# aerius-labs/paillier-halo2

Hardware: AMD Instinct MI355X
Metric: Paillier-encrypt proofs/s (2048-bit n, k=17); MSM achieved HBM GB/s vs peak (higher is better)
Workload: dtype u32 limbs (29-bit reduced radix, 254-bit modular integers), u64 limbs (4096-bit integers)

## Files before the change

### include/pz.h

```cpp
#ifndef PZ_H
#define PZ_H

#include <stddef.h>
#include <stdint.h>

#ifdef __cplusplus
extern "C" {
#endif

typedef struct pz_ctx pz_ctx;
typedef struct pz_bases pz_bases;

enum pz_status {
    PZ_OK = 0,
    PZ_ERR_INVALID = -1,
    PZ_ERR_HIP = -2,
    PZ_ERR_NO_DEVICE = -3,
    PZ_ERR_OOM = -4,
    PZ_ERR_ZERO_MODULUS = -5,
    PZ_ERR_RANGE = -6,
    PZ_ERR_UNSUPPORTED = -7,
    PZ_ERR_CAPACITY = -8,
    PZ_ERR_MESSAGE_RANGE = -9,
    PZ_ERR_ASYNC = -10
// ... 135 lines not shown
                     const uint8_t* d_selectors, const uint64_t* constants, size_t n_constants, const uint32_t* d_map_col,
                     const uint32_t* d_map_row, size_t tile, uint64_t* fixed_affine, uint64_t* sigma_affine);
int pz_vk_keygen(pz_ctx* ctx, const pz_bases* bases_lagrange, uint32_t k, uint32_t lookup_bits, size_t n_adv, size_t n_lk,
                 const uint8_t* selectors, const uint64_t* constants, size_t n_constants, const uint32_t* map_col, const uint32_t* map_row,
                 size_t tile, uint64_t* fixed_affine, uint64_t* sigma_affine);
int pz_g1_compress_dev(pz_ctx* ctx, const uint64_t* d_points, size_t n, uint8_t* d_bytes);
int pz_g1_decompress_dev(pz_ctx* ctx, const uint8_t* d_bytes, size_t n, uint64_t* d_points, int32_t* d_status);
int pz_g1_compress(pz_ctx* ctx, const uint64_t* points, size_t n, uint8_t* bytes);
int pz_g1_decompress(pz_ctx* ctx, const uint8_t* bytes, size_t n, uint64_t* points, int32_t* status, uint64_t* n_bad);
int pz_proof_wire_bytes(const pz_vk* vk, size_t* bytes);
int pz_proof_encode(pz_vk* vk, const uint64_t* proofs_words, size_t n_proofs, uint8_t* out_bytes);
int pz_proof_decode(pz_vk* vk, const uint8_t* bytes, size_t n_proofs, uint64_t* out_words, int32_t* status);
int pz_verify_batch_bytes(pz_vk* vk, const uint8_t* bytes, size_t n_proofs, const uint8_t* seeds, const size_t* seed_offsets,
                          int32_t* verdicts, uint64_t* h_evals, uint64_t* ab_affine, int* all_ok);
typedef struct pz_params pz_params;
#define PZ_SERDE_PROCESSED 0
#define PZ_SERDE_RAW 1
#define PZ_SERDE_RAW_UNCHECKED 2
#define PZ_PARAMS_BAD_G1 1u
#define PZ_PARAMS_BAD_G2 2u
#define PZ_PARAMS_BAD_G0 4u
#define PZ_PARAMS_BAD_POWERS 8u
#define PZ_PARAMS_BAD_LAGRANGE 16u
int pz_g2_compress(pz_ctx* ctx, const uint64_t* points, size_t n, uint8_t* bytes);
int pz_g2_decompress(pz_ctx* ctx, const uint8_t* bytes, size_t n, uint64_t* points, int32_t* status, uint64_t* n_bad);
int pz_g2_check_dev(pz_ctx* ctx, const uint64_t* d_points, size_t n, int32_t* d_status);
int pz_g2_check(pz_ctx* ctx, const uint64_t* points, size_t n, int32_t* status);
int pz_params_file_bytes(uint32_t k, int format, size_t* bytes);
int pz_params_decode(pz_ctx* ctx, const uint8_t* bytes, size_t len, int format, pz_params** out, uint64_t* n_bad);
int pz_params_from_dev(pz_ctx* ctx, uint32_t k, const uint64_t* d_g, const uint64_t* d_g_lagrange, const uint64_t g2[16],
                       const uint64_t s_g2[16], pz_params** out);
int pz_params_info(const pz_params* params, uint32_t* k, uint64_t g0_affine[8], uint64_t g2[16], uint64_t s_g2[16]);
int pz_params_points(const pz_params* params, const uint64_t** d_g, const uint64_t** d_g_lagrange);
int pz_params_bases(pz_params* params, int lagrange, const pz_bases** bases);
int pz_params_encode(const pz_params* params, int format, uint8_t* out, size_t capacity);
int pz_params_downsize(const pz_params* params, uint32_t k_new, pz_params** out);
int pz_params_check(pz_params* params, uint32_t* failed, uint32_t* skipped);
int pz_params_free(pz_params* params);
int pz_poly_eval_dev(pz_ctx* ctx, const uint64_t* d_coeffs, size_t n_cols, size_t col_stride, size_t n,
                     const uint64_t x[4], uint64_t* d_out);
int pz_poly_eval_multi_dev(pz_ctx* ctx, const uint64_t* d_coeffs, size_t n_cols, size_t col_stride, size_t n,
                           const uint64_t* xs, uint32_t n_points, uint64_t* d_out);

int pz_fr_batch_invert_dev(pz_ctx* ctx, uint64_t* d_a, size_t n);
int pz_fr_prefix_product_dev(pz_ctx* ctx, const uint64_t* d_a, size_t n, const uint64_t z0[4], uint64_t* d_z);
int pz_permutation_product_dev(pz_ctx* ctx, const uint64_t* d_cols, size_t col_stride, const uint64_t* d_sigma,
                               size_t sigma_stride, size_t m, uint32_t log_n, const uint64_t omega[4],
                               const uint64_t beta[4], const uint64_t gamma[4], const uint64_t delta_start[4],
                               const uint64_t delta[4], const uint64_t z0[4], uint64_t* d_z);
int pz_permutation_product_sets_dev(pz_ctx* ctx, const uint64_t* d_cols, size_t col_stride, const uint64_t* d_sigma,
                                    size_t sigma_stride, size_t m, uint32_t chunk_len, uint32_t log_n, size_t usable_rows,
                                    const uint64_t omega[4], const uint64_t beta[4], const uint64_t gamma[4],
                                    const uint64_t delta[4], uint64_t* d_z, size_t z_stride);
int pz_lookup_permute_dev(pz_ctx* ctx, const uint64_t* d_inputs, size_t n_cols, size_t col_stride,
                          const uint64_t* d_table, size_t rows, uint32_t value_bits, uint64_t* d_perm_inputs,
                          uint64_t* d_perm_tables, size_t out_stride);
int pz_lookup_product_dev(pz_ctx* ctx, const uint64_t* d_inputs, size_t input_stride, const uint64_t* d_table,
                          const uint64_t* d_perm_inputs, size_t perm_input_stride, const uint64_t* d_perm_tables,
                          size_t perm_table_stride, size_t n_lookups, size_t n, const uint64_t beta[4],
                          const uint64_t gamma[4], const uint64_t z0[4], uint64_t* d_z, size_t z_stride);
int pz_quotient_gate_dev(pz_ctx* ctx, const uint64_t* d_adv_ext, size_t adv_stride, const uint64_t* d_sel_ext,
                         size_t sel_stride, size_t n_cols, uint32_t log_ext, uint32_t rot_step, const uint64_t y[4],
                         uint64_t* d_h);
int pz_quotient_permutation_dev(pz_ctx* ctx, const uint64_t* d_cols_ext, size_t col_stride, const uint64_t* d_sigma_ext,
                                size_t sigma_stride, const uint64_t* d_z_ext, size_t z_stride, uint32_t n_sets,
                                uint32_t chunk_len, uint32_t m_total, uint32_t log_ext, uint32_t rot_step,
                                uint32_t last_rotation, const uint64_t* d_l0, const uint64_t* d_l_last,
                                const uint64_t* d_l_active, const uint64_t beta[4], const uint64_t gamma[4],
                                const uint64_t delta[4], const uint64_t coset_g[4], const uint64_t omega_ext[4],
                                const uint64_t y[4], uint64_t* d_h);
int pz_quotient_permutation_part_dev(pz_ctx* ctx, const uint64_t* d_cols_ext, size_t col_stride, const uint64_t* d_sigma_ext,
                                     size_t sigma_stride, const uint64_t* d_z_ext, size_t z_stride, uint32_t n_sets_total,
                                     uint32_t set_lo, uint32_t n_sets, uint32_t chunk_len, uint32_t m_cols, int head, uint32_t log_ext,
                                     uint32_t rot_step, uint32_t last_rotation, const uint64_t* d_l0, const uint64_t* d_l_last,
                                     const uint64_t* d_l_active, const uint64_t beta[4], const uint64_t gamma[4],
                                     const uint64_t delta[4], const uint64_t coset_g[4], const uint64_t omega_ext[4],
                                     const uint64_t y[4], uint64_t* d_h);
int pz_quotient_lookup_dev(pz_ctx* ctx, const uint64_t* d_input_ext, size_t input_stride, const uint64_t* d_table_ext,
                           const uint64_t* d_perm_input_ext, size_t perm_input_stride, const uint64_t* d_perm_table_ext,
                           size_t perm_table_stride, const uint64_t* d_z_ext, size_t z_stride, uint32_t n_lookups,
                           uint32_t log_ext, uint32_t rot_step, const uint64_t* d_l0, const uint64_t* d_l_last,
                           const uint64_t* d_l_active, const uint64_t beta[4], const uint64_t gamma[4], const uint64_t y[4],
                           uint64_t* d_h);
int pz_quotient_finish_dev(pz_ctx* ctx, uint64_t* d_h, uint32_t log_n, uint32_t log_e, const uint64_t coset_g[4],
                           const uint64_t omega_ext[4]);
int pz_fr_distribute_powers_dev(pz_ctx* ctx, uint64_t* d_a, size_t n_cols, size_t col_stride, size_t n,
                                const uint64_t g[4], const uint64_t c[4]);
int pz_fr_lincomb_dev(pz_ctx* ctx, const uint64_t* d_polys, size_t n_cols, size_t col_stride, size_t n,
                      const uint64_t v[4], uint64_t* d_out, int accumulate);
int pz_poly_div_linear_dev(pz_ctx* ctx, const uint64_t* d_coeffs, size_t n_cols, size_t col_stride, size_t n,
                           const uint64_t x[4], uint64_t* d_q, size_t q_stride);

typedef struct pz_shplonk pz_shplonk;
int pz_shplonk_begin_dev(pz_ctx* ctx, size_t n, uint32_t n_sets, const uint32_t* set_n_polys, const uint64_t* const* d_polys,
                         const uint32_t* set_n_points, const uint32_t* point_idx, uint32_t n_points_total, const uint64_t* points,
                         const uint64_t* evals, const uint64_t y[4], const uint64_t v[4], uint64_t* d_h, pz_shplonk** state);
int pz_shplonk_finish_dev(pz_ctx* ctx, pz_shplonk* state, const uint64_t u[4], const uint64_t* d_h, uint64_t* d_h2);
int pz_shplonk_free(pz_ctx* ctx, pz_shplonk* state);

typedef struct pz_structure pz_structure;
int pz_circuit_structure_dev(pz_ctx* ctx, int kind, uint32_t limbs_n, uint32_t limb_bits, uint32_t lookup_bits, uint32_t k,
                             const uint64_t* exp_g, const uint64_t* exp_r, size_t minimum_rows, uint32_t blinding_factors,
                             pz_structure** out);
int pz_structure_info(const pz_structure* st, size_t* n_adv, size_t* n_adv_filled, size_t* n_lk, size_t* max_rows, size_t* n_constants,
                      size_t* n_cells, size_t* n_lookups, size_t* n_steps_g, size_t* n_steps_r);
int pz_structure_arrays(const pz_structure* st, const uint8_t** d_selectors, const uint32_t** d_map_col, const uint32_t** d_map_row,
                        const uint64_t** d_col_starts, const uint64_t** constants, const uint64_t** col_starts_host);
int pz_structure_free(pz_structure* st);

typedef struct pz_pk pz_pk;
typedef struct pz_proof pz_proof;
#define PZ_BLINDING_SEEDED_TEST_STREAM (~(size_t)0)
#define PZ_PK_EXT_ALL (~(size_t)0)
int pz_pk_create(pz_ctx* ctx, const pz_bases* bases_lagrange, const pz_bases* bases_monomial, uint32_t k, uint32_t lookup_bits,
                 uint32_t blinding_factors, size_t max_rows, size_t n_adv, size_t n_lk, const uint8_t* selectors,
                 const uint64_t* constants, size_t n_constants, const uint32_t* map_col, const uint32_t* map_row, size_t tile,
                 size_t ext_resident_cols, pz_pk** out);
int pz_pk_create_dev(pz_ctx* ctx, const pz_bases* bases_lagrange, const pz_bases* bases_monomial, uint32_t k, uint32_t lookup_bits,
                     uint32_t blinding_factors, size_t max_rows, size_t n_adv, size_t n_lk, const uint8_t* d_selectors,
                     const uint64_t* constants, size_t n_constants, const uint32_t* d_map_col, const uint32_t* d_map_row, size_t tile,
                     size_t ext_resident_cols, pz_pk** out);
int pz_pk_info(const pz_pk* pk, size_t* n_fixed, size_t* n_perm_cols, size_t* n_sets, size_t* blinding_words, size_t* evals_words);
int pz_pk_commitments(const pz_pk* pk, uint64_t* fixed_affine, uint64_t* sigma_affine);
int pz_pk_free(pz_pk* pk);
int pz_proof_begin(pz_pk* pk, uint64_t* d_cols, uint64_t seed, const uint64_t* blinding, size_t n_blinding, pz_proof** out,
                   uint64_t* advice_affine);
int pz_proof_lookups(pz_proof* proof, const uint64_t theta[4], uint64_t* perm_inputs_affine, uint64_t* perm_tables_affine);
int pz_proof_products(pz_proof* proof, const uint64_t beta[4], const uint64_t gamma[4], uint64_t* perm_z_affine,
                      uint64_t* lookup_z_affine, uint64_t* random_affine);
int pz_proof_quotient(pz_proof* proof, const uint64_t y[4], uint64_t* h_affine);
int pz_proof_evaluate(pz_proof* proof, const uint64_t x[4], uint64_t* evals);
int pz_proof_open_begin(pz_proof* proof, const uint64_t y[4], const uint64_t v[4], uint64_t* w1_affine);
int pz_proof_open_finish(pz_proof* proof, const uint64_t u[4], uint64_t* w2_affine, int* quotient_degree_ok);
int pz_proof_free(pz_proof* proof);

int pz_circuit_public_cells(int kind, uint32_t limbs_n, uint32_t limb_bits, uint32_t lookup_bits, size_t n_steps_g, size_t n_steps_r,
                            uint64_t* cells_out, size_t capacity, size_t* n_public);
int pz_structure_expose(pz_structure* st);
int pz_structure_public(const pz_structure* st, size_t* n_instance, size_t* n_public, const uint32_t** d_cell_col, const uint32_t** d_cell_row);
int pz_public_gather_dev(pz_ctx* ctx, const uint64_t* d_cols, size_t col_stride, const uint32_t* d_cell_col, const uint32_t* d_cell_row,
                         size_t n_public, uint64_t* out_words);
int pz_instance_eval_dev(pz_ctx* ctx, uint32_t k, const uint64_t omega[4], const uint64_t n_inv[4], const uint64_t* d_instances,
                         size_t n_public, size_t n_proofs, const uint64_t* d_x, uint64_t* d_out, int32_t* d_flags);
int pz_pk_create_pub(pz_ctx* ctx, const pz_bases* bases_lagrange, const pz_bases* bases_monomial, uint32_t k, uint32_t lookup_bits,
                     uint32_t blinding_factors, size_t max_rows, size_t n_adv, size_t n_lk, size_t n_instance, size_t n_public,
                     const uint8_t* selectors, const uint64_t* constants, size_t n_constants, const uint32_t* map_col, const uint32_t* map_row,
                     size_t tile, size_t ext_resident_cols, pz_pk** out);
int pz_pk_create_pub_dev(pz_ctx* ctx, const pz_bases* bases_lagrange, const pz_bases* bases_monomial, uint32_t k, uint32_t lookup_bits,
                         uint32_t blinding_factors, size_t max_rows, size_t n_adv, size_t n_lk, size_t n_instance, size_t n_public,
                         const uint8_t* d_selectors, const uint64_t* constants, size_t n_constants, const uint32_t* d_map_col,
                         const uint32_t* d_map_row, size_t tile, size_t ext_resident_cols, pz_pk** out);
int pz_vk_keygen_pub_dev(pz_ctx* ctx, const pz_bases* bases_lagrange, uint32_t k, uint32_t lookup_bits, size_t n_adv, size_t n_lk,
                         size_t n_instance, size_t n_public, const uint8_t* d_selectors, const uint64_t* constants, size_t n_constants,
                         const uint32_t* d_map_col, const uint32_t* d_map_row, size_t tile, uint64_t* fixed_affine, uint64_t* sigma_affine);
int pz_vk_keygen_pub(pz_ctx* ctx, const pz_bases* bases_lagrange, uint32_t k, uint32_t lookup_bits, size_t n_adv, size_t n_lk,
                     size_t n_instance, size_t n_public, const uint8_t* selectors, const uint64_t* constants, size_t n_constants,
                     const uint32_t* map_col, const uint32_t* map_row, size_t tile, uint64_t* fixed_affine, uint64_t* sigma_affine);
int pz_vk_create_pub(pz_ctx* ctx, uint32_t k, uint32_t blinding_factors, size_t n_adv, size_t n_lk, size_t n_instance, size_t n_public,
                     const uint64_t* fixed_affine, const uint64_t* sigma_affine, const uint64_t g0_affine[8], const uint64_t g2[16],
                     const uint64_t s_g2[16], pz_vk** out);
int pz_proof_begin_pub(pz_pk* pk, uint64_t* d_cols, uint64_t seed, const uint64_t* blinding, size_t n_blinding, const uint64_t* instances,
                       size_t n_public, pz_proof** out, uint64_t* advice_affine);
int pz_verify_batch_pub(pz_vk* vk, const uint64_t* instances, size_t n_public, const uint64_t* proofs, size_t n_proofs, const uint8_t* seeds,
                        const size_t* seed_offsets, int32_t* verdicts, uint64_t* h_evals, uint64_t* ab_affine, int* all_ok);
int pz_verify_batch_bytes_pub(pz_vk* vk, const uint64_t* instances, size_t n_public, const uint8_t* bytes, size_t n_proofs,
                              const uint8_t* seeds, const size_t* seed_offsets, int32_t* verdicts, uint64_t* h_evals, uint64_t* ab_affine,
// ... 17 lines not shown
```

### paillier_halo2_amd/_lib.py

```python
from __future__ import annotations

import ctypes as C
import os
import subprocess

_HERE = os.path.dirname(os.path.abspath(__file__))
CSRC = os.path.join(_HERE, "csrc")
SO_PATH = os.path.join(CSRC, "libpz_hip.so")
PROBE_SO_PATH = os.path.join(CSRC, "libpz_probe.so")

U64P = C.POINTER(C.c_uint64)
U32P = C.POINTER(C.c_uint32)
VP = C.c_void_p

SIGNATURES = {
    "pz_init": (C.c_int, [C.c_int, C.POINTER(C.c_int), C.POINTER(VP)]),
    "pz_free": (C.c_int, [VP]),
    "pz_strerror": (C.c_char_p, [C.c_int]),
    "pz_last_hip_error": (C.c_char_p, [VP]),
    "pz_set_stream": (C.c_int, [VP, VP]),
    "pz_sync": (C.c_int, [VP]),
    "pz_abi_version": (C.c_int, []),
    "pz_dev_alloc": (C.c_int, [VP, C.c_size_t, C.POINTER(VP)]),
    "pz_dev_cache_limit": (C.c_int, [VP, C.c_size_t]),
# ... 27 lines not shown
    "pz_ntt_fr_to_dev": (C.c_int, [VP, VP, C.c_size_t, VP, C.c_size_t, C.c_size_t, VP, C.c_uint32, VP, VP]),
    "pz_ntt_fr_extend_dev": (C.c_int, [VP, VP, C.c_size_t, C.c_size_t, VP, C.c_size_t, C.c_uint32, C.c_uint32, VP, VP, VP]),
    "pz_ntt_fr_coeff_extend_dev": (C.c_int, [VP, VP, C.c_size_t, C.c_size_t, VP, C.c_size_t, C.c_uint32, C.c_uint32, VP, VP, VP,
                                             VP]),
    "pz_fr_convert_dev": (C.c_int, [VP, VP, C.c_size_t, C.c_int]),
    "pz_fr_from_mask_dev": (C.c_int, [VP, VP, C.c_size_t, VP]),
    "pz_mul_mod": (C.c_int, [VP, C.c_uint32, VP, VP, VP, VP, VP]),
    "pz_paillier_trace": (C.c_int, [VP, C.c_uint32, VP, VP, VP, C.c_uint32, VP, C.POINTER(C.c_size_t), VP]),
    "pz_paillier_encrypt": (C.c_int, [VP, C.c_uint32, C.c_size_t, VP, VP, VP, VP, VP, C.c_size_t, VP, VP, VP]),
    "pz_paillier_encrypt_dev": (C.c_int, [VP, C.c_uint32, C.c_size_t, VP, VP, VP, VP, VP, C.c_size_t, VP, VP, VP]),
    "pz_paillier_encrypt_uniform": (C.c_int, [VP, C.c_uint32, C.c_size_t, C.c_uint32, VP, VP, VP, VP, VP, C.c_size_t, VP, VP, VP]),
    "pz_paillier_encrypt_uniform_dev": (C.c_int, [VP, C.c_uint32, C.c_size_t, C.c_uint32, VP, VP, VP, VP, VP, C.c_size_t, VP, VP, VP]),
    "pz_witness_cells_per_step": (C.c_int, [C.c_uint32, C.c_uint32, C.c_uint32, C.POINTER(C.c_size_t),
                                            C.POINTER(C.c_size_t)]),
    "pz_witness_expand": (C.c_int, [VP, C.c_uint32, C.c_uint32, C.c_uint32, VP, C.c_size_t, VP, VP, VP]),
    "pz_witness_expand_dev": (C.c_int, [VP, C.c_uint32, C.c_uint32, C.c_uint32, VP, C.c_size_t, VP, VP, VP]),
    "pz_refresh_aux": (C.c_int, [C.c_uint32, C.c_uint32, C.c_uint32, VP, C.c_uint32, U32P]),
    "pz_op_cells": (C.c_int, [C.c_int, C.c_uint32, C.c_uint32, C.c_uint32, C.POINTER(C.c_size_t), C.POINTER(C.c_size_t)]),
    "pz_circuit_cells": (C.c_int, [C.c_int, C.c_uint32, C.c_uint32, C.c_uint32, C.c_size_t, C.c_size_t, C.POINTER(C.c_size_t),
                                   C.POINTER(C.c_size_t)]),
    "pz_circuit_expand_dev": (C.c_int, [VP, C.c_int, C.c_uint32, C.c_uint32, C.c_uint32, VP, VP, C.c_size_t, C.c_size_t, VP, VP, VP,
                                        C.c_size_t, C.c_size_t]),
    "pz_circuit_break_points": (C.c_int, [VP, C.c_size_t, C.c_size_t, VP, C.c_size_t, C.POINTER(C.c_size_t)]),
    "pz_circuit_expand_cols_dev": (C.c_int, [VP, C.c_int, C.c_uint32, C.c_uint32, C.c_uint32, VP, VP, C.c_size_t, C.c_size_t, VP, VP, VP,
                                             VP, C.c_size_t, C.c_size_t, C.c_size_t, C.c_size_t]),
    "pz_srs_setup_g1_dev": (C.c_int, [VP, C.c_uint32, VP, VP, VP, VP]),
    "pz_srs_lagrange_from_monomial_dev": (C.c_int, [VP, C.c_uint32, VP, VP, VP, VP]),
    "pz_permutation_sigma_dev": (C.c_int, [VP, VP, VP, C.c_size_t, C.c_uint32, VP, VP, VP, C.c_size_t]),
    "pz_permutation_sigma_part_dev": (C.c_int, [VP, VP, VP, C.c_size_t, C.c_size_t, C.c_size_t, C.c_uint32, VP, VP, VP, C.c_size_t]),
    "pz_keygen_columns_dev": (C.c_int, [VP, VP, VP, C.c_size_t, C.c_size_t, C.c_uint32, C.c_uint32, VP, VP, VP, VP, VP, VP, C.c_size_t]),
    "pz_poly_eval_dev": (C.c_int, [VP, VP, C.c_size_t, C.c_size_t, C.c_size_t, VP, VP]),
    "pz_poly_eval_multi_dev": (C.c_int, [VP, VP, C.c_size_t, C.c_size_t, C.c_size_t, VP, C.c_uint32, VP]),
    "pz_g1_check_dev": (C.c_int, [VP, VP, C.c_size_t, C.POINTER(C.c_uint64)]),
    "pz_g2_generator": (C.c_int, [VP]),
    "pz_g2_mul_dev": (C.c_int, [VP, VP, VP, C.c_size_t, VP]),
    "pz_pairing_dev": (C.c_int, [VP, VP, VP, C.c_size_t, VP]),
    "pz_pairing_check_dev": (C.c_int, [VP, VP, VP, C.c_size_t, C.c_uint32, VP]),
    "pz_vk_create": (C.c_int, [VP, C.c_uint32, C.c_uint32, C.c_size_t, C.c_size_t, VP, VP, VP, VP, VP, C.POINTER(VP)]),
    "pz_vk_info": (C.c_int, [VP, C.POINTER(C.c_size_t), C.POINTER(C.c_size_t)]),
    "pz_verify_batch": (C.c_int, [VP, VP, C.c_size_t, VP, VP, VP, VP, VP, C.POINTER(C.c_int)]),
    "pz_vk_free": (C.c_int, [VP]),
    "pz_vk_keygen_dev": (C.c_int, [VP, VP, C.c_uint32, C.c_uint32, C.c_size_t, C.c_size_t, VP, VP, C.c_size_t, VP, VP, C.c_size_t, VP, VP]),
    "pz_vk_keygen": (C.c_int, [VP, VP, C.c_uint32, C.c_uint32, C.c_size_t, C.c_size_t, VP, VP, C.c_size_t, VP, VP, C.c_size_t, VP, VP]),
    "pz_g1_compress_dev": (C.c_int, [VP, VP, C.c_size_t, VP]),
    "pz_g1_decompress_dev": (C.c_int, [VP, VP, C.c_size_t, VP, VP]),
    "pz_g1_compress": (C.c_int, [VP, VP, C.c_size_t, VP]),
    "pz_g1_decompress": (C.c_int, [VP, VP, C.c_size_t, VP, VP, C.POINTER(C.c_uint64)]),
    "pz_proof_wire_bytes": (C.c_int, [VP, C.POINTER(C.c_size_t)]),
    "pz_proof_encode": (C.c_int, [VP, VP, C.c_size_t, VP]),
    "pz_proof_decode": (C.c_int, [VP, VP, C.c_size_t, VP, VP]),
    "pz_verify_batch_bytes": (C.c_int, [VP, VP, C.c_size_t, VP, VP, VP, VP, VP, C.POINTER(C.c_int)]),
    "pz_g2_compress": (C.c_int, [VP, VP, C.c_size_t, VP]),
    "pz_g2_decompress": (C.c_int, [VP, VP, C.c_size_t, VP, VP, C.POINTER(C.c_uint64)]),
    "pz_g2_check_dev": (C.c_int, [VP, VP, C.c_size_t, VP]),
    "pz_g2_check": (C.c_int, [VP, VP, C.c_size_t, VP]),
    "pz_params_file_bytes": (C.c_int, [C.c_uint32, C.c_int, C.POINTER(C.c_size_t)]),
    "pz_params_decode": (C.c_int, [VP, VP, C.c_size_t, C.c_int, C.POINTER(VP), C.POINTER(C.c_uint64)]),
    "pz_params_from_dev": (C.c_int, [VP, C.c_uint32, VP, VP, VP, VP, C.POINTER(VP)]),
    "pz_params_info": (C.c_int, [VP, U32P, VP, VP, VP]),
    "pz_params_points": (C.c_int, [VP, C.POINTER(VP), C.POINTER(VP)]),
    "pz_params_bases": (C.c_int, [VP, C.c_int, C.POINTER(VP)]),
    "pz_params_encode": (C.c_int, [VP, C.c_int, VP, C.c_size_t]),
    "pz_params_downsize": (C.c_int, [VP, C.c_uint32, C.POINTER(VP)]),
    "pz_params_check": (C.c_int, [VP, U32P, U32P]),
    "pz_params_free": (C.c_int, [VP]),
    "pz_fr_batch_invert_dev": (C.c_int, [VP, VP, C.c_size_t]),
    "pz_fr_prefix_product_dev": (C.c_int, [VP, VP, C.c_size_t, VP, VP]),
    "pz_permutation_product_dev": (C.c_int, [VP, VP, C.c_size_t, VP, C.c_size_t, C.c_size_t, C.c_uint32, VP, VP, VP, VP,
                                             VP, VP, VP]),
    "pz_lookup_permute_dev": (C.c_int, [VP, VP, C.c_size_t, C.c_size_t, VP, C.c_size_t, C.c_uint32, VP, VP, C.c_size_t]),
    "pz_lookup_product_dev": (C.c_int, [VP, VP, C.c_size_t, VP, VP, C.c_size_t, VP, C.c_size_t, C.c_size_t, C.c_size_t, VP, VP,
                                        VP, VP, C.c_size_t]),
    "pz_permutation_product_sets_dev": (C.c_int, [VP, VP, C.c_size_t, VP, C.c_size_t, C.c_size_t, C.c_uint32, C.c_uint32,
                                                  C.c_size_t, VP, VP, VP, VP, VP, C.c_size_t]),
    "pz_quotient_gate_dev": (C.c_int, [VP, VP, C.c_size_t, VP, C.c_size_t, C.c_size_t, C.c_uint32, C.c_uint32, VP, VP]),
    "pz_quotient_permutation_dev": (C.c_int, [VP, VP, C.c_size_t, VP, C.c_size_t, VP, C.c_size_t, C.c_uint32, C.c_uint32,
                                              C.c_uint32, C.c_uint32, C.c_uint32, C.c_uint32, VP, VP, VP, VP, VP, VP, VP, VP,
                                              VP, VP]),
    "pz_quotient_permutation_part_dev": (C.c_int, [VP, VP, C.c_size_t, VP, C.c_size_t, VP, C.c_size_t, C.c_uint32, C.c_uint32, C.c_uint32,
                                                   C.c_uint32, C.c_uint32, C.c_int, C.c_uint32, C.c_uint32, C.c_uint32, VP, VP, VP, VP, VP,
                                                   VP, VP, VP, VP, VP]),
    "pz_quotient_lookup_dev": (C.c_int, [VP, VP, C.c_size_t, VP, VP, C.c_size_t, VP, C.c_size_t, VP, C.c_size_t, C.c_uint32,
                                         C.c_uint32, C.c_uint32, VP, VP, VP, VP, VP, VP, VP]),
    "pz_quotient_finish_dev": (C.c_int, [VP, VP, C.c_uint32, C.c_uint32, VP, VP]),
    "pz_fr_distribute_powers_dev": (C.c_int, [VP, VP, C.c_size_t, C.c_size_t, C.c_size_t, VP, VP]),
    "pz_fr_lincomb_dev": (C.c_int, [VP, VP, C.c_size_t, C.c_size_t, C.c_size_t, VP, VP, C.c_int]),
    "pz_poly_div_linear_dev": (C.c_int, [VP, VP, C.c_size_t, C.c_size_t, C.c_size_t, VP, VP, C.c_size_t]),
    "pz_shplonk_begin_dev": (C.c_int, [VP, C.c_size_t, C.c_uint32, U32P, C.POINTER(VP), U32P, U32P, C.c_uint32, VP, VP, VP, VP, VP,
                                       C.POINTER(VP)]),
    "pz_shplonk_finish_dev": (C.c_int, [VP, VP, VP, VP, VP]),
    "pz_shplonk_free": (C.c_int, [VP, VP]),
    "pz_circuit_structure_dev": (C.c_int, [VP, C.c_int, C.c_uint32, C.c_uint32, C.c_uint32, C.c_uint32, VP, VP, C.c_size_t, C.c_uint32, C.POINTER(VP)]),
    "pz_structure_info": (C.c_int, [VP] + [C.POINTER(C.c_size_t)] * 9),
    "pz_structure_arrays": (C.c_int, [VP] + [C.POINTER(VP)] * 6),
    "pz_structure_free": (C.c_int, [VP]),
    "pz_pk_create": (C.c_int, [VP, VP, VP, C.c_uint32, C.c_uint32, C.c_uint32, C.c_size_t, C.c_size_t, C.c_size_t, VP, VP, C.c_size_t, VP, VP,
                               C.c_size_t, C.c_size_t, C.POINTER(VP)]),
    "pz_pk_create_dev": (C.c_int, [VP, VP, VP, C.c_uint32, C.c_uint32, C.c_uint32, C.c_size_t, C.c_size_t, C.c_size_t, VP, VP, C.c_size_t, VP, VP,
                                   C.c_size_t, C.c_size_t, C.POINTER(VP)]),
    "pz_pk_info": (C.c_int, [VP, C.POINTER(C.c_size_t), C.POINTER(C.c_size_t), C.POINTER(C.c_size_t), C.POINTER(C.c_size_t),
                             C.POINTER(C.c_size_t)]),
    "pz_pk_commitments": (C.c_int, [VP, VP, VP]),
    "pz_pk_free": (C.c_int, [VP]),
    "pz_proof_begin": (C.c_int, [VP, VP, C.c_uint64, VP, C.c_size_t, C.POINTER(VP), VP]),
    "pz_proof_lookups": (C.c_int, [VP, VP, VP, VP]),
    "pz_proof_products": (C.c_int, [VP, VP, VP, VP, VP, VP]),
    "pz_proof_quotient": (C.c_int, [VP, VP, VP]),
    "pz_proof_evaluate": (C.c_int, [VP, VP, VP]),
    "pz_proof_open_begin": (C.c_int, [VP, VP, VP, VP]),
    "pz_proof_open_finish": (C.c_int, [VP, VP, VP, C.POINTER(C.c_int)]),
    "pz_proof_free": (C.c_int, [VP]),
    "pz_circuit_public_cells": (C.c_int, [C.c_int, C.c_uint32, C.c_uint32, C.c_uint32, C.c_size_t, C.c_size_t, VP, C.c_size_t, C.POINTER(C.c_size_t)]),
    "pz_structure_expose": (C.c_int, [VP]),
    "pz_structure_public": (C.c_int, [VP, C.POINTER(C.c_size_t), C.POINTER(C.c_size_t), C.POINTER(VP), C.POINTER(VP)]),
    "pz_public_gather_dev": (C.c_int, [VP, VP, C.c_size_t, VP, VP, C.c_size_t, VP]),
    "pz_instance_eval_dev": (C.c_int, [VP, C.c_uint32, VP, VP, VP, C.c_size_t, C.c_size_t, VP, VP, VP]),
    "pz_pk_create_pub": (C.c_int, [VP, VP, VP, C.c_uint32, C.c_uint32, C.c_uint32, C.c_size_t, C.c_size_t, C.c_size_t, C.c_size_t, C.c_size_t, VP, VP,
                                   C.c_size_t, VP, VP, C.c_size_t, C.c_size_t, C.POINTER(VP)]),
    "pz_pk_create_pub_dev": (C.c_int, [VP, VP, VP, C.c_uint32, C.c_uint32, C.c_uint32, C.c_size_t, C.c_size_t, C.c_size_t, C.c_size_t, C.c_size_t, VP,
                                       VP, C.c_size_t, VP, VP, C.c_size_t, C.c_size_t, C.POINTER(VP)]),
    "pz_vk_keygen_pub_dev": (C.c_int, [VP, VP, C.c_uint32, C.c_uint32, C.c_size_t, C.c_size_t, C.c_size_t, C.c_size_t, VP, VP, C.c_size_t, VP, VP,
                                       C.c_size_t, VP, VP]),
    "pz_vk_keygen_pub": (C.c_int, [VP, VP, C.c_uint32, C.c_uint32, C.c_size_t, C.c_size_t, C.c_size_t, C.c_size_t, VP, VP, C.c_size_t, VP, VP,
                                   C.c_size_t, VP, VP]),
    "pz_vk_create_pub": (C.c_int, [VP, C.c_uint32, C.c_uint32, C.c_size_t, C.c_size_t, C.c_size_t, C.c_size_t, VP, VP, VP, VP, VP, C.POINTER(VP)]),
    "pz_proof_begin_pub": (C.c_int, [VP, VP, C.c_uint64, VP, C.c_size_t, VP, C.c_size_t, C.POINTER(VP), VP]),
    "pz_verify_batch_pub": (C.c_int, [VP, VP, C.c_size_t, VP, C.c_size_t, VP, VP, VP, VP, VP, C.POINTER(C.c_int)]),
    "pz_verify_batch_bytes_pub": (C.c_int, [VP, VP, C.c_size_t, VP, C.c_size_t, VP, VP, VP, VP, VP, C.POINTER(C.c_int)]),
    "pz_key_digest": (C.c_int, [C.c_uint32, C.c_uint32, C.c_size_t, C.c_size_t, C.c_size_t, C.c_size_t, VP, VP, VP]),
    "pz_pk_digest": (C.c_int, [VP, VP]),
    "pz_vk_digest": (C.c_int, [VP, VP]),
    "pz_vk_bind": (C.c_int, [VP, C.c_int]),
    "pz_vk_is_bound": (C.c_int, [VP, C.POINTER(C.c_int)]),
    "pz_timing_enable": (C.c_int, [VP, C.c_int]),
    "pz_timing_reset": (C.c_int, [VP]),
    "pz_timing_get": (C.c_int, [VP, C.c_int, C.POINTER(C.c_double), C.POINTER(C.c_uint64)]),
}

_lib = None


def build(force: bool = False) -> str:
    args = ["make", "-C", CSRC, "-j4"]
    if force:
        args.append("-B")
    subprocess.check_call(args, stdout=subprocess.DEVNULL)
    if not os.path.exists(SO_PATH):
        raise RuntimeError("libpz_hip.so was not produced by the build")
    return SO_PATH


def lib():
    global _lib
    if _lib is None:
        if not os.path.exists(SO_PATH):
            raise RuntimeError(
                f"{SO_PATH} is missing: build it with `python -c 'import __graft_entry__ as g; g.build()'` "
                "(hipcc --offload-arch=gfx950). There is no CPU fallback."
            )
        try:
            import torch
        except Exception:
            pass
        l = C.CDLL(SO_PATH)
        for name, (res, args) in SIGNATURES.items():
            fn = getattr(l, name)
# ... 37 lines not shown
```

### paillier_halo2_amd/csrc/pz_quotient.hip

```cpp
#include "fp29.cuh"
#include "pz_internal.h"

static inline Fr fp_one_host() {
    static const uint64_t ONE[4] = {0xac96341c4ffffffbULL, 0x36fc76959f60cd29ULL, 0x666ea36f7879462eULL, 0x0e0a77c19a07df2fULL};
    Fr r;
    memcpy(r.v, ONE, 32);
    return r;
}
static inline Fr fr_from_u64(const uint64_t x[4]) {
    Fr r;
    memcpy(r.v, x, 32);
    return r;
}

typedef F29<FrTag> Fr29;
__device__ __forceinline__ Fr29 fr29_c261(const Fr& c) { return f29_to_261(f29_from_fp(c)); }
__device__ __forceinline__ Fr29 fr29_one256() {
    Fr29 r;
#pragma unroll
    for (int i = 0; i < 9; ++i) r.v[i] = P29<FrTag>::R256(i);
    return r;
}

struct S29 {
// ... 502 lines not shown
    const Fr* p = a + (size_t)blockIdx.y * cs;
    const size_t lo = c * KD_K, hi = (lo + KD_K < n ? lo + KD_K : n);
    Fr v = fp_zero<FrTag>();
    for (size_t i = hi; i-- > lo;) v = fp_add(fp_mul(v, x), fp_load<FrTag>(p + i));
    fp_store(L + (size_t)blockIdx.y * n_chunks + c, v);
}
__global__ __launch_bounds__(256) void k_kd_carry(Fr* __restrict__ L, size_t n_chunks, Fr x) {
    __shared__ Fr s_v[256], s_x[256];
    Fr* l = L + (size_t)blockIdx.x * n_chunks;
    Fr xk = x;
    for (unsigned s = 1; s < KD_K; s <<= 1) xk = fp_sqr(xk);
    const size_t per = (n_chunks + 255) / 256;
    const size_t lo = threadIdx.x * per, hi = lo + per < n_chunks ? lo + per : n_chunks;
    Fr V = fp_zero<FrTag>(), X = fp_one<FrTag>();
    for (size_t c = hi; c-- > lo && c < n_chunks;) {
        V = fp_add(fp_load<FrTag>(l + c), fp_mul(xk, V));
        X = fp_mul(X, xk);
    }
    s_v[threadIdx.x] = V;
    s_x[threadIdx.x] = X;
    __syncthreads();
    for (unsigned off = 1; off < 256; off <<= 1) {
        Fr v = s_v[threadIdx.x], xx = s_x[threadIdx.x];
        Fr uv = fp_zero<FrTag>(), ux = fp_one<FrTag>();
        const bool has = threadIdx.x + off < 256;
        if (has) { uv = s_v[threadIdx.x + off]; ux = s_x[threadIdx.x + off]; }
        __syncthreads();
        if (has) {
            s_v[threadIdx.x] = fp_add(v, fp_mul(xx, uv));
            s_x[threadIdx.x] = fp_mul(xx, ux);
        }
        __syncthreads();
    }
    Fr carry = threadIdx.x + 1 < 256 ? s_v[threadIdx.x + 1] : fp_zero<FrTag>();
    for (size_t c = hi; c-- > lo && c < n_chunks;) {
        Fr t = fp_load<FrTag>(l + c);
        fp_store(l + c, carry);
        carry = fp_add(t, fp_mul(xk, carry));
    }
}
__global__ __launch_bounds__(256) void k_kd_apply(const Fr* a, size_t cs, size_t n, Fr x,
                                                  const Fr* __restrict__ L, size_t n_chunks, Fr* q, size_t qs) {
    const size_t c = (size_t)blockIdx.x * blockDim.x + threadIdx.x;
    if (c >= n_chunks) return;
    const Fr* p = a + (size_t)blockIdx.y * cs;
    Fr* o = q + (size_t)blockIdx.y * qs;
    const size_t lo = c * KD_K, hi = (lo + KD_K < n ? lo + KD_K : n);
    Fr cur = fp_load<FrTag>(L + (size_t)blockIdx.y * n_chunks + c);
    for (size_t i = hi; i-- > lo;) {
        Fr ai = fp_load<FrTag>(p + i);
        fp_store(o + i, cur);
        cur = fp_add(ai, fp_mul(x, cur));
    }
}

extern "C" int pz_poly_div_linear_dev(pz_ctx* ctx, const uint64_t* d_coeffs, size_t n_cols, size_t col_stride, size_t n,
                                      const uint64_t x[4], uint64_t* d_q, size_t q_stride) {
    if (!ctx || !x || (n_cols && n && (!d_coeffs || !d_q)) || col_stride % 4 || q_stride % 4) return PZ_ERR_INVALID;
    if (n_cols > 1 && (col_stride < 4 * n || q_stride < 4 * n)) return PZ_ERR_INVALID;
    if (n_cols == 0 || n == 0) return PZ_OK;
    if (n_cols > 65535) return PZ_ERR_INVALID;
    PZ_ENTER(ctx);
    const size_t nch = pz_div_up(n, KD_K);
    void* L;
    PZCHK(pz_ws_get(ctx, WS_BIG_A, n_cols * nch * 32, &L));
    Fr xv = fr_from_u64(x);
    hipLaunchKernelGGL(k_kd_local, dim3(pz_div_up(nch, 256), (unsigned)n_cols), dim3(256), 0, ctx->stream,
                       (const Fr*)d_coeffs, col_stride / 4, n, xv, (Fr*)L, nch);
    hipLaunchKernelGGL(k_kd_carry, dim3((unsigned)n_cols), dim3(256), 0, ctx->stream, (Fr*)L, nch, xv);
    hipLaunchKernelGGL(k_kd_apply, dim3(pz_div_up(nch, 256), (unsigned)n_cols), dim3(256), 0, ctx->stream,
                       (const Fr*)d_coeffs, col_stride / 4, n, xv, (const Fr*)L, nch, (Fr*)d_q, q_stride / 4);
    HIPCHK(ctx, hipGetLastError());
    return PZ_OK;
}

struct PermQ {
    const Fr *cols, *sigma, *z, *l0, *llast, *lactive, *xpow;
    size_t cs, ss, zs, N;
    unsigned n_sets, chunk_len, m_total, step, last_rot;
    unsigned set_lo, n_sets_total, head;
    S29 y, gamma, delta, beta266;
    S29 bx266;
    S29 y_chain, y_sets;
};
__global__ __launch_bounds__(256) void k_quotient_permutation(PermQ q, Fr* __restrict__ h) {
    const size_t i0 = (size_t)blockIdx.x * blockDim.x + threadIdx.x;
    const size_t half = q.N >> 1;
    if (i0 >= half) return;
    const size_t mask = q.N - 1;
    size_t row[2], i_next[2], i_last[2];
    Fr29 acc[2];
#pragma unroll
    for (int r = 0; r < 2; ++r) {
        row[r] = i0 + (r ? half : 0);
        i_next[r] = (row[r] + q.step) & mask;
        i_last[r] = (row[r] + q.N - (size_t)q.last_rot * q.step) & mask;
        acc[r] = f29_load<FrTag>(h + row[r]);
    }
#pragma unroll
    for (int r = 0; r < 2 && q.head; ++r) {
        const size_t i = row[r];
        const Fr29 one = fr29_one256();
        const Fr29 l0 = f29_load_shl5<FrTag>(q.l0 + i);
        const Fr29 z_first = f29_load<FrTag>(q.z + i);
        acc[r] = f29_mul2_s(acc[r], q.y.v, f29_sub<2, 29>(one, z_first), l0);
        {
            const Fr29 ll = f29_load_shl5<FrTag>(q.llast + i);
            const Fr zl = fp_load<FrTag>(q.z + (size_t)(q.n_sets_total - 1) * q.zs + i);
            const Fr29 z_lastset = f29_from_fp(zl);
            acc[r] = f29_mul2_s(acc[r], q.y.v, f29_sub<2, 29>(f29_mul(z_lastset, f29_from_fp_shl5(zl)), z_lastset), ll);
        }
        if (q.n_sets_total > 1) {
            Fr29 t0 = f29_sub<2, 29>(f29_load<FrTag>(q.z + q.zs + i), f29_load<FrTag>(q.z + i_last[r]));
            for (unsigned j = 2; j < q.n_sets_total; ++j) {
                const Fr29 d = f29_sub<2, 29>(f29_load<FrTag>(q.z + (size_t)j * q.zs + i), f29_load<FrTag>(q.z + (size_t)(j - 1) * q.zs + i_last[r]));
                t0 = f29_add(f29_mul_s(t0, q.y.v), d);
            }
            acc[r] = f29_mul2_s(acc[r], q.y_chain.v, t0, l0);
        }
    }
    Fr29 cur = f29_mul_s(f29_load<FrTag>(q.xpow + i0), q.bx266.v);
    unsigned c = 0;
    Fr v_n[2], s_n[2];
#pragma unroll
    for (int r = 0; r < 2; ++r) {
        v_n[r] = fp_load<FrTag>(q.cols + row[r]);
        s_n[r] = fp_load<FrTag>(q.sigma + row[r]);
    }
    Fr29 hs[2];
    for (unsigned j = 0; j < q.n_sets; ++j) {
        Fr29 left[2], right[2];
#pragma unroll
        for (int r = 0; r < 2; ++r) {
            left[r] = f29_load<FrTag>(q.z + (size_t)(q.set_lo + j) * q.zs + i_next[r]);
            right[r] = f29_load<FrTag>(q.z + (size_t)(q.set_lo + j) * q.zs + row[r]);
        }
        for (unsigned t = 0; t < q.chunk_len && c < q.m_total; ++t, ++c) {
            const unsigned cn = c + 1 < q.m_total ? c + 1 : c;
#pragma unroll
            for (int r = 0; r < 2; ++r) {
                const Fr29 v = f29_add_s(f29_from_fp_shl5(v_n[r]), q.gamma.v);
                const Fr29 sg = f29_from_fp(s_n[r]);
                v_n[r] = fp_load<FrTag>(q.cols + (size_t)cn * q.cs + row[r]);
                s_n[r] = fp_load<FrTag>(q.sigma + (size_t)cn * q.ss + row[r]);
                left[r] = f29_mul(left[r], f29_add(v, f29_mul_s(sg, q.beta266.v)));
                right[r] = f29_mul(right[r], r ? f29_sub<2, 29>(v, cur) : f29_add(v, cur));
            }
            cur = f29_mul_s(cur, q.delta.v);
        }
#pragma unroll
        for (int r = 0; r < 2; ++r) {
            const Fr29 diff = f29_sub<2, 29>(left[r], right[r]);
            hs[r] = j ? f29_add(f29_mul_s(hs[r], q.y.v), diff) : diff;
        }
    }
#pragma unroll
    for (int r = 0; r < 2; ++r) {
        acc[r] = f29_mul2_s(acc[r], q.y_sets.v, hs[r], f29_load_shl5<FrTag>(q.lactive + row[r]));
        f29_store<0>(h + row[r], acc[r]);
    }
}

extern "C" int pz_quotient_permutation_part_dev(pz_ctx* ctx, const uint64_t* d_cols_ext, size_t col_stride,
                                                const uint64_t* d_sigma_ext, size_t sigma_stride, const uint64_t* d_z_ext,
                                                size_t z_stride, uint32_t n_sets_total, uint32_t set_lo, uint32_t n_sets,
                                                uint32_t chunk_len, uint32_t m_cols, int head, uint32_t log_ext, uint32_t rot_step,
                                                uint32_t last_rotation, const uint64_t* d_l0, const uint64_t* d_l_last,
                                                const uint64_t* d_l_active, const uint64_t beta[4], const uint64_t gamma[4],
                                                const uint64_t delta[4], const uint64_t coset_g[4], const uint64_t omega_ext[4],
                                                const uint64_t y[4], uint64_t* d_h) {
    if (!ctx || !d_cols_ext || !d_sigma_ext || !d_z_ext || !d_l0 || !d_l_last || !d_l_active || !beta || !gamma || !delta ||
        !coset_g || !omega_ext || !y || !d_h)
        return PZ_ERR_INVALID;
    if (log_ext > 28 || log_ext == 0 || n_sets == 0 || chunk_len == 0 || m_cols == 0 || col_stride % 4 || sigma_stride % 4 || z_stride % 4)
        return PZ_ERR_INVALID;
    if (n_sets_total == 0 || (size_t)set_lo + n_sets > n_sets_total) return PZ_ERR_INVALID;
    const size_t N = (size_t)1 << log_ext;
    if ((size_t)n_sets * chunk_len < m_cols || (size_t)(n_sets - 1) * chunk_len >= m_cols) return PZ_ERR_INVALID;
    if (set_lo + n_sets < n_sets_total && (size_t)n_sets * chunk_len != m_cols) return PZ_ERR_INVALID;
    if (rot_step == 0 || rot_step >= N || (size_t)last_rotation * rot_step >= N) return PZ_ERR_INVALID;
    if ((m_cols > 1 && (col_stride < 4 * N || sigma_stride < 4 * N)) || (n_sets_total > 1 && z_stride < 4 * N)) return PZ_ERR_INVALID;
    if (!host_fr_canonical(beta) || !host_fr_canonical(gamma) || !host_fr_canonical(delta) || !host_fr_canonical(y)) return PZ_ERR_INVALID;
    PZ_ENTER(ctx);
    PermQ q;
    q.cols = (const Fr*)d_cols_ext; q.sigma = (const Fr*)d_sigma_ext; q.z = (const Fr*)d_z_ext;
    q.l0 = (const Fr*)d_l0; q.llast = (const Fr*)d_l_last; q.lactive = (const Fr*)d_l_active;
    q.cs = col_stride / 4; q.ss = sigma_stride / 4; q.zs = z_stride / 4; q.N = N;
    q.n_sets = n_sets; q.chunk_len = chunk_len; q.m_total = m_cols; q.step = rot_step; q.last_rot = last_rotation;
    q.set_lo = set_lo; q.n_sets_total = n_sets_total; q.head = head ? 1u : 0u;
    q.beta266 = host_fr_shl(beta, 10); q.gamma = host_fr_shl(gamma, 5); q.delta = host_fr_shl(delta, 5); q.y = host_fr_shl(y, 5);
    uint64_t yp[4], bx[4];
    host_fr_pow(delta, set_lo * chunk_len, bx);
    host_fr_mul(bx, beta, bx);
    q.bx266 = host_fr_shl(bx, 10);
    host_fr_pow(y, n_sets_total - 1, yp);
    q.y_chain = host_fr_shl(yp, 5);
    host_fr_pow(y, n_sets, yp);
    q.y_sets = host_fr_shl(yp, 5);
    void* xp;
    PZCHK(pz_get_pow_table(ctx, omega_ext, N, &xp, coset_g));
    q.xpow = (const Fr*)xp;
    hipLaunchKernelGGL(k_quotient_permutation, dim3(pz_div_up(N / 2, 256)), dim3(256), 0, ctx->stream, q, (Fr*)d_h);
    HIPCHK(ctx, hipGetLastError());
    return PZ_OK;
}
extern "C" int pz_quotient_permutation_dev(pz_ctx* ctx, const uint64_t* d_cols_ext, size_t col_stride,
                                           const uint64_t* d_sigma_ext, size_t sigma_stride, const uint64_t* d_z_ext,
                                           size_t z_stride, uint32_t n_sets, uint32_t chunk_len, uint32_t m_total,
                                           uint32_t log_ext, uint32_t rot_step, uint32_t last_rotation,
                                           const uint64_t* d_l0, const uint64_t* d_l_last, const uint64_t* d_l_active,
                                           const uint64_t beta[4], const uint64_t gamma[4], const uint64_t delta[4],
                                           const uint64_t coset_g[4], const uint64_t omega_ext[4], const uint64_t y[4],
                                           uint64_t* d_h) {
    return pz_quotient_permutation_part_dev(ctx, d_cols_ext, col_stride, d_sigma_ext, sigma_stride, d_z_ext, z_stride, n_sets, 0, n_sets,
                                            chunk_len, m_total, 1, log_ext, rot_step, last_rotation, d_l0, d_l_last, d_l_active, beta, gamma,
                                            delta, coset_g, omega_ext, y, d_h);
}

struct LookQ {
    const Fr *a, *s, *ap, *sp, *z, *l0, *llast, *lactive;
    size_t as, aps, sps, zs, N;
    unsigned n_lookups, step;
    S29 beta, gamma, y;
};
__global__ __launch_bounds__(256) void k_quotient_lookup(LookQ q, Fr* __restrict__ h) {
    const size_t i = (size_t)blockIdx.x * blockDim.x + threadIdx.x;
    if (i >= q.N) return;
    const size_t mask = q.N - 1;
    const size_t i_next = (i + q.step) & mask, i_prev = (i + q.N - q.step) & mask;
    const Fr29 one = fr29_one256();
    const Fr29 l0 = f29_load_shl5<FrTag>(q.l0 + i), ll = f29_load_shl5<FrTag>(q.llast + i), la = f29_load_shl5<FrTag>(q.lactive + i);
    const Fr29 sg = f29_add_s(f29_load_shl5<FrTag>(q.s + i), q.gamma.v);
    Fr29 acc = f29_load<FrTag>(h + i);
    for (unsigned k = 0; k < q.n_lookups; ++k) {
        const Fr zf = fp_load<FrTag>(q.z + (size_t)k * q.zs + i);
        const Fr29 z = f29_from_fp(zf), zn = f29_load<FrTag>(q.z + (size_t)k * q.zs + i_next);
        const Fr apf = fp_load<FrTag>(q.ap + (size_t)k * q.aps + i), spf = fp_load<FrTag>(q.sp + (size_t)k * q.sps + i);
        const Fr29 ap = f29_from_fp(apf), sp = f29_from_fp(spf);
        acc = f29_mul2_s(acc, q.y.v, f29_sub<2, 29>(one, z), l0);
        acc = f29_mul2_s(acc, q.y.v, f29_sub<2, 29>(f29_mul(z, f29_from_fp_shl5(zf)), z), ll);
        const Fr29 f1 = f29_mul(f29_add_s(f29_from_fp_shl5(apf), q.beta.v), f29_add_s(f29_from_fp_shl5(spf), q.gamma.v));
        const Fr29 f2 = f29_mul(f29_add_s(f29_load_shl5<FrTag>(q.a + (size_t)k * q.as + i), q.beta.v), sg);
        acc = f29_mul2_s(acc, q.y.v, f29_sub<2, 29>(f29_mul(zn, f1), f29_mul(z, f2)), la);
        const Fr29 ams = f29_carry(f29_sub<2, 29>(ap, sp));
        acc = f29_mul2_s(acc, q.y.v, ams, l0);
        const Fr29 dprev = f29_sub<64, 29>(f29_from_fp_shl5(apf), f29_load_shl5<FrTag>(q.ap + (size_t)k * q.aps + i_prev));
        acc = f29_mul2_s(acc, q.y.v, f29_mul(ams, dprev), la);
    }
    f29_store<0>(h + i, acc);
}

extern "C" int pz_quotient_lookup_dev(pz_ctx* ctx, const uint64_t* d_input_ext, size_t input_stride, const uint64_t* d_table_ext,
                                      const uint64_t* d_perm_input_ext, size_t perm_input_stride,
                                      const uint64_t* d_perm_table_ext, size_t perm_table_stride, const uint64_t* d_z_ext,
                                      size_t z_stride, uint32_t n_lookups, uint32_t log_ext, uint32_t rot_step,
                                      const uint64_t* d_l0, const uint64_t* d_l_last, const uint64_t* d_l_active,
                                      const uint64_t beta[4], const uint64_t gamma[4], const uint64_t y[4], uint64_t* d_h) {
    if (!ctx || !d_input_ext || !d_table_ext || !d_perm_input_ext || !d_perm_table_ext || !d_z_ext || !d_l0 || !d_l_last ||
        !d_l_active || !beta || !gamma || !y || !d_h)
        return PZ_ERR_INVALID;
    if (log_ext > 28 || input_stride % 4 || perm_input_stride % 4 || perm_table_stride % 4 || z_stride % 4) return PZ_ERR_INVALID;
    const size_t N = (size_t)1 << log_ext;
    if (rot_step == 0 || rot_step >= N) return PZ_ERR_INVALID;
    if (n_lookups > 1 && (input_stride < 4 * N || perm_input_stride < 4 * N || perm_table_stride < 4 * N || z_stride < 4 * N))
        return PZ_ERR_INVALID;
    if (!host_fr_canonical(beta) || !host_fr_canonical(gamma) || !host_fr_canonical(y)) return PZ_ERR_INVALID;
    if (n_lookups == 0) return PZ_OK;
    PZ_ENTER(ctx);
    LookQ q;
    q.a = (const Fr*)d_input_ext; q.s = (const Fr*)d_table_ext; q.ap = (const Fr*)d_perm_input_ext;
    q.sp = (const Fr*)d_perm_table_ext; q.z = (const Fr*)d_z_ext;
    q.l0 = (const Fr*)d_l0; q.llast = (const Fr*)d_l_last; q.lactive = (const Fr*)d_l_active;
    q.as = input_stride / 4; q.aps = perm_input_stride / 4; q.sps = perm_table_stride / 4; q.zs = z_stride / 4; q.N = N;
    q.n_lookups = n_lookups; q.step = rot_step;
    q.beta = host_fr_shl(beta, 5); q.gamma = host_fr_shl(gamma, 5); q.y = host_fr_shl(y, 5);
    hipLaunchKernelGGL(k_quotient_lookup, dim3(pz_div_up(N, 256)), dim3(256), 0, ctx->stream, q, (Fr*)d_h);
    HIPCHK(ctx, hipGetLastError());
    return PZ_OK;
}

__global__ __launch_bounds__(256) void k_lincomb(const Fr* __restrict__ p, size_t cs, unsigned n_cols, size_t n, Fr v,
                                                 Fr* __restrict__ out, int accumulate) {
    const size_t i = (size_t)blockIdx.x * blockDim.x + threadIdx.x;
    if (i >= n) return;
    Fr acc = accumulate ? fp_load<FrTag>(out + i) : fp_zero<FrTag>();
    for (unsigned j = 0; j < n_cols; ++j) acc = fp_add(fp_mul(acc, v), fp_load<FrTag>(p + (size_t)j * cs + i));
    fp_store(out + i, acc);
}

extern "C" int pz_fr_lincomb_dev(pz_ctx* ctx, const uint64_t* d_polys, size_t n_cols, size_t col_stride, size_t n,
                                 const uint64_t v[4], uint64_t* d_out, int accumulate) {
    if (!ctx || !v || (n && (!d_out || (n_cols && !d_polys))) || col_stride % 4 || (n_cols > 1 && col_stride < 4 * n))
        return PZ_ERR_INVALID;
    if (n_cols > 0xffffffffu) return PZ_ERR_INVALID;
    if (n == 0) return PZ_OK;
    PZ_ENTER(ctx);
    hipLaunchKernelGGL(k_lincomb, dim3(pz_div_up(n, 256)), dim3(256), 0, ctx->stream, (const Fr*)d_polys, col_stride / 4,
                       (unsigned)n_cols, n, fr_from_u64(v), (Fr*)d_out, accumulate);
    HIPCHK(ctx, hipGetLastError());
    return PZ_OK;
}
```

### paillier_halo2_amd/engine.py

```python
from __future__ import annotations

import ctypes as C
from typing import Optional, Sequence, Tuple

import numpy as np

from . import _lib
from ._lib import PzError, VP


def _np(a, shape_last: Optional[int] = None) -> np.ndarray:
    arr = np.ascontiguousarray(a, dtype=np.uint64)
    if shape_last is not None and (arr.ndim == 0 or arr.shape[-1] != shape_last):
        arr = arr.reshape(-1, shape_last)
    return arr


def _ptr(a: np.ndarray) -> VP:
    return VP(a.ctypes.data)


class Bases:

    def __init__(self, engine: "Engine", handle: VP):
# ... 690 lines not shown
        self._chk(self.L.pz_poly_eval_dev(self.ctx, VP(d_coeffs), n_cols, col_stride_u64, n, _ptr(_np(x).reshape(4)),
                                          VP(d_out)), "pz_poly_eval_dev")

    def poly_eval_multi_dev(self, d_coeffs: int, n_cols: int, col_stride_u64: int, n: int, xs, d_out: int):
        x = _np(xs).reshape(-1, 4)
        self._chk(self.L.pz_poly_eval_multi_dev(self.ctx, VP(d_coeffs), n_cols, col_stride_u64, n, _ptr(x), x.shape[0], VP(d_out)),
                  "pz_poly_eval_multi_dev")

    def _fr1(self, x):
        a = _np(x).reshape(4)
        keep = self.__dict__.setdefault("_keep", [])
        keep.append(a)
        del keep[:-32]
        return _ptr(a)

    def fr_batch_invert_dev(self, d_a: int, n: int):
        self._chk(self.L.pz_fr_batch_invert_dev(self.ctx, VP(d_a), n), "pz_fr_batch_invert_dev")

    def fr_prefix_product_dev(self, d_a: int, n: int, z0, d_z: int):
        self._chk(self.L.pz_fr_prefix_product_dev(self.ctx, VP(d_a), n, self._fr1(z0), VP(d_z)), "pz_fr_prefix_product_dev")

    def permutation_product_dev(self, d_cols: int, col_stride_u64: int, d_sigma: int, sigma_stride_u64: int, m: int,
                                log_n: int, omega, beta, gamma, delta_start, delta, z0, d_z: int):
        self._chk(self.L.pz_permutation_product_dev(self.ctx, VP(d_cols), col_stride_u64, VP(d_sigma), sigma_stride_u64, m,
                                                    log_n, self._fr1(omega), self._fr1(beta), self._fr1(gamma),
                                                    self._fr1(delta_start), self._fr1(delta), self._fr1(z0), VP(d_z)),
                  "pz_permutation_product_dev")

    def lookup_permute_dev(self, d_inputs: int, n_cols: int, col_stride_u64: int, d_table: int, rows: int, value_bits: int,
                           d_perm_inputs: int, d_perm_tables: int, out_stride_u64: int):
        self._chk(self.L.pz_lookup_permute_dev(self.ctx, VP(d_inputs), n_cols, col_stride_u64, VP(d_table), rows, value_bits,
                                               VP(d_perm_inputs), VP(d_perm_tables), out_stride_u64), "pz_lookup_permute_dev")

    def lookup_product_dev(self, d_inputs: int, input_stride_u64: int, d_table: int, d_perm_inputs: int,
                           perm_input_stride_u64: int, d_perm_tables: int, perm_table_stride_u64: int, n_lookups: int, n: int,
                           beta, gamma, z0, d_z: int, z_stride_u64: int):
        self._chk(self.L.pz_lookup_product_dev(self.ctx, VP(d_inputs), input_stride_u64, VP(d_table), VP(d_perm_inputs),
                                               perm_input_stride_u64, VP(d_perm_tables), perm_table_stride_u64, n_lookups, n,
                                               self._fr1(beta), self._fr1(gamma), self._fr1(z0), VP(d_z), z_stride_u64),
                  "pz_lookup_product_dev")

    def permutation_product_sets_dev(self, d_cols: int, col_stride_u64: int, d_sigma: int, sigma_stride_u64: int, m: int,
                                     chunk_len: int, log_n: int, usable_rows: int, omega, beta, gamma, delta, d_z: int,
                                     z_stride_u64: int):
        self._chk(self.L.pz_permutation_product_sets_dev(self.ctx, VP(d_cols), col_stride_u64, VP(d_sigma), sigma_stride_u64, m,
                                                         chunk_len, log_n, usable_rows, self._fr1(omega), self._fr1(beta),
                                                         self._fr1(gamma), self._fr1(delta), VP(d_z), z_stride_u64),
                  "pz_permutation_product_sets_dev")

    def quotient_gate_dev(self, d_adv_ext: int, adv_stride_u64: int, d_sel_ext: int, sel_stride_u64: int, n_cols: int,
                          log_ext: int, rot_step: int, y, d_h: int):
        self._chk(self.L.pz_quotient_gate_dev(self.ctx, VP(d_adv_ext), adv_stride_u64, VP(d_sel_ext), sel_stride_u64,
                                              n_cols, log_ext, rot_step, self._fr1(y), VP(d_h)), "pz_quotient_gate_dev")

    def quotient_permutation_dev(self, d_cols_ext: int, col_stride_u64: int, d_sigma_ext: int, sigma_stride_u64: int,
                                 d_z_ext: int, z_stride_u64: int, n_sets: int, chunk_len: int, m_total: int, log_ext: int,
                                 rot_step: int, last_rotation: int, d_l0: int, d_l_last: int, d_l_active: int, beta, gamma,
                                 delta, coset_g, omega_ext, y, d_h: int):
        self._chk(self.L.pz_quotient_permutation_dev(
            self.ctx, VP(d_cols_ext), col_stride_u64, VP(d_sigma_ext), sigma_stride_u64, VP(d_z_ext), z_stride_u64, n_sets,
            chunk_len, m_total, log_ext, rot_step, last_rotation, VP(d_l0), VP(d_l_last), VP(d_l_active), self._fr1(beta),
            self._fr1(gamma), self._fr1(delta), self._fr1(coset_g), self._fr1(omega_ext), self._fr1(y), VP(d_h)),
            "pz_quotient_permutation_dev")

    def quotient_permutation_part_dev(self, d_cols_ext: int, col_stride_u64: int, d_sigma_ext: int, sigma_stride_u64: int, d_z_ext: int,
                                      z_stride_u64: int, n_sets_total: int, set_lo: int, n_sets: int, chunk_len: int, m_cols: int,
                                      head: bool, log_ext: int, rot_step: int, last_rotation: int, d_l0: int, d_l_last: int,
                                      d_l_active: int, beta, gamma, delta, coset_g, omega_ext, y, d_h: int):
        self._chk(self.L.pz_quotient_permutation_part_dev(
            self.ctx, VP(d_cols_ext), col_stride_u64, VP(d_sigma_ext), sigma_stride_u64, VP(d_z_ext), z_stride_u64, n_sets_total, set_lo,
            n_sets, chunk_len, m_cols, int(head), log_ext, rot_step, last_rotation, VP(d_l0), VP(d_l_last), VP(d_l_active),
            self._fr1(beta), self._fr1(gamma), self._fr1(delta), self._fr1(coset_g), self._fr1(omega_ext), self._fr1(y), VP(d_h)),
            "pz_quotient_permutation_part_dev")

    def quotient_lookup_dev(self, d_input_ext: int, input_stride_u64: int, d_table_ext: int, d_perm_input_ext: int,
                            perm_input_stride_u64: int, d_perm_table_ext: int, perm_table_stride_u64: int, d_z_ext: int,
                            z_stride_u64: int, n_lookups: int, log_ext: int, rot_step: int, d_l0: int, d_l_last: int,
                            d_l_active: int, beta, gamma, y, d_h: int):
        self._chk(self.L.pz_quotient_lookup_dev(
            self.ctx, VP(d_input_ext), input_stride_u64, VP(d_table_ext), VP(d_perm_input_ext), perm_input_stride_u64,
            VP(d_perm_table_ext), perm_table_stride_u64, VP(d_z_ext), z_stride_u64, n_lookups, log_ext, rot_step, VP(d_l0),
            VP(d_l_last), VP(d_l_active), self._fr1(beta), self._fr1(gamma), self._fr1(y), VP(d_h)), "pz_quotient_lookup_dev")

    def quotient_finish_dev(self, d_h: int, log_n: int, log_e: int, coset_g, omega_ext):
        self._chk(self.L.pz_quotient_finish_dev(self.ctx, VP(d_h), log_n, log_e, self._fr1(coset_g), self._fr1(omega_ext)),
                  "pz_quotient_finish_dev")

    def fr_distribute_powers_dev(self, d_a: int, n_cols: int, col_stride_u64: int, n: int, g, c=None):
        self._chk(self.L.pz_fr_distribute_powers_dev(self.ctx, VP(d_a), n_cols, col_stride_u64, n, self._fr1(g),
                                                     self._fr1(c) if c is not None else None),
                  "pz_fr_distribute_powers_dev")

    def fr_lincomb_dev(self, d_polys: int, n_cols: int, col_stride_u64: int, n: int, v, d_out: int, accumulate: bool = False):
        self._chk(self.L.pz_fr_lincomb_dev(self.ctx, VP(d_polys), n_cols, col_stride_u64, n, self._fr1(v), VP(d_out),
                                           int(accumulate)), "pz_fr_lincomb_dev")

    def poly_div_linear_dev(self, d_coeffs: int, n_cols: int, col_stride_u64: int, n: int, x, d_q: int, q_stride_u64: int):
        self._chk(self.L.pz_poly_div_linear_dev(self.ctx, VP(d_coeffs), n_cols, col_stride_u64, n, self._fr1(x), VP(d_q),
                                                q_stride_u64), "pz_poly_div_linear_dev")

    def shplonk_begin_dev(self, n: int, sets, points, y, v, d_h: int):
        n_sets = len(sets)
        npol = (C.c_uint32 * n_sets)(*[len(s_[0]) for s_ in sets])
        npts = (C.c_uint32 * n_sets)(*[len(s_[1]) for s_ in sets])
        ptrs = [p for s_ in sets for p in s_[0]]
        parr = (VP * len(ptrs))(*[VP(p) for p in ptrs])
        idx = [i for s_ in sets for i in s_[1]]
        iarr = (C.c_uint32 * len(idx))(*idx)
        pts = _np(points, 4)
        ev = np.ascontiguousarray(np.concatenate([_np(s_[2]).reshape(-1, 4) for s_ in sets]), dtype=np.uint64)
        st = VP()
        self._chk(self.L.pz_shplonk_begin_dev(self.ctx, n, n_sets, npol, parr, npts, iarr, pts.shape[0], _ptr(pts), _ptr(ev), self._fr1(y),
                                              self._fr1(v), VP(d_h), C.byref(st)), "pz_shplonk_begin_dev")
        return st

    def shplonk_finish_dev(self, state, u, d_h: int, d_h2: int):
        self._chk(self.L.pz_shplonk_finish_dev(self.ctx, state, self._fr1(u), VP(d_h), VP(d_h2)), "pz_shplonk_finish_dev")

    def timing_enable(self, on: bool = True):
        self._chk(self.L.pz_timing_enable(self.ctx, int(on)), "pz_timing_enable")

    def timing_reset(self):
        self._chk(self.L.pz_timing_reset(self.ctx), "pz_timing_reset")

    def timing_get(self, which: int) -> Tuple[float, int]:
        ms = C.c_double()
        n = C.c_uint64()
        self._chk(self.L.pz_timing_get(self.ctx, which, C.byref(ms), C.byref(n)), "pz_timing_get")
        return ms.value, n.value

    def dev_alloc(self, nbytes: int) -> int:
        d = VP()
        self._chk(self.L.pz_dev_alloc(self.ctx, nbytes, C.byref(d)), "pz_dev_alloc")
        return d.value or 0

    def dev_free(self, d: int):
        self._chk(self.L.pz_dev_free(self.ctx, VP(d)), "pz_dev_free")

    def dev_arena(self, nbytes: int):
        self._chk(self.L.pz_dev_arena(self.ctx, C.c_size_t(nbytes)), "pz_dev_arena")

    def dev_arena_info(self) -> dict:
        out = (C.c_uint64 * 6)()
        self._chk(self.L.pz_dev_arena_info(self.ctx, out), "pz_dev_arena_info")
        return dict(zip(("bytes", "used", "peak", "largest_hole", "served", "missed"), (int(v) for v in out)))

    def dev_mem_info(self):
        f, t = C.c_size_t(0), C.c_size_t(0)
        self._chk(self.L.pz_dev_mem_info(self.ctx, C.byref(f), C.byref(t)), "pz_dev_mem_info")
        return int(f.value), int(t.value)

    def upload(self, d_dst: int, arr):
        a = np.ascontiguousarray(arr)
        self._chk(self.L.pz_upload(self.ctx, VP(d_dst), VP(a.ctypes.data), a.nbytes), "pz_upload")

    def download(self, d_src: int, shape, dtype=np.uint64) -> np.ndarray:
        out = np.empty(shape, dtype=dtype)
        self._chk(self.L.pz_download(self.ctx, VP(out.ctypes.data), VP(d_src), out.nbytes), "pz_download")
        return out

    def dev_memset(self, d: int, value: int, nbytes: int):
        self._chk(self.L.pz_dev_memset(self.ctx, VP(d), value, nbytes), "pz_dev_memset")

    def dev_copy(self, d_dst: int, d_src: int, nbytes: int):
        self._chk(self.L.pz_dev_copy(self.ctx, VP(d_dst), VP(d_src), nbytes), "pz_dev_copy")

# ... 9 lines not shown
```

### paillier_halo2_amd/host/create_proof.hpp

```cpp
#pragma once
#include <cstdint>
#include <cstdio>
#include <cstdlib>
#include <cstring>
#include <functional>
#include <memory>
#include <string>
#include <vector>

#include "../../include/pz.h"
#include "fr_host.hpp"
#include "key_digest.hpp"
#include "transcript.hpp"

namespace pzp {
using pzh::Fr;

struct PzpError {
    int rc;
};
#ifdef PZP_THROW
#define PZP_FAIL(rc_, what_) throw ::pzp::PzpError{rc_}
#else
#define PZP_FAIL(rc_, what_)                                                                               \
// ... 168 lines not shown
        if (!dmc || !dmr) {
            void *mc = tmp.get(m * n * 4), *mr = tmp.get(m * n * 4);
            PZP_CK(pz_upload(cx.c, mc, st.map_col.data(), m * n * 4));
            PZP_CK(pz_upload(cx.c, mr, st.map_row.data(), m * n * 4));
            dmc = (const uint32_t*)mc;
            dmr = (const uint32_t*)mr;
        }
        const Fr delta = pzh::delta();
        PZP_CK(pz_permutation_sigma_dev(cx.c, dmc, dmr, m, st.k, d.omega.v, delta.v, sigma, 4 * n));
        PZP_CK(pz_sync(cx.c));
    }
    {
        Structure& s_ = pk->st;
        std::vector<uint8_t>().swap(s_.selectors);
        std::vector<uint32_t>().swap(s_.map_col);
        std::vector<uint32_t>().swap(s_.map_row);
    }
    pk->sigma_lagrange = cx.alloc(cx.cols(m) * n * 4);
    PZP_CK(pz_dev_copy(cx.c, pk->sigma_lagrange, sigma, m * n * 32));
    uint64_t* com_f = cx.alloc(cx.cols(F) * 12);
    uint64_t* com_s = cx.alloc(cx.cols(m) * 12);
    for (int pi = 0; pi < 2; ++pi) {
        pk->fixed_ext[pi] = cx.alloc((pk->res_fixed ? cx.cols(pk->res_fixed) : 1) * d.parts[pi].size * 4);
        pk->sigma_ext[pi] = cx.alloc((pk->res_sigma ? cx.cols(pk->res_sigma) : 1) * d.parts[pi].size * 4);
        pk->l_ext[pi] = cx.alloc(3 * d.parts[pi].size * 4);
        pk->table_ext[pi] = cx.alloc(d.parts[pi].size * 4);
    }
    struct Job { uint64_t* cols; size_t cnt; uint64_t* com; uint64_t** ext; size_t res; };
    Job jobs[2] = {{fixed, F, com_f, pk->fixed_ext, pk->res_fixed}, {sigma, m, com_s, pk->sigma_ext, pk->res_sigma}};
    for (auto& jb : jobs) {
        for (size_t c0 = 0; c0 < jb.cnt; c0 += 256) {
            const size_t cnt = jb.cnt - c0 < 256 ? jb.cnt - c0 : 256;
            const size_t r_here = jb.res <= c0 ? 0 : (jb.res - c0 < cnt ? jb.res - c0 : cnt);
            const size_t lo[2] = {c0, c0 + r_here}, bc[2] = {r_here, cnt - r_here};
            for (int keep = 1; keep >= 0; --keep) {
                const size_t b0 = lo[1 - keep], bn = bc[1 - keep];
                if (!bn) continue;
                const Part& A_ = d.parts[0];
                PZP_CK(pz_keygen_columns_dev(cx.c, bl, jb.cols + b0 * n * 4, bn, 4 * n, st.k, A_.log_e, d.omega.v, d.omega_inv.v, d.n_inv.v,
                                             A_.gens.data(), jb.com + b0 * 12, keep ? jb.ext[0] + b0 * A_.size * 4 : nullptr, 4 * A_.size));
                if (!keep) continue;
                const Part& B_ = d.parts[1];
                PZP_CK(pz_ntt_fr_extend_dev(cx.c, jb.cols + b0 * n * 4, bn, 4 * n, jb.ext[1] + b0 * B_.size * 4, 4 * B_.size, st.k, B_.log_e, d.omega.v,
                                            B_.gens.data(), nullptr));
            }
        }
    }
    pk->fixed_coeff = fixed;
    pk->sigma_coeff = sigma;
    for (int pi = 0; pi < 2; ++pi)
        PZP_CK(pz_ntt_fr_extend_dev(cx.c, fixed + (A + 1) * n * 4, 1, 4 * n, pk->table_ext[pi], 4 * d.parts[pi].size, st.k, d.parts[pi].log_e,
                                    d.omega.v, d.parts[pi].gens.data(), nullptr));
    {
        uint64_t* lrows = cx.alloc(3 * n * 4);
        std::vector<Fr> col(n);
        const Fr zero = {{0, 0, 0, 0}};
        for (int w = 0; w < 3; ++w) {
            for (size_t i = 0; i < n; ++i) col[i] = (w == 0 ? i == 0 : w == 1 ? i == d.usable : i < d.usable) ? pzh::FR_ONE : zero;
            upload_mont(cx, lrows + (size_t)w * n * 4, col);
        }
        PZP_CK(pz_ntt_fr_dev(cx.c, lrows, 3, 4 * n, d.omega_inv.v, st.k, nullptr, d.n_inv.v));
        for (int pi = 0; pi < 2; ++pi)
            PZP_CK(pz_ntt_fr_extend_dev(cx.c, lrows, 3, 4 * n, pk->l_ext[pi], 4 * d.parts[pi].size, st.k, d.parts[pi].log_e, d.omega.v,
                                        d.parts[pi].gens.data(), nullptr));
    }
    std::vector<uint64_t> jac(12 * (F > m ? F : m));
    pk->fixed_commit.resize(8 * F);
    pk->sigma_commit.resize(8 * m);
    PZP_CK(pz_download(cx.c, jac.data(), com_f, F * 96));
    PZP_CK(pz_g1_normalize(cx.c, jac.data(), F, pk->fixed_commit.data()));
    PZP_CK(pz_download(cx.c, jac.data(), com_s, m * 96));
    PZP_CK(pz_g1_normalize(cx.c, jac.data(), m, pk->sigma_commit.data()));
    return pk.release();
}

struct Proof {
    std::vector<std::pair<std::string, std::vector<uint64_t>>> commitments;
    std::vector<std::pair<std::string, std::vector<uint64_t>>> evals;
    std::vector<std::pair<std::string, uint32_t>> eval_points;
    bool h_degree_ok = false;
};

struct Workspace {
    uint64_t *Ap, *Sp, *Zl, *Z, *z_ext[2], *ext[2], *lk_ext[2][4], *hh[2], *hp[2], *h, *tmp, *rnd, *hcomb, *w1, *w2, *blind, *out12, *evals;
    uint64_t* key_ext[2] = {nullptr, nullptr};
    size_t tile, lt;
};

inline Workspace make_workspace(Ctx& cx, const ProvingKey& pk, size_t tile = 64) {
    const Domain& d = pk.dom;
    const size_t n = d.n, Lk = pk.st.n_lk, S = pk.n_sets, m = pk.st.m();
    Workspace w;
    w.tile = tile;
    w.lt = tile < Lk ? tile : Lk;
    w.Ap = cx.alloc(cx.cols(Lk) * n * 4); w.Sp = cx.alloc(cx.cols(Lk) * n * 4); w.Zl = cx.alloc(cx.cols(Lk) * n * 4);
    w.Z = cx.alloc(cx.cols(S) * n * 4);
    const size_t big = d.parts[0].size > d.parts[1].size ? d.parts[0].size : d.parts[1].size;
    w.z_ext[0] = w.z_ext[1] = cx.alloc(cx.cols(S) * big * 4);
    if (pk.streamed)
        for (int q = 0; q < 2; ++q) w.key_ext[q] = cx.alloc(tile * big * 4);
    for (int pi = 0; pi < 2; ++pi) {
        const size_t Np = d.parts[pi].size;
        w.ext[pi] = cx.alloc(tile * Np * 4);
        for (int q = 0; q < 4; ++q) w.lk_ext[pi][q] = cx.alloc(w.lt * Np * 4);
        w.hh[pi] = cx.alloc(2 * Np * 4);
        w.hp[pi] = cx.alloc(Np * 4);
    }
    w.h = cx.alloc(4 * n * 4);
    w.tmp = cx.alloc(2 * n * 4);
    w.rnd = cx.alloc(n * 4);
    w.hcomb = cx.alloc(n * 4);
    w.w1 = cx.alloc(n * 4);
    w.w2 = cx.alloc(n * 4);
    w.blind = cx.alloc((cx.cols(m) + cx.cols(S) + 3 * cx.cols(Lk)) * (d.bf + 1) * 4 + n * 4);
    {
        size_t pts = m - 1;
        if (2 * Lk > pts) pts = 2 * Lk;
        if (S + Lk + 1 > pts) pts = S + Lk + 1;
        if (pts < 3) pts = 3;
        w.out12 = cx.alloc(cx.cols(pts) * 12);
    }
    w.evals = cx.alloc((4 * cx.cols(m) + 4 * cx.cols(S) + 16) * 4 * 4);
    return w;
}

struct Rng {
    uint64_t s;
    const uint64_t* words = nullptr;
    size_t n_words = 0, used = 0;
    explicit Rng(uint64_t seed) : s(seed * 0x9e3779b97f4a7c15ULL + 1) {}
    Rng(const uint64_t* w, size_t n) : s(1), words(w), n_words(n) {}
    uint64_t next() {
        if (words) {
            if (used >= n_words) PZP_FAIL(PZ_ERR_INVALID, "blinding words exhausted");
            return words[used++];
        }
        s ^= s << 13; s ^= s >> 7; s ^= s << 17;
        return s;
    }
    void fill(std::vector<uint64_t>& v) {
        for (size_t i = 0; i + 3 < v.size(); i += 4) {
            for (;;) {
                for (int j = 0; j < 4; ++j) v[i + j] = next();
                v[i + 3] &= 0x3fffffffffffffffULL;
                bool below = false;
                for (int j = 3; j >= 0; --j)
                    if (v[i + j] != pzh::FR_MOD[j]) {
                        below = v[i + j] < pzh::FR_MOD[j];
                        break;
                    }
                if (below) break;
            }
        }
    }
};
inline size_t blinding_words(const ProvingKey& pk) {
    const size_t b = pk.dom.bf + 1, W = pk.st.n_adv + pk.st.n_lk, Lk = pk.st.n_lk, S = pk.n_sets;
    return 2 * 4 * (W * b + 2 * Lk * b + (S + Lk) * (b - 1) + pk.dom.n);
}

inline void blind_rows(Ctx& cx, Workspace& w, Rng& rng, uint64_t* d_cols, size_t count, size_t n, size_t row0) {
    const size_t rows = n - row0;
    std::vector<uint64_t> host(count * rows * 4);
    rng.fill(host);
    PZP_CK(pz_upload(cx.c, w.blind, host.data(), host.size() * 8));
    PZP_CK(pz_dev_copy_2d(cx.c, d_cols + row0 * 4, n * 32, w.blind, rows * 32, rows * 32, count));
}

inline Fr pow_small(const Fr& a, uint64_t e) { return pzh::pow_u64(a, e); }

struct Fam {
    const char* name;
    const uint64_t* polys;
    size_t count;
    std::vector<int> idx;
};

struct Session {
    Ctx& cx;
    ProvingKey& pk;
    Workspace& w;
    uint64_t* d_cols;
    Rng rng;
    Fr beta, gamma, y, x, xs[6];
    uint64_t* pieces = nullptr;
    std::vector<Fam> fams;
    std::vector<std::vector<uint64_t>> ev;
    pz_shplonk* state = nullptr;
    int phase = 0;
    std::vector<uint64_t> instances;
// ... 3 lines not shown
        if (state) pz_shplonk_free(cx.c, state);
    }
    void expect(int p) {
        if (phase != p) PZP_FAIL(PZ_ERR_INVALID, "proof phases out of order");
        phase = -1;
    }
    void done(int p) { phase = p + 1; }
    void commit(const pz_bases* b, const uint64_t* t, size_t count, uint64_t* out) {
        uint32_t nw = 0, cb = 0;
        size_t np = 0;
        PZP_CK(pz_bases_info(b, &np, &cb, &nw));
        PZP_CK(pz_msm_g1_dev(cx.c, b, t, count, pk.dom.n, 4 * pk.dom.n, 0, nw, out));
    }
    void affine(const uint64_t* d_jac, size_t count, uint64_t* out) {
        std::vector<uint64_t> jac(12 * count);
        PZP_CK(pz_download(cx.c, jac.data(), d_jac, count * 96));
        PZP_CK(pz_g1_normalize(cx.c, jac.data(), count, out));
    }

    void advice(uint64_t* out_affine, const std::function<void()>& after_launch = nullptr) {
        expect(0);
        const Domain& d = pk.dom;
        const size_t n = d.n, W = pk.st.n_adv + pk.st.n_lk;
        blind_rows(cx, w, rng, d_cols, W, n, d.usable);
        PZP_CK(pz_dev_copy(cx.c, d_cols + W * n * 4, pk.const_lagrange, n * 32));
        if (pk.st.n_instance) {
            if (instances.size() != 4 * pk.st.n_public) PZP_FAIL(PZ_ERR_INVALID, "instances do not match the key's n_public");
            PZP_CK(pz_dev_memset(cx.c, d_cols + (W + 1) * n * 4, 0, n * 32));
            PZP_CK(pz_upload(cx.c, d_cols + (W + 1) * n * 4, instances.data(), instances.size() * 8));
        }
        commit(pk.bl, d_cols, W, w.out12);
        if (after_launch) after_launch();
        affine(w.out12, W, out_affine);
        done(0);
    }
    void lookups(uint64_t* out_inputs, uint64_t* out_tables) {
        expect(1);
        const Domain& d = pk.dom;
        const size_t n = d.n, Lk = pk.st.n_lk;
        uint64_t* lk_in = d_cols + pk.st.n_adv * n * 4;
        PZP_CK(pz_lookup_permute_dev(cx.c, lk_in, Lk, 4 * n, pk.table_lagrange, d.usable, pk.st.lookup_bits, w.Ap, w.Sp, 4 * n));
        blind_rows(cx, w, rng, w.Ap, Lk, n, d.usable);
        blind_rows(cx, w, rng, w.Sp, Lk, n, d.usable);
        commit(pk.bl, w.Ap, Lk, w.out12);
        commit(pk.bl, w.Sp, Lk, w.out12 + Lk * 12);
        affine(w.out12, Lk, out_inputs);
        affine(w.out12 + Lk * 12, Lk, out_tables);
        done(1);
    }
    void products(const Fr& beta_, const Fr& gamma_, uint64_t* out_z, uint64_t* out_zl, uint64_t* out_random) {
        expect(2);
        beta = beta_; gamma = gamma_;
        const Domain& d = pk.dom;
        const size_t n = d.n, u = d.usable, Lk = pk.st.n_lk, S = pk.n_sets;
        const Fr delta = pzh::delta();
        uint64_t* lk_in = d_cols + pk.st.n_adv * n * 4;
        PZP_CK(pz_permutation_product_sets_dev(cx.c, d_cols, 4 * n, pk.sigma_lagrange, 4 * n, pk.st.m(), CHUNK, d.k, u, d.omega.v, beta.v, gamma.v,
                                               delta.v, w.Z, 4 * n));
        blind_rows(cx, w, rng, w.Z, S, n, u + 1);
        PZP_CK(pz_lookup_product_dev(cx.c, lk_in, 4 * n, pk.table_lagrange, w.Ap, 4 * n, w.Sp, 4 * n, Lk, n, beta.v, gamma.v, pzh::FR_ONE.v, w.Zl,
                                     4 * n));
        blind_rows(cx, w, rng, w.Zl, Lk, n, u + 1);
        blind_rows(cx, w, rng, w.rnd, 1, n, 0);
        commit(pk.bl, w.Z, S, w.out12);
        commit(pk.bl, w.Zl, Lk, w.out12 + S * 12);
        commit(pk.bm, w.rnd, 1, w.out12 + (S + Lk) * 12);
        affine(w.out12, S, out_z);
        affine(w.out12 + S * 12, Lk, out_zl);
        affine(w.out12 + (S + Lk) * 12, 1, out_random);
        done(2);
    }
    void quotient(const Fr& y_, uint64_t* out_h) {
        expect(3);
        y = y_;
        const Structure& st = pk.st;
        const Domain& d = pk.dom;
        const size_t n = d.n, A = st.n_adv, Lk = st.n_lk, m = st.m(), S = pk.n_sets, tile = w.tile;
        const unsigned k = d.k, bf = d.bf;
        const Fr delta = pzh::delta();
        auto to_coeff = [&](uint64_t* t, size_t cnt) {
            for (size_t c0 = 0; c0 < cnt; c0 += tile)
                PZP_CK(pz_ntt_fr_dev(cx.c, t + c0 * n * 4, cnt - c0 < tile ? cnt - c0 : tile, 4 * n, d.omega_inv.v, k, nullptr, d.n_inv.v));
        };
        to_coeff(d_cols, m); to_coeff(w.Ap, Lk); to_coeff(w.Sp, Lk); to_coeff(w.Z, S); to_coeff(w.Zl, Lk);
        const size_t n_perm_lines = 2 + (S - 1) + S;
        const Fr y_gate = pow_small(y, n_perm_lines + 5 * Lk);
        for (int pi = 0; pi < 2; ++pi) {
            const Part& pt = d.parts[pi];
            const size_t Np = pt.size;
            const unsigned lg = k + pt.log_e, rot = 1u << pt.log_e;
            auto extend = [&](const uint64_t* src, size_t cnt, uint64_t* dst) {
                PZP_CK(pz_ntt_fr_extend_dev(cx.c, src, cnt, 4 * n, dst, 4 * Np, k, pt.log_e, d.omega.v, pt.gens.data(), nullptr));
            };
            for (size_t s0 = 0; s0 < S; s0 += tile) extend(w.Z + s0 * n * 4, S - s0 < tile ? S - s0 : tile, w.z_ext[pi] + s0 * Np * 4);
            PZP_CK(pz_dev_memset(cx.c, w.hh[pi], 0, 2 * Np * 32));
            uint64_t *hg = w.hh[pi], *hp = w.hh[pi] + Np * 4;
            const uint64_t *l0 = pk.l_ext[pi], *llast = pk.l_ext[pi] + Np * 4, *lact = pk.l_ext[pi] + 2 * Np * 4;
            auto key_tile = [&](const uint64_t* coeff, const uint64_t* resident, size_t res, int which, size_t c0, size_t cnt) -> const uint64_t* {
                if (c0 + cnt <= res) return resident + c0 * Np * 4;
                extend(coeff + c0 * n * 4, cnt, w.key_ext[which]);
                return w.key_ext[which];
            };
            for (size_t c0 = 0; c0 < m; c0 += tile) {
                const size_t cnt = m - c0 < tile ? m - c0 : tile;
                extend(d_cols + c0 * n * 4, cnt, w.ext[pi]);
                const size_t na = c0 >= A ? 0 : (A - c0 < cnt ? A - c0 : cnt);
                if (na && pi == 0)
                    PZP_CK(pz_quotient_gate_dev(cx.c, w.ext[pi], 4 * Np, key_tile(pk.fixed_coeff, pk.fixed_ext[pi], pk.res_fixed, 0, c0, na), 4 * Np, na,
                                                lg, rot, y.v, hg));
                PZP_CK(pz_quotient_permutation_part_dev(cx.c, w.ext[pi], 4 * Np, key_tile(pk.sigma_coeff, pk.sigma_ext[pi], pk.res_sigma, 1, c0, cnt),
                                                        4 * Np, w.z_ext[pi], 4 * Np,
                                                        (uint32_t)S, (uint32_t)(c0 / CHUNK), (uint32_t)((cnt + CHUNK - 1) / CHUNK), CHUNK, (uint32_t)cnt,
                                                        c0 == 0, lg, rot, bf + 1, l0, llast, lact, beta.v, gamma.v, delta.v, pt.coset_g.v, pt.omega.v,
                                                        y.v, hp));
            }
            uint64_t* hq = w.hp[pi];
            PZP_CK(pz_dev_copy(cx.c, hq, hp, Np * 32));
            for (size_t l0_ = 0; l0_ < Lk; l0_ += w.lt) {
                const size_t cnt = Lk - l0_ < w.lt ? Lk - l0_ : w.lt;
                extend(d_cols + (A + l0_) * n * 4, cnt, w.lk_ext[pi][0]);
                extend(w.Ap + l0_ * n * 4, cnt, w.lk_ext[pi][1]);
                extend(w.Sp + l0_ * n * 4, cnt, w.lk_ext[pi][2]);
                extend(w.Zl + l0_ * n * 4, cnt, w.lk_ext[pi][3]);
                PZP_CK(pz_quotient_lookup_dev(cx.c, w.lk_ext[pi][0], 4 * Np, pk.table_ext[pi], w.lk_ext[pi][1], 4 * Np,
                                              w.lk_ext[pi][2], 4 * Np, w.lk_ext[pi][3], 4 * Np, (uint32_t)cnt, lg, rot, l0, llast, lact, beta.v, gamma.v,
                                              y.v, hq));
            }
            PZP_CK(pz_quotient_finish_dev(cx.c, hq, k, pt.log_e, pt.coset_g.v, pt.omega.v));
            PZP_CK(pz_ntt_fr_dev(cx.c, hq, 1, 4 * Np, pt.omega_inv.v, lg, nullptr, pt.size_inv.v));
            const Fr cg_inv = pzh::inv(pt.coset_g);
            PZP_CK(pz_fr_distribute_powers_dev(cx.c, hq, 1, 4 * Np, Np, cg_inv.v, nullptr));
            if (pi == 0) {
                PZP_CK(pz_quotient_finish_dev(cx.c, hg, k, pt.log_e, pt.coset_g.v, pt.omega.v));
                PZP_CK(pz_ntt_fr_dev(cx.c, hg, 1, 4 * Np, pt.omega_inv.v, lg, nullptr, pt.size_inv.v));
                PZP_CK(pz_fr_distribute_powers_dev(cx.c, hg, 1, 4 * Np, Np, cg_inv.v, nullptr));
            }
        }
        pieces = w.h;
        {
            const Fr g2n = pow_small(pzh::mul(d.coset_g, d.coset_g), n);
            const Fr lam = pow_small(d.parts[1].coset_g, n);
            uint64_t *U = w.hp[0], *h1 = w.hp[0] + n * 4, *V = w.hp[1];
            uint64_t *t0 = w.tmp, *t1 = w.tmp + n * 4;
            PZP_CK(pz_dev_copy(cx.c, pieces + n * 4, h1, n * 32));
            PZP_CK(pz_dev_copy(cx.c, t0, h1, n * 32));
            PZP_CK(pz_dev_copy(cx.c, t1, V, n * 32));
            const Fr mlam = pzh::neg(lam), m1 = pzh::neg(pzh::FR_ONE), mg2n = pzh::neg(g2n);
            PZP_CK(pz_fr_lincomb_dev(cx.c, w.tmp, 2, 4 * n, n, mlam.v, pieces + 2 * n * 4, 0));
            PZP_CK(pz_dev_copy(cx.c, t0, pieces + 2 * n * 4, n * 32));
            PZP_CK(pz_dev_copy(cx.c, t1, U, n * 32));
            PZP_CK(pz_fr_lincomb_dev(cx.c, w.tmp, 2, 4 * n, n, m1.v, pieces + 2 * n * 4, 0));
            const Fr half = pzh::inv(pzh::add(g2n, g2n));
            PZP_CK(pz_fr_distribute_powers_dev(cx.c, pieces + 2 * n * 4, 1, 4 * n, n, pzh::FR_ONE.v, half.v));
            PZP_CK(pz_dev_copy(cx.c, t0, pieces + 2 * n * 4, n * 32));
            PZP_CK(pz_dev_copy(cx.c, t1, U, n * 32));
            PZP_CK(pz_fr_lincomb_dev(cx.c, w.tmp, 2, 4 * n, n, mg2n.v, pieces, 0));
            for (size_t i = 0; i < 2; ++i) {
                PZP_CK(pz_dev_copy(cx.c, t0, w.hh[0] + i * n * 4, n * 32));
                PZP_CK(pz_dev_copy(cx.c, t1, pieces + i * n * 4, n * 32));
                PZP_CK(pz_fr_lincomb_dev(cx.c, w.tmp, 2, 4 * n, n, y_gate.v, pieces + i * n * 4, 0));
            }
        }
        commit(pk.bm, pieces, 3, w.out12);
        affine(w.out12, 3, out_h);
        done(3);
    }
    void evaluate(const Fr& x_) {
        expect(4);
        x = x_;
        const Structure& st = pk.st;
        const Domain& d = pk.dom;
        const size_t n = d.n, A = st.n_adv, Lk = st.n_lk, m = st.m(), S = pk.n_sets;
        xs[0] = x;
        xs[1] = pzh::mul(x, d.omega);
        xs[2] = pzh::mul(xs[1], d.omega);
        xs[3] = pzh::mul(xs[2], d.omega);
        xs[4] = pzh::mul(x, pow_small(d.omega_inv, d.bf + 1));
        xs[5] = pzh::mul(x, d.omega_inv);
        const Fr xn = pow_small(x, n);
        PZP_CK(pz_fr_lincomb_dev(cx.c, pieces + 2 * n * 4, 1, 4 * n, n, xn.v, w.hcomb, 0));
        PZP_CK(pz_fr_lincomb_dev(cx.c, pieces + 1 * n * 4, 1, 4 * n, n, xn.v, w.hcomb, 1));
        PZP_CK(pz_fr_lincomb_dev(cx.c, pieces, 1, 4 * n, n, xn.v, w.hcomb, 1));
        fams = {{"advice", d_cols, A, {0, 1, 2, 3}}, {"lookup_advice", d_cols + A * n * 4, Lk + 1, {0}}, {"fixed", pk.fixed_coeff, pk.F, {0}},
                {"sigma", pk.sigma_coeff, m, {0}}, {"perm_z", w.Z, S, {0, 1, 4}}, {"lookup_z", w.Zl, Lk, {0, 1}}, {"perm_inputs", w.Ap, Lk, {0, 5}},
                {"perm_tables", w.Sp, Lk, {0}}, {"random", w.rnd, 1, {0}}, {"h", w.hcomb, 1, {0}}};
        ev.assign(fams.size(), {});
        for (size_t f = 0; f < fams.size(); ++f) {
            const Fam& fm = fams[f];
            std::vector<uint64_t> pts;
            for (int i : fm.idx) pts.insert(pts.end(), xs[i].v, xs[i].v + 4);
            PZP_CK(pz_poly_eval_multi_dev(cx.c, fm.polys, fm.count, 4 * n, n, pts.data(), (uint32_t)fm.idx.size(), w.evals));
            ev[f].resize(fm.count * fm.idx.size() * 4);
            PZP_CK(pz_download(cx.c, ev[f].data(), w.evals, ev[f].size() * 8));
        }
        done(4);
    }
    void open_begin(const Fr& shy, const Fr& shv, uint64_t* out_w1) {
        expect(5);
        const size_t n = pk.dom.n, A = pk.st.n_adv, Lk = pk.st.n_lk, m = pk.st.m(), S = pk.n_sets, F = pk.F;
        auto fam_of = [&](const char* nm) -> size_t {
            for (size_t f = 0; f < fams.size(); ++f)
                if (!strcmp(fams[f].name, nm)) return f;
            return 0;
        };
        struct Member { size_t fam, idx; };
        std::vector<std::pair<std::vector<uint32_t>, std::vector<Member>>> sets;
        {
            std::vector<Member> s0;
            for (size_t i = 0; i < Lk; ++i) s0.push_back({fam_of("lookup_advice"), i});
            for (size_t i = 0; i < F; ++i) s0.push_back({fam_of("fixed"), i});
            for (size_t i = 0; i < m; ++i) s0.push_back({fam_of("sigma"), i});
            for (size_t i = 0; i < Lk; ++i) s0.push_back({fam_of("perm_tables"), i});
            s0.push_back({fam_of("h"), 0});
            s0.push_back({fam_of("random"), 0});
            sets.push_back({{0}, s0});
            std::vector<Member> s1;
            for (size_t i = 0; i < A; ++i) s1.push_back({fam_of("advice"), i});
            sets.push_back({{0, 1, 2, 3}, s1});
            if (S > 1) {
                std::vector<Member> s2;
                for (size_t i = 0; i + 1 < S; ++i) s2.push_back({fam_of("perm_z"), i});
                sets.push_back({{0, 1, 4}, s2});
            }
            std::vector<Member> s3;
            s3.push_back({fam_of("perm_z"), S - 1});
            for (size_t i = 0; i < Lk; ++i) s3.push_back({fam_of("lookup_z"), i});
            sets.push_back({{0, 1}, s3});
            std::vector<Member> s4;
            for (size_t i = 0; i < Lk; ++i) s4.push_back({fam_of("perm_inputs"), i});
            sets.push_back({{0, 5}, s4});
        }
        std::vector<uint32_t> set_n_polys, set_n_points, point_idx;
        std::vector<const uint64_t*> polys;
        std::vector<uint64_t> evals_flat, points;
        for (int i = 0; i < 6; ++i) points.insert(points.end(), xs[i].v, xs[i].v + 4);
        for (auto& sp : sets) {
            set_n_polys.push_back((uint32_t)sp.second.size());
            set_n_points.push_back((uint32_t)sp.first.size());
            for (uint32_t pi_ : sp.first) point_idx.push_back(pi_);
            for (const Member& mb : sp.second) {
                const Fam& fm = fams[mb.fam];
                polys.push_back(fm.polys + mb.idx * n * 4);
                const size_t npts = fm.idx.size();
                for (size_t q = 0; q < sp.first.size(); ++q)
                    evals_flat.insert(evals_flat.end(), &ev[mb.fam][(mb.idx * npts + q) * 4], &ev[mb.fam][(mb.idx * npts + q) * 4] + 4);
            }
        }
        PZP_CK(pz_shplonk_begin_dev(cx.c, n, (uint32_t)sets.size(), set_n_polys.data(), polys.data(), set_n_points.data(), point_idx.data(), 6,
                                    points.data(), evals_flat.data(), shy.v, shv.v, w.w1, &state));
        commit(pk.bm, w.w1, 1, w.out12);
        affine(w.out12, 1, out_w1);
        done(5);
    }
    bool open_finish(const Fr& shu, uint64_t* out_w2) {
        expect(6);
        const size_t n = pk.dom.n;
        pz_shplonk* st_ = state;
        state = nullptr;
        PZP_CK(pz_shplonk_finish_dev(cx.c, st_, shu.v, w.w1, w.w2));
        commit(pk.bm, w.w2, 1, w.out12);
        affine(w.out12, 1, out_w2);
        uint64_t top[12 + 8];
        PZP_CK(pz_download(cx.c, top, pieces + (3 * n - 3) * 4, 96));
        PZP_CK(pz_download(cx.c, top + 12, w.hh[0] + (2 * n - 2) * 4, 64));
        done(6);
        for (int i = 0; i < 12 + 8; ++i)
            if (top[i]) return false;
        return true;
    }
};

inline Proof create_proof(Ctx& cx, ProvingKey& pk, Workspace& w, uint64_t* d_cols, Transcript& tr, uint64_t seed,
                          const std::function<void()>& after_advice_launch = nullptr) {
    const size_t A = pk.st.n_adv, Lk = pk.st.n_lk, S = pk.n_sets, W = A + Lk;
    Session se(cx, pk, w, d_cols, Rng(seed));
    Proof pr;
    auto keep = [&](const char* name, const std::vector<uint64_t>& aff) {
        tr.common_points(aff.data(), aff.size() / 8);
        pr.commitments.push_back({name, aff});
    };
    std::vector<uint64_t> a(8 * W), b, c;
    se.advice(a.data(), after_advice_launch);
    tr.common_points(a.data(), W);
    pr.commitments.push_back({"advice", std::vector<uint64_t>(a.begin(), a.begin() + 8 * A)});
    pr.commitments.push_back({"lookup_advice", std::vector<uint64_t>(a.begin() + 8 * A, a.end())});
    tr.squeeze("theta");
    a.assign(8 * Lk, 0); b.assign(8 * Lk, 0);
    se.lookups(a.data(), b.data());
    keep("perm_inputs", a);
    keep("perm_tables", b);
    const Fr beta = tr.squeeze("beta"), gamma = tr.squeeze("gamma");
    a.assign(8 * S, 0); b.assign(8 * Lk, 0); c.assign(8, 0);
    se.products(beta, gamma, a.data(), b.data(), c.data());
    keep("perm_z", a);
    keep("lookup_z", b);
    keep("random", c);
    const Fr y = tr.squeeze("y");
    a.assign(24, 0);
    se.quotient(y, a.data());
    keep("h", a);
    const Fr x = tr.squeeze("x");
    se.evaluate(x);
    for (size_t f = 0; f < se.fams.size(); ++f) {
        pr.evals.push_back({se.fams[f].name, se.ev[f]});
        pr.eval_points.push_back({se.fams[f].name, (uint32_t)se.fams[f].idx.size()});
        if (strcmp(se.fams[f].name, "h")) tr.common_scalars(se.ev[f].data(), se.ev[f].size() / 4);
    }
    const Fr shy = tr.squeeze("sh_y"), shv = tr.squeeze("sh_v");
    a.assign(8, 0);
    se.open_begin(shy, shv, a.data());
    keep("w1", a);
    const Fr shu = tr.squeeze("sh_u");
    pr.h_degree_ok = se.open_finish(shu, a.data());
    keep("w2", a);
    return pr;
}

}
```

### paillier_halo2_amd/prover.py

```python
from __future__ import annotations

from dataclasses import dataclass, field
from typing import Dict, List, Optional, Sequence, Tuple

import numpy as np

from . import consts
from .engine import Bases, Engine

FR = consts.FR_R
M = consts.fr_mont_limbs

LOG_E = 2
CHUNK = 2
ZETA = pow(consts.FR_GENERATOR, (FR - 1) // 3, FR)
DELTA = pow(consts.FR_GENERATOR, 1 << consts.FR_S, FR)


@dataclass
class CircuitStructure:
    k: int
    lookup_bits: int
    max_rows: int
    blinding_factors: int
# ... 243 lines not shown

class HashTranscript(Transcript):

    PERSONAL = b"Halo2-Transcript"

    def __init__(self, seed: bytes = b"pz", key_digest: Optional[bytes] = None):
        import hashlib

        self.seed = bytes(seed)
        self.key_digest = None if key_digest is None else bytes(key_digest)
        if self.key_digest is not None and len(self.key_digest) != 64:
            raise ValueError("a key digest is 64 bytes")
        self.h = hashlib.blake2b((self.key_digest or b"") + self.seed, digest_size=64, person=self.PERSONAL)
        self.drawn: Dict[str, int] = {}

    def _items(self, tag: int, a: np.ndarray, words: int):
        a = np.ascontiguousarray(a, dtype=np.uint64).reshape(-1, words)
        buf = np.empty((a.shape[0], 1 + 8 * words), dtype=np.uint8)
        buf[:, 0] = tag
        buf[:, 1:] = a.view(np.uint8).reshape(a.shape[0], 8 * words)
        self.h.update(buf.tobytes())

    def absorb_affine(self, *host_arrays):
        for a in host_arrays:
            self._items(1, a, 8)

    def absorb_points(self, eng: Engine, *jac_tensors):
        out = [eng.g1_normalize(t.cpu().numpy().view(np.uint64)) for t in jac_tensors]
        self.absorb_affine(*out)
        return out

    def absorb_scalars(self, *host_arrays):
        for a in host_arrays:
            self._items(2, a, 4)

    def squeeze(self, name: str) -> int:
        self.h.update(b"\0")
        v = int.from_bytes(self.h.digest(), "little") % FR
        self.drawn[name] = v
        return v

    def challenges(self) -> Challenges:
        return Challenges(**self.drawn, transcript_seed=self.seed)


@dataclass
class Proof:
    commitments: Dict[str, np.ndarray] = field(default_factory=dict)
    evals: Dict[str, np.ndarray] = field(default_factory=dict)
    h_degree_ok: bool = False
    h_top: Optional[np.ndarray] = None


def rotation_points(dom: Domain, x: int) -> List[int]:
    w = dom.omega
    return [x % FR, x * w % FR, x * pow(w, 2, FR) % FR, x * pow(w, 3, FR) % FR, x * pow(w, -(dom.bf + 1), FR) % FR, x * pow(w, -1, FR) % FR]


def query_layout(A: int, Lk: int, m: int, S: int):
    F = A + 2
    sets = [([0], [("lookup_advice", i) for i in range(Lk)] + [("fixed", i) for i in range(F)] + [("sigma", i) for i in range(m)]
             + [("perm_tables", i) for i in range(Lk)] + [("h", 0), ("random", 0)]),
            ([0, 1, 2, 3], [("advice", i) for i in range(A)])]
    if S > 1:
        sets.append(([0, 1, 4], [("perm_z", i) for i in range(S - 1)]))
    sets.append(([0, 1], [("perm_z", S - 1)] + [("lookup_z", i) for i in range(Lk)]))
    sets.append(([0, 5], [("perm_inputs", i) for i in range(Lk)]))
    return sets


class Workspace:

    def __init__(self, pk: ProvingKey, tile: int = 64, lookup_tile: Optional[int] = None):
        d, st = pk.dom, pk.st
        n, N, Lk, S = d.n, d.N, st.n_lk, pk.n_sets
        assert tile % CHUNK == 0
        self.tile = tile
        self.Ap, self.Sp, self.Zl = _zeros_cap(Lk, n, 4, q=8), _zeros_cap(Lk, n, 4, q=8), _zeros_cap(Lk, n, 4, q=8)
        self.Z = _zeros_cap(S, n, 4)
        lt = min(tile, Lk, lookup_tile or tile)
        big = max(pt["size"] for pt in d.parts)
        self._z_ext_flat = _zeros_cap(S, big, 4).view(-1)
        self.z_ext = [self._z_ext_flat[: S * pt["size"] * 4].view(S, pt["size"], 4) for pt in d.parts]
        self.ext = [_zeros(tile, pt["size"], 4) for pt in d.parts]
        if pk.streamed:
            self._key_tiles = [_zeros(tile, big, 4).view(-1) for _ in range(2)]
            self.key_ext = [[kt[: tile * pt["size"] * 4].view(tile, pt["size"], 4) for kt in self._key_tiles] for pt in d.parts]
        self.lk_ext = [[_zeros(lt, pt["size"], 4) for _ in range(4)] for pt in d.parts]
        self.hh = [_zeros(2, pt["size"], 4) for pt in d.parts]
        self.hp = [_zeros(pt["size"], 4) for pt in d.parts]
        self.h = _zeros(N, 4)
        self.tmp = _zeros(2, n, 4)
        self.rnd = _zeros(1, n, 4)
        self.hcomb = _zeros(n, 4)
        self.w1, self.w2 = _zeros(n, 4), _zeros(n, 4)


def create_proof(pk: ProvingKey, cols, tr, seed: Optional[int] = 0, tile: int = 64, hooks=None, ws: Optional[Workspace] = None,
                 timings: Optional[Dict[str, float]] = None, eng: Optional[Engine] = None, instances: Optional[Sequence[int]] = None) -> Proof:
    import time

    torch = _torch()
    eng, st, d = eng or pk.eng, pk.st, pk.dom
    n, N, k, u, bf = d.n, d.N, d.k, d.usable, d.bf
    A, Lk, m, S = st.n_adv, st.n_lk, st.m, pk.n_sets
    W = A + Lk
    if isinstance(tr, Challenges):
        tr = Transcript(tr)
    if ws is None:
        ws = Workspace(pk, tile)
    tile = ws.tile
    assert tuple(cols.shape) == (m, n, 4)
    hooks = hooks or {}
    gen = torch.Generator(device="cuda")
    if seed is None:
        import os

        seed = int.from_bytes(os.urandom(8), "little") >> 1
    gen.manual_seed(seed)
    pr = Proof()
    bl, bm = pk.bases_lagrange, pk.bases_monomial
    t_last = [time.perf_counter()]

    def phase(name):
        if "on_phase" in hooks:
            hooks["on_phase"](name)
        if timings is not None:
            eng.sync()
            now = time.perf_counter()
            timings[name] = timings.get(name, 0.0) + (now - t_last[0]) * 1e3
            t_last[0] = now

    eng2, split_cols = hooks.get("commit_engine"), int(hooks.get("commit_split", 512))

    def commit(bases, t, count, stride_u64):
        out = _zeros(count, 12)
        if eng2 is None or count < 2 * split_cols:
            eng.msm_dev(bases, t.data_ptr(), count, n, stride_u64, out.data_ptr())
            return out
        eng2.wait_for(eng)
        for i, c0 in enumerate(range(0, count, split_cols)):
            (eng if i % 2 == 0 else eng2).msm_dev(bases, t[c0].data_ptr(), min(split_cols, count - c0), n, stride_u64, out[c0].data_ptr())
        eng.wait_for(eng2)
        return out

    def to_coeff(t, cnt):
        for c0 in range(0, cnt, tile):
            eng.ntt_dev(t[c0].data_ptr(), min(tile, cnt - c0), 4 * n, M(d.omega_inv), k, None, M(d.n_inv))

    def extend(src, cnt, dst, pt):
        eng.ntt_extend_dev(src.data_ptr(), cnt, 4 * n, dst.data_ptr(), 4 * pt["size"], k, pt["log_e"], M(d.omega), pt["gens"], None)

    if st.n_instance and not st.n_public:
        raise ValueError("a structure with the instance column names its public cells (at least one)")
    n_pub = st.n_public if st.n_instance else 0
    if (len(instances) if instances is not None else 0) != n_pub:
        raise ValueError("this key's statement has %d public values" % n_pub)
    if n_pub:
        if any(not 0 <= int(v) < FR for v in instances):
            raise ValueError("a public value must be a field element")
        inst_m = np.stack([M(int(v)) for v in instances]).astype(np.uint64)
        tr.absorb_scalars(inst_m.reshape(n_pub, 1, 4))
    cols[:W, u:] = _random_fr(gen, W, n - u)
    cols[W] = pk.const_lagrange
    if st.n_instance:
        cols[W + 1] = 0
        cols[W + 1, :n_pub] = torch.from_numpy(inst_m.view(np.int64)).to(cols.device)
    if "advice" in hooks:
        hooks["advice"](cols)
    c_adv = commit(bl, cols, W, 4 * n)
    if "after_advice_launch" in hooks:
        hooks["after_advice_launch"]()
    (a_adv,) = tr.absorb_points(eng, c_adv)
    tr.squeeze("theta")
    phase("advice_commit")
    Ap, Sp, Zl, Z = ws.Ap, ws.Sp, ws.Zl, ws.Z
    lk_in = cols[A:W]
    eng.lookup_permute_dev(lk_in.data_ptr(), Lk, 4 * n, pk.table_lagrange.data_ptr(), u, st.lookup_bits, Ap.data_ptr(), Sp.data_ptr(), 4 * n)
    if "permuted" in hooks:
        hooks["permuted"](Ap, Sp)
    Ap[:, u:] = _random_fr(gen, Lk, n - u)
    Sp[:, u:] = _random_fr(gen, Lk, n - u)
    c_ap, c_sp = commit(bl, Ap, Lk, 4 * n), commit(bl, Sp, Lk, 4 * n)
    a_ap, a_sp = tr.absorb_points(eng, c_ap, c_sp)
    beta_i, gamma_i = tr.squeeze("beta"), tr.squeeze("gamma")
    beta, gamma = M(beta_i), M(gamma_i)
    phase("lookup_permute_commit")
    eng.permutation_product_sets_dev(cols.data_ptr(), 4 * n, pk.sigma_lagrange.data_ptr(), 4 * n, m, CHUNK, k, u, M(d.omega), beta, gamma,
                                     M(DELTA), Z.data_ptr(), 4 * n)
    Z[:, u + 1:] = _random_fr(gen, S, n - u - 1)
    eng.lookup_product_dev(lk_in.data_ptr(), 4 * n, pk.table_lagrange.data_ptr(), Ap.data_ptr(), 4 * n, Sp.data_ptr(), 4 * n, Lk, n, beta,
                           gamma, M(1), Zl.data_ptr(), 4 * n)
    Zl[:, u + 1:] = _random_fr(gen, Lk, n - u - 1)
    if "products" in hooks:
        hooks["products"](Z, Zl)
    c_z, c_zl = commit(bl, Z, S, 4 * n), commit(bl, Zl, Lk, 4 * n)
    rnd = ws.rnd
    rnd.copy_(_random_fr(gen, 1, n))
    c_rnd = commit(bm, rnd, 1, 4 * n)
    a_z, a_zl, a_rnd = tr.absorb_points(eng, c_z, c_zl, c_rnd)
    y_i = tr.squeeze("y")
    y = M(y_i)
    phase("products_commit")
    for t, cnt in ((cols, m), (Ap, Lk), (Sp, Lk), (Z, S), (Zl, Lk)):
        to_coeff(t, cnt)
    n_perm_lines = 2 + (S - 1) + S
    lt = ws.lk_ext[0][0].shape[0]
    split_gate = len(d.parts) == 2
    for pi, pt in enumerate(d.parts):
        Np, lg, rot = pt["size"], k + pt["log_e"], pt["E"]
        cg, om = M(pt["coset_g"]), M(pt["omega"])
        z_ext = ws.z_ext[pi]
        for s0 in range(0, S, tile):
            extend(Z[s0:s0 + tile], min(tile, S - s0), z_ext[s0:s0 + tile], pt)
        ws.hh[pi].zero_()
        hg, hp = ws.hh[pi][0], ws.hh[pi][1]
        ext = ws.ext[pi]
        l0, llast, lact = (pk.l_ext[pi][i].data_ptr() for i in range(3))
        Rf, Rs = pk.ext_resident

        def key_tile(coeff, resident, R_, which, c0, cnt):
            if not pk.streamed or c0 + cnt <= R_:
                return resident[pi][c0].data_ptr()
            buf = ws.key_ext[pi][which]
            extend(coeff[c0:c0 + cnt], cnt, buf, pt)
            return buf.data_ptr()

        for c0 in range(0, m, tile):
            cnt = min(tile, m - c0)
            extend(cols[c0:c0 + cnt], cnt, ext, pt)
            na = max(0, min(A, c0 + cnt) - c0)
            if na and (pi == 0 or not split_gate):
                eng.quotient_gate_dev(ext.data_ptr(), 4 * Np, key_tile(pk.fixed_coeff, pk.fixed_ext, Rf, 0, c0, na), 4 * Np, na, lg, rot, y, hg.data_ptr())
            set_lo, nsets = c0 // CHUNK, -(-cnt // CHUNK)
            eng.quotient_permutation_part_dev(ext.data_ptr(), 4 * Np, key_tile(pk.sigma_coeff, pk.sigma_ext, Rs, 1, c0, cnt), 4 * Np, z_ext.data_ptr(), 4 * Np, S, set_lo,
                                              nsets, CHUNK, cnt, c0 == 0, lg, rot, bf + 1, l0, llast, lact, beta, gamma, M(DELTA), cg, om, y,
                                              hp.data_ptr())
        hq = ws.hp[pi]
        if split_gate:
            hq.copy_(hp)
        else:
            eng.fr_lincomb_dev(ws.hh[pi].data_ptr(), 2, 4 * Np, Np, M(pow(y_i, n_perm_lines, FR)), hq.data_ptr())
        for l0_ in range(0, Lk, lt):
            cnt = min(lt, Lk - l0_)
            e_in, e_ap, e_sp, e_zl = ws.lk_ext[pi]
            extend(cols[A + l0_:A + l0_ + cnt], cnt, e_in, pt)
            extend(Ap[l0_:l0_ + cnt], cnt, e_ap, pt)
            extend(Sp[l0_:l0_ + cnt], cnt, e_sp, pt)
            extend(Zl[l0_:l0_ + cnt], cnt, e_zl, pt)
            eng.quotient_lookup_dev(e_in.data_ptr(), 4 * Np, pk.table_ext[pi].data_ptr(), e_ap.data_ptr(), 4 * Np, e_sp.data_ptr(), 4 * Np,
                                    e_zl.data_ptr(), 4 * Np, cnt, lg, rot, l0, llast, lact, beta, gamma, y, hq.data_ptr())
        eng.quotient_finish_dev(hq.data_ptr(), k, pt["log_e"], cg, om)
        eng.ntt_dev(hq.data_ptr(), 1, 4 * Np, M(pt["omega_inv"]), lg, None, M(pt["size_inv"]))
        eng.fr_distribute_powers_dev(hq.data_ptr(), 1, 4 * Np, Np, M(pow(pt["coset_g"], -1, FR)))
        if split_gate and pi == 0:
            eng.quotient_finish_dev(hg.data_ptr(), k, pt["log_e"], cg, om)
            eng.ntt_dev(hg.data_ptr(), 1, 4 * Np, M(pt["omega_inv"]), lg, None, M(pt["size_inv"]))
            eng.fr_distribute_powers_dev(hg.data_ptr(), 1, 4 * Np, Np, M(pow(pt["coset_g"], -1, FR)))
    h = ws.h
    pieces = h.view(d.E, n, 4)
    if len(d.parts) == 1:
        h.copy_(ws.hp[0])
    else:
        g2n = pow(d.coset_g, 2 * n, FR)
        lam = pow(d.parts[1]["coset_g"], n, FR)
        U, h1, V = ws.hp[0][:n], ws.hp[0][n:], ws.hp[1]
        pieces[1].copy_(h1)
        t01 = ws.tmp
        t01[0].copy_(h1); t01[1].copy_(V)
        eng.fr_lincomb_dev(t01.data_ptr(), 2, 4 * n, n, M(-lam % FR), pieces[2].data_ptr())
        t01[0].copy_(pieces[2]); t01[1].copy_(U)
        eng.fr_lincomb_dev(t01.data_ptr(), 2, 4 * n, n, M(FR - 1), pieces[2].data_ptr())
        eng.fr_distribute_powers_dev(pieces[2].data_ptr(), 1, 4 * n, n, M(1), M(pow(2 * g2n, -1, FR)))
        t01[0].copy_(pieces[2]); t01[1].copy_(U)
        eng.fr_lincomb_dev(t01.data_ptr(), 2, 4 * n, n, M(-g2n % FR), pieces[0].data_ptr())
        pieces[3].zero_()
        c_gate = M(pow(y_i, n_perm_lines + 5 * Lk, FR))
        gq = ws.hh[0][0]
        for i in range(2):
            t01[0].copy_(gq[i * n:(i + 1) * n]); t01[1].copy_(pieces[i])
            eng.fr_lincomb_dev(t01.data_ptr(), 2, 4 * n, n, c_gate, pieces[i].data_ptr())
    c_h = commit(bm, pieces, d.E - 1, 4 * n)
    (a_h,) = tr.absorb_points(eng, c_h)
    x_i = tr.squeeze("x")
    phase("quotient")
    xs = rotation_points(d, x_i)
    P = lambda idx: np.stack([M(xs[i]) for i in idx])

    def evals(t, cnt, idx):
        out = _zeros(cnt, len(idx), 4)
        eng.poly_eval_multi_dev(t.data_ptr(), cnt, 4 * n, n, P(idx), out.data_ptr())
        return out

    xn = pow(x_i, n, FR)
    hcomb = ws.hcomb
    for i in reversed(range(d.E - 1)):
        eng.fr_lincomb_dev(pieces[i].data_ptr(), 1, 4 * n, n, M(xn), hcomb.data_ptr(), i != d.E - 2)
    F = A + 2
    e_adv = evals(cols, A, [0, 1, 2, 3])
    e_lk = evals(cols[A:], Lk + 1, [0])
    e_fix = evals(pk.fixed_coeff, F, [0])
    e_sig = evals(pk.sigma_coeff, m, [0])
    e_z = evals(Z, S, [0, 1, 4])
    e_zl = evals(Zl, Lk, [0, 1])
    e_ap = evals(Ap, Lk, [0, 5])
    e_sp = evals(Sp, Lk, [0])
    e_rnd = evals(rnd, 1, [0])
    e_h = evals(hcomb.view(1, n, 4), 1, [0])
    eng.sync()
    host = lambda t: t.cpu().numpy().view(np.uint64)
    polys = {"lookup_advice": cols[A:], "fixed": pk.fixed_coeff, "sigma": pk.sigma_coeff, "perm_tables": Sp, "h": hcomb.view(1, n, 4),
             "random": rnd, "advice": cols, "perm_z": Z, "lookup_z": Zl, "perm_inputs": Ap}
    ev = {"lookup_advice": host(e_lk), "fixed": host(e_fix), "sigma": host(e_sig), "perm_tables": host(e_sp), "h": host(e_h),
          "random": host(e_rnd), "advice": host(e_adv), "perm_z": host(e_z), "lookup_z": host(e_zl), "perm_inputs": host(e_ap)}
    tr.absorb_scalars(*[ev[f] for f in ("advice", "lookup_advice", "fixed", "sigma", "perm_z", "lookup_z", "perm_inputs", "perm_tables", "random")])
    shy, shv = tr.squeeze("sh_y"), tr.squeeze("sh_v")
    phase("evaluations")
    base_ptr = {f: t.data_ptr() for f, t in polys.items()}
    sets = []
    for idx, members in query_layout(A, Lk, m, S):
        ptrs = [base_ptr[f] + i * (n * 32) for f, i in members]
        rows, start = [], 0
        while start < len(members):
            f, i0 = members[start]
            end = start
            while end + 1 < len(members) and members[end + 1] == (f, members[end][1] + 1):
                end += 1
            rows.append(ev[f][i0:i0 + end - start + 1, :len(idx)])
            start = end + 1
        sets.append((ptrs, idx, np.concatenate(rows)))
    w1, w2 = ws.w1, ws.w2
    state = eng.shplonk_begin_dev(n, sets, np.stack([M(p) for p in xs]), M(shy), M(shv), w1.data_ptr())
    c_w1 = commit(bm, w1.view(1, n, 4), 1, 4 * n)
    (a_w1,) = tr.absorb_points(eng, c_w1)
    shu = tr.squeeze("sh_u")
    eng.shplonk_finish_dev(state, M(shu), w1.data_ptr(), w2.data_ptr())
    c_w2 = commit(bm, w2.view(1, n, 4), 1, 4 * n)
    eng.sync()
    phase("multiopen")
    pr.commitments = {"advice": a_adv[:A], "lookup_advice": a_adv[A:], "perm_inputs": a_ap, "perm_tables": a_sp,
                      "perm_z": a_z, "lookup_z": a_zl, "random": a_rnd, "h": a_h, "w1": a_w1, "w2": eng.g1_normalize(host(c_w2))}
    pr.evals = {"advice": ev["advice"], "lookup_advice": ev["lookup_advice"][:Lk], "constants": ev["lookup_advice"][Lk:], "fixed": ev["fixed"],
                "sigma": ev["sigma"], "perm_z": ev["perm_z"], "lookup_z": ev["lookup_z"], "perm_inputs": ev["perm_inputs"],
                "perm_tables": ev["perm_tables"], "random": ev["random"], "h": ev["h"]}
    top = host(h[3 * n - 3:] if len(d.parts) == 1 else h[3 * n - 3:3 * n])
    pr.h_top = top
    pr.h_degree_ok = not top.any()
    if split_gate:
        pr.h_degree_ok = pr.h_degree_ok and not host(ws.hh[0][0][2 * n - 2:2 * n]).any()
    phase("finalise")
    return pr
```

### rust/pz-sys/src/lib.rs

```rust
#![allow(non_camel_case_types)]
use core::ffi::{c_char, c_int, c_void};

#[repr(C)] pub struct pz_ctx     { _p: [u8; 0] }
#[repr(C)] pub struct pz_bases   { _p: [u8; 0] }
#[repr(C)] pub struct pz_shplonk { _p: [u8; 0] }
#[repr(C)] pub struct pz_pk      { _p: [u8; 0] }
#[repr(C)] pub struct pz_structure { _p: [u8; 0] }
#[repr(C)] pub struct pz_proof   { _p: [u8; 0] }
#[repr(C)] pub struct pz_vk      { _p: [u8; 0] }
#[repr(C)] pub struct pz_params  { _p: [u8; 0] }

extern "C" {
    pub fn pz_init(n_devices: c_int, device_ids: *const c_int, out: *mut *mut pz_ctx) -> c_int;
    pub fn pz_free(ctx: *mut pz_ctx) -> c_int;
    pub fn pz_strerror(status: c_int) -> *const c_char;
    pub fn pz_last_hip_error(ctx: *const pz_ctx) -> *const c_char;
    pub fn pz_set_stream(ctx: *mut pz_ctx, hip_stream: *mut c_void) -> c_int;
    pub fn pz_sync(ctx: *mut pz_ctx) -> c_int;
    pub fn pz_abi_version() -> c_int;

    pub fn pz_dev_alloc(ctx: *mut pz_ctx, bytes: usize, d_out: *mut *mut c_void) -> c_int;
    pub fn pz_dev_cache_limit(ctx: *mut pz_ctx, max_bytes: usize) -> c_int;
    pub fn pz_dev_arena(ctx: *mut pz_ctx, bytes: usize) -> c_int;
    pub fn pz_dev_arena_info(ctx: *mut pz_ctx, out: *mut u64) -> c_int;
// ... 161 lines not shown
                                d_selectors: *const u8, constants: *const u64, n_constants: usize, d_map_col: *const u32,
                                d_map_row: *const u32, tile: usize, ext_resident_cols: usize, out: *mut *mut pz_pk) -> c_int;
    pub fn pz_vk_keygen_pub_dev(ctx: *mut pz_ctx, bases_lagrange: *const pz_bases, k: u32, lookup_bits: u32, n_adv: usize, n_lk: usize,
                                n_instance: usize, n_public: usize, d_selectors: *const u8, constants: *const u64, n_constants: usize,
                                d_map_col: *const u32, d_map_row: *const u32, tile: usize, fixed_affine: *mut u64,
                                sigma_affine: *mut u64) -> c_int;
    pub fn pz_vk_keygen_pub(ctx: *mut pz_ctx, bases_lagrange: *const pz_bases, k: u32, lookup_bits: u32, n_adv: usize, n_lk: usize,
                            n_instance: usize, n_public: usize, selectors: *const u8, constants: *const u64, n_constants: usize,
                            map_col: *const u32, map_row: *const u32, tile: usize, fixed_affine: *mut u64, sigma_affine: *mut u64) -> c_int;
    pub fn pz_vk_create_pub(ctx: *mut pz_ctx, k: u32, blinding_factors: u32, n_adv: usize, n_lk: usize, n_instance: usize, n_public: usize,
                            fixed_affine: *const u64, sigma_affine: *const u64, g0_affine: *const u64, g2: *const u64, s_g2: *const u64,
                            out: *mut *mut pz_vk) -> c_int;
    pub fn pz_proof_begin_pub(pk: *mut pz_pk, d_cols: *mut u64, seed: u64, blinding: *const u64, n_blinding: usize, instances: *const u64,
                              n_public: usize, out: *mut *mut pz_proof, advice_affine: *mut u64) -> c_int;
    pub fn pz_verify_batch_pub(vk: *mut pz_vk, instances: *const u64, n_public: usize, proofs: *const u64, n_proofs: usize, seeds: *const u8,
                               seed_offsets: *const usize, verdicts: *mut i32, h_evals: *mut u64, ab_affine: *mut u64,
                               all_ok: *mut c_int) -> c_int;
    pub fn pz_verify_batch_bytes_pub(vk: *mut pz_vk, instances: *const u64, n_public: usize, bytes: *const u8, n_proofs: usize,
                                     seeds: *const u8, seed_offsets: *const usize, verdicts: *mut i32, h_evals: *mut u64,
                                     ab_affine: *mut u64, all_ok: *mut c_int) -> c_int;
    pub fn pz_key_digest(k: u32, blinding_factors: u32, n_adv: usize, n_lk: usize, n_instance: usize, n_public: usize,
                         fixed_affine: *const u64, sigma_affine: *const u64, out: *mut u8) -> c_int;
    pub fn pz_pk_digest(pk: *const pz_pk, out: *mut u8) -> c_int;
    pub fn pz_vk_digest(vk: *const pz_vk, out: *mut u8) -> c_int;
    pub fn pz_vk_bind(vk: *mut pz_vk, on: c_int) -> c_int;
    pub fn pz_vk_is_bound(vk: *const pz_vk, on: *mut c_int) -> c_int;
    pub fn pz_g2_compress(ctx: *mut pz_ctx, points: *const u64, n: usize, bytes: *mut u8) -> c_int;
    pub fn pz_g2_decompress(ctx: *mut pz_ctx, bytes: *const u8, n: usize, points: *mut u64, status: *mut i32, n_bad: *mut u64) -> c_int;
    pub fn pz_g2_check_dev(ctx: *mut pz_ctx, d_points: *const u64, n: usize, d_status: *mut i32) -> c_int;
    pub fn pz_g2_check(ctx: *mut pz_ctx, points: *const u64, n: usize, status: *mut i32) -> c_int;
    pub fn pz_params_file_bytes(k: u32, format: c_int, bytes: *mut usize) -> c_int;
    pub fn pz_params_decode(ctx: *mut pz_ctx, bytes: *const u8, len: usize, format: c_int, out: *mut *mut pz_params, n_bad: *mut u64) -> c_int;
    pub fn pz_params_from_dev(ctx: *mut pz_ctx, k: u32, d_g: *const u64, d_g_lagrange: *const u64, g2: *const u64, s_g2: *const u64,
                              out: *mut *mut pz_params) -> c_int;
    pub fn pz_params_info(params: *const pz_params, k: *mut u32, g0_affine: *mut u64, g2: *mut u64, s_g2: *mut u64) -> c_int;
    pub fn pz_params_points(params: *const pz_params, d_g: *mut *const u64, d_g_lagrange: *mut *const u64) -> c_int;
    pub fn pz_params_bases(params: *mut pz_params, lagrange: c_int, bases: *mut *const pz_bases) -> c_int;
    pub fn pz_params_encode(params: *const pz_params, format: c_int, out: *mut u8, capacity: usize) -> c_int;
    pub fn pz_params_downsize(params: *const pz_params, k_new: u32, out: *mut *mut pz_params) -> c_int;
    pub fn pz_params_check(params: *mut pz_params, failed: *mut u32, skipped: *mut u32) -> c_int;
    pub fn pz_params_free(params: *mut pz_params) -> c_int;
    pub fn pz_poly_eval_dev(ctx: *mut pz_ctx, d_coeffs: *const u64, n_cols: usize, col_stride: usize, n: usize,
                            x: *const u64, d_out: *mut u64) -> c_int;
    pub fn pz_poly_eval_multi_dev(ctx: *mut pz_ctx, d_coeffs: *const u64, n_cols: usize, col_stride: usize, n: usize,
                                  xs: *const u64, n_points: u32, d_out: *mut u64) -> c_int;

    pub fn pz_fr_batch_invert_dev(ctx: *mut pz_ctx, d_a: *mut u64, n: usize) -> c_int;
    pub fn pz_fr_prefix_product_dev(ctx: *mut pz_ctx, d_a: *const u64, n: usize, z0: *const u64, d_z: *mut u64) -> c_int;
    pub fn pz_permutation_product_dev(ctx: *mut pz_ctx, d_cols: *const u64, col_stride: usize, d_sigma: *const u64,
                                      sigma_stride: usize, m: usize, log_n: u32, omega: *const u64, beta: *const u64,
                                      gamma: *const u64, delta_start: *const u64, delta: *const u64, z0: *const u64,
                                      d_z: *mut u64) -> c_int;
    pub fn pz_lookup_permute_dev(ctx: *mut pz_ctx, d_inputs: *const u64, n_cols: usize, col_stride: usize, d_table: *const u64,
                                 rows: usize, value_bits: u32, d_perm_inputs: *mut u64, d_perm_tables: *mut u64,
                                 out_stride: usize) -> c_int;
    pub fn pz_lookup_product_dev(ctx: *mut pz_ctx, d_inputs: *const u64, input_stride: usize, d_table: *const u64,
                                 d_perm_inputs: *const u64, perm_input_stride: usize, d_perm_tables: *const u64,
                                 perm_table_stride: usize, n_lookups: usize, n: usize, beta: *const u64, gamma: *const u64,
                                 z0: *const u64, d_z: *mut u64, z_stride: usize) -> c_int;
    pub fn pz_permutation_product_sets_dev(ctx: *mut pz_ctx, d_cols: *const u64, col_stride: usize, d_sigma: *const u64,
                                           sigma_stride: usize, m: usize, chunk_len: u32, log_n: u32, usable_rows: usize,
                                           omega: *const u64, beta: *const u64, gamma: *const u64, delta: *const u64,
                                           d_z: *mut u64, z_stride: usize) -> c_int;
    pub fn pz_quotient_gate_dev(ctx: *mut pz_ctx, d_adv_ext: *const u64, adv_stride: usize, d_sel_ext: *const u64,
                                sel_stride: usize, n_cols: usize, log_ext: u32, rot_step: u32, y: *const u64,
                                d_h: *mut u64) -> c_int;
    pub fn pz_quotient_permutation_dev(ctx: *mut pz_ctx, d_cols_ext: *const u64, col_stride: usize, d_sigma_ext: *const u64,
                                       sigma_stride: usize, d_z_ext: *const u64, z_stride: usize, n_sets: u32, chunk_len: u32,
                                       m_total: u32, log_ext: u32, rot_step: u32, last_rotation: u32, d_l0: *const u64,
                                       d_l_last: *const u64, d_l_active: *const u64, beta: *const u64, gamma: *const u64,
                                       delta: *const u64, coset_g: *const u64, omega_ext: *const u64, y: *const u64,
                                       d_h: *mut u64) -> c_int;
    pub fn pz_quotient_permutation_part_dev(ctx: *mut pz_ctx, d_cols_ext: *const u64, col_stride: usize, d_sigma_ext: *const u64,
                                            sigma_stride: usize, d_z_ext: *const u64, z_stride: usize, n_sets_total: u32,
                                            set_lo: u32, n_sets: u32, chunk_len: u32, m_cols: u32, head: c_int, log_ext: u32,
                                            rot_step: u32, last_rotation: u32, d_l0: *const u64, d_l_last: *const u64,
                                            d_l_active: *const u64, beta: *const u64, gamma: *const u64, delta: *const u64,
                                            coset_g: *const u64, omega_ext: *const u64, y: *const u64, d_h: *mut u64) -> c_int;
    pub fn pz_quotient_lookup_dev(ctx: *mut pz_ctx, d_input_ext: *const u64, input_stride: usize, d_table_ext: *const u64,
                                  d_perm_input_ext: *const u64, perm_input_stride: usize, d_perm_table_ext: *const u64,
                                  perm_table_stride: usize, d_z_ext: *const u64, z_stride: usize, n_lookups: u32, log_ext: u32,
                                  rot_step: u32, d_l0: *const u64, d_l_last: *const u64, d_l_active: *const u64,
                                  beta: *const u64, gamma: *const u64, y: *const u64, d_h: *mut u64) -> c_int;
    pub fn pz_quotient_finish_dev(ctx: *mut pz_ctx, d_h: *mut u64, log_n: u32, log_e: u32, coset_g: *const u64,
                                  omega_ext: *const u64) -> c_int;
    pub fn pz_fr_distribute_powers_dev(ctx: *mut pz_ctx, d_a: *mut u64, n_cols: usize, col_stride: usize, n: usize,
                                       g: *const u64, c: *const u64) -> c_int;
    pub fn pz_fr_lincomb_dev(ctx: *mut pz_ctx, d_polys: *const u64, n_cols: usize, col_stride: usize, n: usize, v: *const u64,
                             d_out: *mut u64, accumulate: c_int) -> c_int;
    pub fn pz_poly_div_linear_dev(ctx: *mut pz_ctx, d_coeffs: *const u64, n_cols: usize, col_stride: usize, n: usize,
                                  x: *const u64, d_q: *mut u64, q_stride: usize) -> c_int;

    pub fn pz_witness_cells_per_step(limbs: u32, limb_bits: u32, lookup_bits: u32, advice_cells: *mut usize,
                                     lookup_cells: *mut usize) -> c_int;
    pub fn pz_witness_expand(ctx: *mut pz_ctx, limbs: u32, limb_bits: u32, lookup_bits: u32, steps: *const u64, n_steps: usize,
                             modulus: *const u64, advice_out: *mut u64, lookup_out: *mut u64) -> c_int;
    pub fn pz_witness_expand_dev(ctx: *mut pz_ctx, limbs: u32, limb_bits: u32, lookup_bits: u32,
                                 d_steps: *const u64, n_steps: usize, d_modulus: *const u64, d_advice: *mut u64,
                                 d_lookup: *mut u64) -> c_int;
    pub fn pz_circuit_cells(kind: c_int, limbs_n: u32, limb_bits: u32, lookup_bits: u32, n_steps_g: usize, n_steps_r: usize,
                            advice_cells: *mut usize, lookup_cells: *mut usize) -> c_int;
    pub fn pz_circuit_expand_dev(ctx: *mut pz_ctx, kind: c_int, limbs_n: u32, limb_bits: u32, lookup_bits: u32,
                                 inputs: *const u64, d_steps: *const u64, n_steps_g: usize, n_steps_r: usize,
                                 d_modulus: *const u64, d_advice: *mut u64, d_lookup: *mut u64, rows: usize,
                                 col_stride: usize) -> c_int;
    pub fn pz_circuit_break_points(gate_mask: *const u8, n_cells: usize, max_rows: usize, starts_out: *mut u64, capacity: usize,
                                   n_cols: *mut usize) -> c_int;
    pub fn pz_circuit_expand_cols_dev(ctx: *mut pz_ctx, kind: c_int, limbs_n: u32, limb_bits: u32, lookup_bits: u32,
                                      inputs: *const u64, d_steps: *const u64, n_steps_g: usize, n_steps_r: usize,
                                      d_modulus: *const u64, d_advice: *mut u64, d_lookup: *mut u64, d_col_starts: *const u64,
                                      n_adv_cols: usize, max_rows: usize, lookup_rows: usize, col_stride: usize) -> c_int;
    pub fn pz_refresh_aux(limb_bits: u32, num_limbs_l: u32, num_limbs_r: u32, increased_limbs: *mut u8, capacity: u32,
                          n_out: *mut u32) -> c_int;
    pub fn pz_op_cells(op: c_int, limbs: u32, limb_bits: u32, lookup_bits: u32, advice_cells: *mut usize,
                       lookup_cells: *mut usize) -> c_int;

    pub fn pz_timing_enable(ctx: *mut pz_ctx, on: c_int) -> c_int;
    pub fn pz_timing_reset(ctx: *mut pz_ctx) -> c_int;
    pub fn pz_timing_get(ctx: *mut pz_ctx, which: c_int, total_ms: *mut f64, launches: *mut u64) -> c_int;
}

const _: () = assert!(core::mem::size_of::<halo2curves::bn256::Fr>() == 32);
const _: () = assert!(core::mem::size_of::<halo2curves::bn256::Fq>() == 32);
const _: () = assert!(core::mem::size_of::<halo2curves::bn256::G1Affine>() == 64);
const _: () = assert!(core::mem::size_of::<halo2curves::bn256::G1>() == 96);
const _: () = assert!(core::mem::align_of::<halo2curves::bn256::Fr>() == 8);
```

Before: 1.307.

## Split quotient into low-degree part and l_active-multiplied degree term

Adds split variants of the permutation and lookup quotient kernels. They accumulate the terms that are multiplied by l_active into a separate buffer instead of the main quotient, and a new d_rows kernel plus a row-multiply kernel recombine them. The high-degree part is handled on the first coset part only and then reconstructed for the second part from base-domain rows, so the second coset no longer needs a full extension of every column. It also replaces copy-plus-lincomb sequences with axpy calls. The cost is extra buffers and NTT work, plus more complex algebra that must stay correct.

Measured after the change: 1.432 (median of 6 runs). +9.6%, better.

```diff
diff --git a/include/pz.h b/include/pz.h
--- a/include/pz.h
+++ b/include/pz.h
@@ -241,6 +241,27 @@
                            uint32_t log_ext, uint32_t rot_step, const uint64_t* d_l0, const uint64_t* d_l_last,
                            const uint64_t* d_l_active, const uint64_t beta[4], const uint64_t gamma[4], const uint64_t y[4],
                            uint64_t* d_h);
+int pz_quotient_permutation_split_dev(pz_ctx* ctx, const uint64_t* d_cols_ext, size_t col_stride, const uint64_t* d_sigma_ext,
+                                      size_t sigma_stride, const uint64_t* d_z_ext, size_t z_stride, uint32_t n_sets_total,
+                                      uint32_t set_lo, uint32_t n_sets, uint32_t chunk_len, uint32_t m_cols, int head, uint32_t log_ext,
+                                      uint32_t rot_step, uint32_t last_rotation, const uint64_t* d_l0, const uint64_t* d_l_last,
+                                      const uint64_t beta[4], const uint64_t gamma[4], const uint64_t delta[4],
+                                      const uint64_t coset_g[4], const uint64_t omega_ext[4], const uint64_t y[4], uint64_t* d_h_low,
+                                      uint64_t* d_h_d);
+int pz_quotient_lookup_split_dev(pz_ctx* ctx, const uint64_t* d_input_ext, size_t input_stride, const uint64_t* d_table_ext,
+                                 const uint64_t* d_perm_input_ext, size_t perm_input_stride, const uint64_t* d_perm_table_ext,
+                                 size_t perm_table_stride, const uint64_t* d_z_ext, size_t z_stride, uint32_t n_lookups,
+                                 uint32_t log_ext, uint32_t rot_step, const uint64_t* d_l0, const uint64_t* d_l_last,
+                                 const uint64_t* d_l_active, const uint64_t beta[4], const uint64_t gamma[4], const uint64_t y[4],
+                                 uint64_t* d_h_low, uint64_t* d_h_d);
+int pz_quotient_d_rows_dev(pz_ctx* ctx, const uint64_t* d_cols, size_t col_stride, const uint64_t* d_sigma, size_t sigma_stride,
+                           const uint64_t* d_z, size_t z_stride, uint32_t m, uint32_t chunk_len, const uint64_t* d_input,
+                           size_t input_stride, const uint64_t* d_table, const uint64_t* d_perm_input, size_t perm_input_stride,
+                           const uint64_t* d_perm_table, size_t perm_table_stride, const uint64_t* d_zl, size_t zl_stride,
+                           uint32_t n_lookups, uint32_t log_n, size_t row_lo, const uint64_t omega[4], const uint64_t beta[4],
+                           const uint64_t gamma[4], const uint64_t delta[4], const uint64_t y[4], uint64_t* d_out);
+int pz_fr_mul_row_dev(pz_ctx* ctx, const uint64_t* d_a, size_t n_cols, size_t col_stride, size_t n, const uint64_t* d_row,
+                      uint64_t* d_out, size_t out_stride);
 int pz_quotient_finish_dev(pz_ctx* ctx, uint64_t* d_h, uint32_t log_n, uint32_t log_e, const uint64_t coset_g[4],
                            const uint64_t omega_ext[4]);
 int pz_fr_distribute_powers_dev(pz_ctx* ctx, uint64_t* d_a, size_t n_cols, size_t col_stride, size_t n,
diff --git a/paillier_halo2_amd/_lib.py b/paillier_halo2_amd/_lib.py
--- a/paillier_halo2_amd/_lib.py
+++ b/paillier_halo2_amd/_lib.py
@@ -133,6 +133,15 @@
                                                    VP, VP, VP, VP, VP]),
     "pz_quotient_lookup_dev": (C.c_int, [VP, VP, C.c_size_t, VP, VP, C.c_size_t, VP, C.c_size_t, VP, C.c_size_t, C.c_uint32,
                                          C.c_uint32, C.c_uint32, VP, VP, VP, VP, VP, VP, VP]),
+    "pz_quotient_permutation_split_dev": (C.c_int, [VP, VP, C.c_size_t, VP, C.c_size_t, VP, C.c_size_t, C.c_uint32, C.c_uint32, C.c_uint32,
+                                                    C.c_uint32, C.c_uint32, C.c_int, C.c_uint32, C.c_uint32, C.c_uint32, VP, VP, VP, VP, VP,
+                                                    VP, VP, VP, VP, VP]),
+    "pz_quotient_lookup_split_dev": (C.c_int, [VP, VP, C.c_size_t, VP, VP, C.c_size_t, VP, C.c_size_t, VP, C.c_size_t, C.c_uint32,
+                                               C.c_uint32, C.c_uint32, VP, VP, VP, VP, VP, VP, VP, VP]),
+    "pz_quotient_d_rows_dev": (C.c_int, [VP, VP, C.c_size_t, VP, C.c_size_t, VP, C.c_size_t, C.c_uint32, C.c_uint32, VP, C.c_size_t, VP,
+                                         VP, C.c_size_t, VP, C.c_size_t, VP, C.c_size_t, C.c_uint32, C.c_uint32, C.c_size_t, VP, VP, VP, VP,
+                                         VP, VP]),
+    "pz_fr_mul_row_dev": (C.c_int, [VP, VP, C.c_size_t, C.c_size_t, C.c_size_t, VP, VP, C.c_size_t]),
     "pz_quotient_finish_dev": (C.c_int, [VP, VP, C.c_uint32, C.c_uint32, VP, VP]),
     "pz_fr_distribute_powers_dev": (C.c_int, [VP, VP, C.c_size_t, C.c_size_t, C.c_size_t, VP, VP]),
     "pz_fr_lincomb_dev": (C.c_int, [VP, VP, C.c_size_t, C.c_size_t, C.c_size_t, VP, VP, C.c_int]),
diff --git a/paillier_halo2_amd/csrc/pz_quotient.hip b/paillier_halo2_amd/csrc/pz_quotient.hip
--- a/paillier_halo2_amd/csrc/pz_quotient.hip
+++ b/paillier_halo2_amd/csrc/pz_quotient.hip
@@ -608,8 +608,9 @@
     S29 y, gamma, delta, beta266;
     S29 bx266;
     S29 y_chain, y_sets;
+    S29 y_sets_d;
 };
-__global__ __launch_bounds__(256) void k_quotient_permutation(PermQ q, Fr* __restrict__ h) {
+template <bool SPLIT> __global__ __launch_bounds__(256) void k_quotient_permutation(PermQ q, Fr* __restrict__ h, Fr* __restrict__ hd) {
     const size_t i0 = (size_t)blockIdx.x * blockDim.x + threadIdx.x;
     const size_t half = q.N >> 1;
     if (i0 >= half) return;
@@ -682,21 +683,25 @@
     }
 #pragma unroll
     for (int r = 0; r < 2; ++r) {
-        acc[r] = f29_mul2_s(acc[r], q.y_sets.v, hs[r], f29_load_shl5<FrTag>(q.lactive + row[r]));
+        if (SPLIT) {
+            f29_store<0>(hd + row[r], f29_mul2_s(f29_load<FrTag>(hd + row[r]), q.y_sets_d.v, hs[r], f29_one<FrTag>()));
+            acc[r] = f29_mul_s(acc[r], q.y_sets.v);
+        } else {
+            acc[r] = f29_mul2_s(acc[r], q.y_sets.v, hs[r], f29_load_shl5<FrTag>(q.lactive + row[r]));
+        }
         f29_store<0>(h + row[r], acc[r]);
     }
 }
 
-extern "C" int pz_quotient_permutation_part_dev(pz_ctx* ctx, const uint64_t* d_cols_ext, size_t col_stride,
-                                                const uint64_t* d_sigma_ext, size_t sigma_stride, const uint64_t* d_z_ext,
-                                                size_t z_stride, uint32_t n_sets_total, uint32_t set_lo, uint32_t n_sets,
-                                                uint32_t chunk_len, uint32_t m_cols, int head, uint32_t log_ext, uint32_t rot_step,
-                                                uint32_t last_rotation, const uint64_t* d_l0, const uint64_t* d_l_last,
-                                                const uint64_t* d_l_active, const uint64_t beta[4], const uint64_t gamma[4],
-                                                const uint64_t delta[4], const uint64_t coset_g[4], const uint64_t omega_ext[4],
-                                                const uint64_t y[4], uint64_t* d_h) {
-    if (!ctx || !d_cols_ext || !d_sigma_ext || !d_z_ext || !d_l0 || !d_l_last || !d_l_active || !beta || !gamma || !delta ||
-        !coset_g || !omega_ext || !y || !d_h)
+static int quotient_permutation_launch(pz_ctx* ctx, const uint64_t* d_cols_ext, size_t col_stride, const uint64_t* d_sigma_ext,
+                                       size_t sigma_stride, const uint64_t* d_z_ext, size_t z_stride, uint32_t n_sets_total,
+                                       uint32_t set_lo, uint32_t n_sets, uint32_t chunk_len, uint32_t m_cols, int head, uint32_t log_ext,
+                                       uint32_t rot_step, uint32_t last_rotation, const uint64_t* d_l0, const uint64_t* d_l_last,
+                                       const uint64_t* d_l_active, const uint64_t beta[4], const uint64_t gamma[4],
+                                       const uint64_t delta[4], const uint64_t coset_g[4], const uint64_t omega_ext[4],
+                                       const uint64_t y[4], uint64_t* d_h, uint64_t* d_hd) {
+    if (!ctx || !d_cols_ext || !d_sigma_ext || !d_z_ext || !d_l0 || !d_l_last || (!d_l_active && !d_hd) || !beta || !gamma || !delta ||
+        !coset_g || !omega_ext || !y || !d_h || d_h == d_hd)
         return PZ_ERR_INVALID;
     if (log_ext > 28 || log_ext == 0 || n_sets == 0 || chunk_len == 0 || m_cols == 0 || col_stride % 4 || sigma_stride % 4 || z_stride % 4)
         return PZ_ERR_INVALID;
@@ -723,12 +728,41 @@
     q.y_chain = host_fr_shl(yp, 5);
     host_fr_pow(y, n_sets, yp);
     q.y_sets = host_fr_shl(yp, 5);
+    host_fr_pow(y, n_sets + (head ? 2 + (n_sets_total > 1 ? n_sets_total - 1 : 0) : 0), yp);
+    q.y_sets_d = host_fr_shl(yp, 5);
     void* xp;
     PZCHK(pz_get_pow_table(ctx, omega_ext, N, &xp, coset_g));
     q.xpow = (const Fr*)xp;
-    hipLaunchKernelGGL(k_quotient_permutation, dim3(pz_div_up(N / 2, 256)), dim3(256), 0, ctx->stream, q, (Fr*)d_h);
-    HIPCHK(ctx, hipGetLastError());
-    return PZ_OK;
+    if (d_hd) hipLaunchKernelGGL(k_quotient_permutation<true>, dim3(pz_div_up(N / 2, 256)), dim3(256), 0, ctx->stream, q, (Fr*)d_h, (Fr*)d_hd);
+    else hipLaunchKernelGGL(k_quotient_permutation<false>, dim3(pz_div_up(N / 2, 256)), dim3(256), 0, ctx->stream, q, (Fr*)d_h, (Fr*)nullptr);
+    HIPCHK(ctx, hipGetLastError());
+    return PZ_OK;
+}
+extern "C" int pz_quotient_permutation_part_dev(pz_ctx* ctx, const uint64_t* d_cols_ext, size_t col_stride,
+                                                const uint64_t* d_sigma_ext, size_t sigma_stride, const uint64_t* d_z_ext,
+                                                size_t z_stride, uint32_t n_sets_total, uint32_t set_lo, uint32_t n_sets,
+                                                uint32_t chunk_len, uint32_t m_cols, int head, uint32_t log_ext, uint32_t rot_step,
+                                                uint32_t last_rotation, const uint64_t* d_l0, const uint64_t* d_l_last,
+                                                const uint64_t* d_l_active, const uint64_t beta[4], const uint64_t gamma[4],
+                                                const uint64_t delta[4], const uint64_t coset_g[4], const uint64_t omega_ext[4],
+                                                const uint64_t y[4], uint64_t* d_h) {
+    if (!d_l_active) return PZ_ERR_INVALID;
+    return quotient_permutation_launch(ctx, d_cols_ext, col_stride, d_sigma_ext, sigma_stride, d_z_ext, z_stride, n_sets_total, set_lo, n_sets,
+                                       chunk_len, m_cols, head, log_ext, rot_step, last_rotation, d_l0, d_l_last, d_l_active, beta, gamma, delta,
+                                       coset_g, omega_ext, y, d_h, nullptr);
+}
+extern "C" int pz_quotient_permutation_split_dev(pz_ctx* ctx, const uint64_t* d_cols_ext, size_t col_stride,
+                                                 const uint64_t* d_sigma_ext, size_t sigma_stride, const uint64_t* d_z_ext,
+                                                 size_t z_stride, uint32_t n_sets_total, uint32_t set_lo, uint32_t n_sets,
+                                                 uint32_t chunk_len, uint32_t m_cols, int head, uint32_t log_ext, uint32_t rot_step,
+                                                 uint32_t last_rotation, const uint64_t* d_l0, const uint64_t* d_l_last,
+                                                 const uint64_t beta[4], const uint64_t gamma[4], const uint64_t delta[4],
+                                                 const uint64_t coset_g[4], const uint64_t omega_ext[4], const uint64_t y[4],
+                                                 uint64_t* d_h_low, uint64_t* d_h_d) {
+    if (!d_h_d) return PZ_ERR_INVALID;
+    return quotient_permutation_launch(ctx, d_cols_ext, col_stride, d_sigma_ext, sigma_stride, d_z_ext, z_stride, n_sets_total, set_lo, n_sets,
+                                       chunk_len, m_cols, head, log_ext, rot_step, last_rotation, d_l0, d_l_last, nullptr, beta, gamma, delta,
+                                       coset_g, omega_ext, y, d_h_low, d_h_d);
 }
 extern "C" int pz_quotient_permutation_dev(pz_ctx* ctx, const uint64_t* d_cols_ext, size_t col_stride,
                                            const uint64_t* d_sigma_ext, size_t sigma_stride, const uint64_t* d_z_ext,
@@ -748,8 +782,9 @@
     size_t as, aps, sps, zs, N;
     unsigned n_lookups, step;
     S29 beta, gamma, y;
+    S29 y2, y3;
 };
-__global__ __launch_bounds__(256) void k_quotient_lookup(LookQ q, Fr* __restrict__ h) {
+template <bool SPLIT> __global__ __launch_bounds__(256) void k_quotient_lookup(LookQ q, Fr* __restrict__ h, Fr* __restrict__ hd) {
     const size_t i = (size_t)blockIdx.x * blockDim.x + threadIdx.x;
     if (i >= q.N) return;
     const size_t mask = q.N - 1;
@@ -757,7 +792,8 @@
     const Fr29 one = fr29_one256();
     const Fr29 l0 = f29_load_shl5<FrTag>(q.l0 + i), ll = f29_load_shl5<FrTag>(q.llast + i), la = f29_load_shl5<FrTag>(q.lactive + i);
     const Fr29 sg = f29_add_s(f29_load_shl5<FrTag>(q.s + i), q.gamma.v);
-    Fr29 acc = f29_load<FrTag>(h + i);
+    Fr29 acc = f29_load<FrTag>(h + i), accd;
+    if (SPLIT) accd = f29_load<FrTag>(hd + i);
     for (unsigned k = 0; k < q.n_lookups; ++k) {
         const Fr zf = fp_load<FrTag>(q.z + (size_t)k * q.zs + i);
         const Fr29 z = f29_from_fp(zf), zn = f29_load<FrTag>(q.z + (size_t)k * q.zs + i_next);
@@ -767,23 +803,28 @@
         acc = f29_mul2_s(acc, q.y.v, f29_sub<2, 29>(f29_mul(z, f29_from_fp_shl5(zf)), z), ll);
         const Fr29 f1 = f29_mul(f29_add_s(f29_from_fp_shl5(apf), q.beta.v), f29_add_s(f29_from_fp_shl5(spf), q.gamma.v));
         const Fr29 f2 = f29_mul(f29_add_s(f29_load_shl5<FrTag>(q.a + (size_t)k * q.as + i), q.beta.v), sg);
-        acc = f29_mul2_s(acc, q.y.v, f29_sub<2, 29>(f29_mul(zn, f1), f29_mul(z, f2)), la);
+        if (SPLIT) {
+            accd = f29_mul_s(f29_mul2_s(accd, q.y3.v, f29_sub<2, 29>(f29_mul(zn, f1), f29_mul(z, f2)), f29_one<FrTag>()), q.y2.v);
+            acc = f29_mul_s(acc, q.y.v);
+        } else {
+            acc = f29_mul2_s(acc, q.y.v, f29_sub<2, 29>(f29_mul(zn, f1), f29_mul(z, f2)), la);
+        }
         const Fr29 ams = f29_carry(f29_sub<2, 29>(ap, sp));
         acc = f29_mul2_s(acc, q.y.v, ams, l0);
         const Fr29 dprev = f29_sub<64, 29>(f29_from_fp_shl5(apf), f29_load_shl5<FrTag>(q.ap + (size_t)k * q.aps + i_prev));
         acc = f29_mul2_s(acc, q.y.v, f29_mul(ams, dprev), la);
     }
     f29_store<0>(h + i, acc);
-}
-
-extern "C" int pz_quotient_lookup_dev(pz_ctx* ctx, const uint64_t* d_input_ext, size_t input_stride, const uint64_t* d_table_ext,
-                                      const uint64_t* d_perm_input_ext, size_t perm_input_stride,
-                                      const uint64_t* d_perm_table_ext, size_t perm_table_stride, const uint64_t* d_z_ext,
-                                      size_t z_stride, uint32_t n_lookups, uint32_t log_ext, uint32_t rot_step,
-                                      const uint64_t* d_l0, const uint64_t* d_l_last, const uint64_t* d_l_active,
-                                      const uint64_t beta[4], const uint64_t gamma[4], const uint64_t y[4], uint64_t* d_h) {
+    if (SPLIT) f29_store<0>(hd + i, accd);
+}
+
+static int quotient_lookup_launch(pz_ctx* ctx, const uint64_t* d_input_ext, size_t input_stride, const uint64_t* d_table_ext,
+                                  const uint64_t* d_perm_input_ext, size_t perm_input_stride, const uint64_t* d_perm_table_ext,
+                                  size_t perm_table_stride, const uint64_t* d_z_ext, size_t z_stride, uint32_t n_lookups, uint32_t log_ext,
+                                  uint32_t rot_step, const uint64_t* d_l0, const uint64_t* d_l_last, const uint64_t* d_l_active,
+                                  const uint64_t beta[4], const uint64_t gamma[4], const uint64_t y[4], uint64_t* d_h, uint64_t* d_hd) {
     if (!ctx || !d_input_ext || !d_table_ext || !d_perm_input_ext || !d_perm_table_ext || !d_z_ext || !d_l0 || !d_l_last ||
-        !d_l_active || !beta || !gamma || !y || !d_h)
+        !d_l_active || !beta || !gamma || !y || !d_h || d_h == d_hd)
         return PZ_ERR_INVALID;
     if (log_ext > 28 || input_stride % 4 || perm_input_stride % 4 || perm_table_stride % 4 || z_stride % 4) return PZ_ERR_INVALID;
     const size_t N = (size_t)1 << log_ext;
@@ -800,7 +841,136 @@
     q.as = input_stride / 4; q.aps = perm_input_stride / 4; q.sps = perm_table_stride / 4; q.zs = z_stride / 4; q.N = N;
     q.n_lookups = n_lookups; q.step = rot_step;
     q.beta = host_fr_shl(beta, 5); q.gamma = host_fr_shl(gamma, 5); q.y = host_fr_shl(y, 5);
-    hipLaunchKernelGGL(k_quotient_lookup, dim3(pz_div_up(N, 256)), dim3(256), 0, ctx->stream, q, (Fr*)d_h);
+    uint64_t yp[4];
+    host_fr_mul(y, y, yp);
+    q.y2 = host_fr_shl(yp, 5);
+    host_fr_mul(yp, y, yp);
+    q.y3 = host_fr_shl(yp, 5);
+    if (d_hd) hipLaunchKernelGGL(k_quotient_lookup<true>, dim3(pz_div_up(N, 256)), dim3(256), 0, ctx->stream, q, (Fr*)d_h, (Fr*)d_hd);
+    else hipLaunchKernelGGL(k_quotient_lookup<false>, dim3(pz_div_up(N, 256)), dim3(256), 0, ctx->stream, q, (Fr*)d_h, (Fr*)nullptr);
+    HIPCHK(ctx, hipGetLastError());
+    return PZ_OK;
+}
+extern "C" int pz_quotient_lookup_dev(pz_ctx* ctx, const uint64_t* d_input_ext, size_t input_stride, const uint64_t* d_table_ext,
+                                      const uint64_t* d_perm_input_ext, size_t perm_input_stride,
+                                      const uint64_t* d_perm_table_ext, size_t perm_table_stride, const uint64_t* d_z_ext,
+                                      size_t z_stride, uint32_t n_lookups, uint32_t log_ext, uint32_t rot_step,
+                                      const uint64_t* d_l0, const uint64_t* d_l_last, const uint64_t* d_l_active,
+                                      const uint64_t beta[4], const uint64_t gamma[4], const uint64_t y[4], uint64_t* d_h) {
+    return quotient_lookup_launch(ctx, d_input_ext, input_stride, d_table_ext, d_perm_input_ext, perm_input_stride, d_perm_table_ext,
+                                  perm_table_stride, d_z_ext, z_stride, n_lookups, log_ext, rot_step, d_l0, d_l_last, d_l_active, beta, gamma, y,
+                                  d_h, nullptr);
+}
+extern "C" int pz_quotient_lookup_split_dev(pz_ctx* ctx, const uint64_t* d_input_ext, size_t input_stride, const uint64_t* d_table_ext,
+                                            const uint64_t* d_perm_input_ext, size_t perm_input_stride,
+                                            const uint64_t* d_perm_table_ext, size_t perm_table_stride, const uint64_t* d_z_ext,
+                                            size_t z_stride, uint32_t n_lookups, uint32_t log_ext, uint32_t rot_step,
+                                            const uint64_t* d_l0, const uint64_t* d_l_last, const uint64_t* d_l_active,
+                                            const uint64_t beta[4], const uint64_t gamma[4], const uint64_t y[4], uint64_t* d_h_low,
+                                            uint64_t* d_h_d) {
+    if (!d_h_d) return PZ_ERR_INVALID;
+    return quotient_lookup_launch(ctx, d_input_ext, input_stride, d_table_ext, d_perm_input_ext, perm_input_stride, d_perm_table_ext,
+                                  perm_table_stride, d_z_ext, z_stride, n_lookups, log_ext, rot_step, d_l0, d_l_last, d_l_active, beta, gamma, y,
+                                  d_h_low, d_h_d);
+}
+
+struct DRowsQ {
+    const Fr *cols, *sigma, *z, *a, *s, *ap, *sp, *zl, *wpow, *dpow, *ypow;
+    size_t cs, ss, zs, as, aps, sps, zls, n, row_lo;
+    unsigned m, chunk_len, n_sets, n_lookups;
+    Fr beta, gamma;
+};
+__global__ __launch_bounds__(256) void k_quotient_d_rows(DRowsQ q, Fr* __restrict__ part) {
+    __shared__ Fr s_t[256];
+    const unsigned t = blockIdx.x * 256 + threadIdx.x;
+    const size_t i = q.row_lo + blockIdx.y, i_next = (i + 1) & (q.n - 1);
+    Fr term = fp_zero<FrTag>();
+    if (t < q.n_sets) {
+        const unsigned c0 = t * q.chunk_len;
+        Fr left = fp_load<FrTag>(q.z + (size_t)t * q.zs + i_next), right = fp_load<FrTag>(q.z + (size_t)t * q.zs + i);
+        const Fr bw = fp_mul(q.beta, fp_load<FrTag>(q.wpow + i));
+        for (unsigned c = c0; c < c0 + q.chunk_len && c < q.m; ++c) {
+            const Fr v = fp_add(fp_load<FrTag>(q.cols + (size_t)c * q.cs + i), q.gamma);
+            left = fp_mul(left, fp_add(v, fp_mul(q.beta, fp_load<FrTag>(q.sigma + (size_t)c * q.ss + i))));
+            right = fp_mul(right, fp_add(v, fp_mul(bw, fp_load<FrTag>(q.dpow + c))));
+        }
+        term = fp_mul(fp_sub(left, right), fp_load<FrTag>(q.ypow + (q.n_sets - 1 - t) + 5u * q.n_lookups));
+    } else if (t - q.n_sets < q.n_lookups) {
+        const unsigned l = t - q.n_sets;
+        const Fr zn = fp_load<FrTag>(q.zl + (size_t)l * q.zls + i_next), z = fp_load<FrTag>(q.zl + (size_t)l * q.zls + i);
+        const Fr f1 = fp_mul(fp_add(fp_load<FrTag>(q.ap + (size_t)l * q.aps + i), q.beta), fp_add(fp_load<FrTag>(q.sp + (size_t)l * q.sps + i), q.gamma));
+        const Fr f2 = fp_mul(fp_add(fp_load<FrTag>(q.a + (size_t)l * q.as + i), q.beta), fp_add(fp_load<FrTag>(q.s + i), q.gamma));
+        term = fp_mul(fp_sub(fp_mul(zn, f1), fp_mul(z, f2)), fp_load<FrTag>(q.ypow + 5u * (q.n_lookups - 1 - l) + 2u));
+    }
+    s_t[threadIdx.x] = term;
+    __syncthreads();
+    for (unsigned off = 128; off; off >>= 1) {
+        if (threadIdx.x < off) s_t[threadIdx.x] = fp_add(s_t[threadIdx.x], s_t[threadIdx.x + off]);
+        __syncthreads();
+    }
+    if (threadIdx.x == 0) fp_store(part + (size_t)blockIdx.y * gridDim.x + blockIdx.x, s_t[0]);
+}
+__global__ void k_quotient_d_rows_sum(const Fr* __restrict__ part, unsigned nb, size_t rows, size_t row_lo, Fr* __restrict__ out) {
+    const size_t r = (size_t)blockIdx.x * blockDim.x + threadIdx.x;
+    if (r >= rows) return;
+    Fr acc = fp_zero<FrTag>();
+    for (unsigned b = 0; b < nb; ++b) acc = fp_add(acc, fp_load<FrTag>(part + r * nb + b));
+    fp_store(out + row_lo + r, acc);
+}
+
+extern "C" int pz_quotient_d_rows_dev(pz_ctx* ctx, const uint64_t* d_cols, size_t col_stride, const uint64_t* d_sigma, size_t sigma_stride,
+                                      const uint64_t* d_z, size_t z_stride, uint32_t m, uint32_t chunk_len, const uint64_t* d_input,
+                                      size_t input_stride, const uint64_t* d_table, const uint64_t* d_perm_input, size_t perm_input_stride,
+                                      const uint64_t* d_perm_table, size_t perm_table_stride, const uint64_t* d_zl, size_t zl_stride,
+                                      uint32_t n_lookups, uint32_t log_n, size_t row_lo, const uint64_t omega[4], const uint64_t beta[4],
+                                      const uint64_t gamma[4], const uint64_t delta[4], const uint64_t y[4], uint64_t* d_out) {
+    if (!ctx || !d_cols || !d_sigma || !d_z || !omega || !beta || !gamma || !delta || !y || !d_out || m == 0 || chunk_len == 0 || log_n > 26)
+        return PZ_ERR_INVALID;
+    if (n_lookups && (!d_input || !d_table || !d_perm_input || !d_perm_table || !d_zl)) return PZ_ERR_INVALID;
+    const size_t n = (size_t)1 << log_n;
+    const size_t n_sets = ((size_t)m + chunk_len - 1) / chunk_len;
+    if (row_lo >= n || n - row_lo > 65535 || m > 0xffffffu || n_lookups > 0xffffffu) return PZ_ERR_INVALID;
+    if (col_stride % 4 || sigma_stride % 4 || z_stride % 4 || input_stride % 4 || perm_input_stride % 4 || perm_table_stride % 4 || zl_stride % 4)
+        return PZ_ERR_INVALID;
+    if ((m > 1 && (col_stride < 4 * n || sigma_stride < 4 * n)) || (n_sets > 1 && z_stride < 4 * n)) return PZ_ERR_INVALID;
+    if (n_lookups > 1 && (input_stride < 4 * n || perm_input_stride < 4 * n || perm_table_stride < 4 * n || zl_stride < 4 * n)) return PZ_ERR_INVALID;
+    if (!host_fr_canonical(beta) || !host_fr_canonical(gamma) || !host_fr_canonical(delta) || !host_fr_canonical(y)) return PZ_ERR_INVALID;
+    PZ_ENTER(ctx);
+    const size_t rows = n - row_lo;
+    const unsigned nb = pz_div_up(n_sets + n_lookups, 256);
+    void *wp, *dp, *yp, *part;
+    PZCHK(pz_get_pow_table(ctx, omega, n, &wp));
+    PZCHK(pz_get_pow_table(ctx, delta, m, &dp));
+    PZCHK(pz_get_pow_table(ctx, y, n_sets + 5 * (size_t)n_lookups, &yp));
+    PZCHK(pz_ws_get(ctx, WS_MISC, rows * nb * 32, &part));
+    DRowsQ q;
+    q.cols = (const Fr*)d_cols; q.sigma = (const Fr*)d_sigma; q.z = (const Fr*)d_z; q.a = (const Fr*)d_input; q.s = (const Fr*)d_table;
+    q.ap = (const Fr*)d_perm_input; q.sp = (const Fr*)d_perm_table; q.zl = (const Fr*)d_zl;
+    q.wpow = (const Fr*)wp; q.dpow = (const Fr*)dp; q.ypow = (const Fr*)yp;
+    q.cs = col_stride / 4; q.ss = sigma_stride / 4; q.zs = z_stride / 4; q.as = input_stride / 4; q.aps = perm_input_stride / 4;
+    q.sps = perm_table_stride / 4; q.zls = zl_stride / 4; q.n = n; q.row_lo = row_lo;
+    q.m = m; q.chunk_len = chunk_len; q.n_sets = (unsigned)n_sets; q.n_lookups = n_lookups;
+    q.beta = fr_from_u64(beta); q.gamma = fr_from_u64(gamma);
+    HIPCHK(ctx, hipMemsetAsync(d_out, 0, n * 32, ctx->stream));
+    hipLaunchKernelGGL(k_quotient_d_rows, dim3(nb, (unsigned)rows), dim3(256), 0, ctx->stream, q, (Fr*)part);
+    hipLaunchKernelGGL(k_quotient_d_rows_sum, dim3(pz_div_up(rows, 64)), dim3(64), 0, ctx->stream, (const Fr*)part, nb, rows, row_lo, (Fr*)d_out);
+    HIPCHK(ctx, hipGetLastError());
+    return PZ_OK;
+}
+
+__global__ __launch_bounds__(256) void k_mul_row_cols(const Fr* a, size_t cs, size_t n, const Fr* __restrict__ row, Fr* out, size_t os) {
+    const size_t i = (size_t)blockIdx.x * blockDim.x + threadIdx.x;
+    if (i >= n) return;
+    fp_store(out + (size_t)blockIdx.y * os + i, fp_mul(fp_load<FrTag>(a + (size_t)blockIdx.y * cs + i), fp_load<FrTag>(row + i)));
+}
+extern "C" int pz_fr_mul_row_dev(pz_ctx* ctx, const uint64_t* d_a, size_t n_cols, size_t col_stride, size_t n, const uint64_t* d_row,
+                                 uint64_t* d_out, size_t out_stride) {
+    if (!ctx || col_stride % 4 || out_stride % 4 || (n_cols > 1 && (col_stride < 4 * n || out_stride < 4 * n))) return PZ_ERR_INVALID;
+    if (n_cols == 0 || n == 0) return PZ_OK;
+    if (!d_a || !d_row || !d_out || n_cols > 65535) return PZ_ERR_INVALID;
+    PZ_ENTER(ctx);
+    hipLaunchKernelGGL(k_mul_row_cols, dim3(pz_div_up(n, 256), (unsigned)n_cols), dim3(256), 0, ctx->stream, (const Fr*)d_a, col_stride / 4, n,
+                       (const Fr*)d_row, (Fr*)d_out, out_stride / 4);
     HIPCHK(ctx, hipGetLastError());
     return PZ_OK;
 }
diff --git a/paillier_halo2_amd/engine.py b/paillier_halo2_amd/engine.py
--- a/paillier_halo2_amd/engine.py
+++ b/paillier_halo2_amd/engine.py
@@ -796,6 +796,40 @@
             VP(d_perm_table_ext), perm_table_stride_u64, VP(d_z_ext), z_stride_u64, n_lookups, log_ext, rot_step, VP(d_l0),
             VP(d_l_last), VP(d_l_active), self._fr1(beta), self._fr1(gamma), self._fr1(y), VP(d_h)), "pz_quotient_lookup_dev")
 
+    def quotient_permutation_split_dev(self, d_cols_ext: int, col_stride_u64: int, d_sigma_ext: int, sigma_stride_u64: int, d_z_ext: int,
+                                       z_stride_u64: int, n_sets_total: int, set_lo: int, n_sets: int, chunk_len: int, m_cols: int,
+                                       head: bool, log_ext: int, rot_step: int, last_rotation: int, d_l0: int, d_l_last: int,
+                                       beta, gamma, delta, coset_g, omega_ext, y, d_h_low: int, d_h_d: int):
+        self._chk(self.L.pz_quotient_permutation_split_dev(
+            self.ctx, VP(d_cols_ext), col_stride_u64, VP(d_sigma_ext), sigma_stride_u64, VP(d_z_ext), z_stride_u64, n_sets_total, set_lo,
+            n_sets, chunk_len, m_cols, int(head), log_ext, rot_step, last_rotation, VP(d_l0), VP(d_l_last),
+            self._fr1(beta), self._fr1(gamma), self._fr1(delta), self._fr1(coset_g), self._fr1(omega_ext), self._fr1(y), VP(d_h_low),
+            VP(d_h_d)), "pz_quotient_permutation_split_dev")
+
+    def quotient_lookup_split_dev(self, d_input_ext: int, input_stride_u64: int, d_table_ext: int, d_perm_input_ext: int,
+                                  perm_input_stride_u64: int, d_perm_table_ext: int, perm_table_stride_u64: int, d_z_ext: int,
+                                  z_stride_u64: int, n_lookups: int, log_ext: int, rot_step: int, d_l0: int, d_l_last: int,
+                                  d_l_active: int, beta, gamma, y, d_h_low: int, d_h_d: int):
+        self._chk(self.L.pz_quotient_lookup_split_dev(
+            self.ctx, VP(d_input_ext), input_stride_u64, VP(d_table_ext), VP(d_perm_input_ext), perm_input_stride_u64,
+            VP(d_perm_table_ext), perm_table_stride_u64, VP(d_z_ext), z_stride_u64, n_lookups, log_ext, rot_step, VP(d_l0),
+            VP(d_l_last), VP(d_l_active), self._fr1(beta), self._fr1(gamma), self._fr1(y), VP(d_h_low), VP(d_h_d)),
+            "pz_quotient_lookup_split_dev")
+
+    def quotient_d_rows_dev(self, d_cols: int, col_stride_u64: int, d_sigma: int, sigma_stride_u64: int, d_z: int, z_stride_u64: int,
+                            m: int, chunk_len: int, d_input: int, input_stride_u64: int, d_table: int, d_perm_input: int,
+                            perm_input_stride_u64: int, d_perm_table: int, perm_table_stride_u64: int, d_zl: int, zl_stride_u64: int,
+                            n_lookups: int, log_n: int, row_lo: int, omega, beta, gamma, delta, y, d_out: int):
+        self._chk(self.L.pz_quotient_d_rows_dev(
+            self.ctx, VP(d_cols), col_stride_u64, VP(d_sigma), sigma_stride_u64, VP(d_z), z_stride_u64, m, chunk_len, VP(d_input),
+            input_stride_u64, VP(d_table), VP(d_perm_input), perm_input_stride_u64, VP(d_perm_table), perm_table_stride_u64, VP(d_zl),
+            zl_stride_u64, n_lookups, log_n, row_lo, self._fr1(omega), self._fr1(beta), self._fr1(gamma), self._fr1(delta),
+            self._fr1(y), VP(d_out)), "pz_quotient_d_rows_dev")
+
+    def fr_mul_row_dev(self, d_a: int, n_cols: int, col_stride_u64: int, n: int, d_row: int, d_out: int, out_stride_u64: int):
+        self._chk(self.L.pz_fr_mul_row_dev(self.ctx, VP(d_a), n_cols, col_stride_u64, n, VP(d_row), VP(d_out), out_stride_u64),
+                  "pz_fr_mul_row_dev")
+
     def quotient_finish_dev(self, d_h: int, log_n: int, log_e: int, coset_g, omega_ext):
         self._chk(self.L.pz_quotient_finish_dev(self.ctx, VP(d_h), log_n, log_e, self._fr1(coset_g), self._fr1(omega_ext)),
                   "pz_quotient_finish_dev")
diff --git a/paillier_halo2_amd/host/create_proof.hpp b/paillier_halo2_amd/host/create_proof.hpp
--- a/paillier_halo2_amd/host/create_proof.hpp
+++ b/paillier_halo2_amd/host/create_proof.hpp
@@ -274,7 +274,7 @@
 };
 
 struct Workspace {
-    uint64_t *Ap, *Sp, *Zl, *Z, *z_ext[2], *ext[2], *lk_ext[2][4], *hh[2], *hp[2], *h, *tmp, *rnd, *hcomb, *w1, *w2, *blind, *out12, *evals;
+    uint64_t *Ap, *Sp, *Zl, *Z, *z_ext, *ext[2], *lk_ext[4], *hh, *hp[2], *gq, *dvec, *d2, *h, *tmp, *rnd, *hcomb, *w1, *w2, *blind, *out12, *evals;
     uint64_t* key_ext[2] = {nullptr, nullptr};
     size_t tile, lt;
 };
@@ -287,17 +287,19 @@
     w.lt = tile < Lk ? tile : Lk;
     w.Ap = cx.alloc(cx.cols(Lk) * n * 4); w.Sp = cx.alloc(cx.cols(Lk) * n * 4); w.Zl = cx.alloc(cx.cols(Lk) * n * 4);
     w.Z = cx.alloc(cx.cols(S) * n * 4);
-    const size_t big = d.parts[0].size > d.parts[1].size ? d.parts[0].size : d.parts[1].size;
-    w.z_ext[0] = w.z_ext[1] = cx.alloc(cx.cols(S) * big * 4);
+    const size_t NA = d.parts[0].size, NB = d.parts[1].size;
+    w.z_ext = cx.alloc(cx.cols(S) * NA * 4);
     if (pk.streamed)
-        for (int q = 0; q < 2; ++q) w.key_ext[q] = cx.alloc(tile * big * 4);
-    for (int pi = 0; pi < 2; ++pi) {
-        const size_t Np = d.parts[pi].size;
-        w.ext[pi] = cx.alloc(tile * Np * 4);
-        for (int q = 0; q < 4; ++q) w.lk_ext[pi][q] = cx.alloc(w.lt * Np * 4);
-        w.hh[pi] = cx.alloc(2 * Np * 4);
-        w.hp[pi] = cx.alloc(Np * 4);
-    }
+        for (int q = 0; q < 2; ++q) w.key_ext[q] = cx.alloc(tile * NA * 4);
+    w.ext[0] = cx.alloc(tile * NA * 4);
+    w.ext[1] = cx.alloc(NB * 4);
+    for (int q = 0; q < 4; ++q) w.lk_ext[q] = cx.alloc(w.lt * NA * 4);
+    w.hh = cx.alloc(3 * NA * 4);
+    w.hp[0] = cx.alloc(NA * 4);
+    w.hp[1] = cx.alloc(NB * 4);
+    w.gq = cx.alloc(NA * 4);
+    w.dvec = cx.alloc(n * 4);
+    w.d2 = cx.alloc(n * 4);
     w.h = cx.alloc(4 * n * 4);
     w.tmp = cx.alloc(2 * n * 4);
     w.rnd = cx.alloc(n * 4);
@@ -467,84 +469,96 @@
             for (size_t c0 = 0; c0 < cnt; c0 += tile)
                 PZP_CK(pz_ntt_fr_dev(cx.c, t + c0 * n * 4, cnt - c0 < tile ? cnt - c0 : tile, 4 * n, d.omega_inv.v, k, nullptr, d.n_inv.v));
         };
+        PZP_CK(pz_quotient_d_rows_dev(cx.c, d_cols, 4 * n, pk.sigma_lagrange, 4 * n, w.Z, 4 * n, (uint32_t)m, CHUNK, d_cols + A * n * 4, 4 * n,
+                                      pk.table_lagrange, w.Ap, 4 * n, w.Sp, 4 * n, w.Zl, 4 * n, (uint32_t)Lk, k, d.usable, d.omega.v, beta.v, gamma.v,
+                                      delta.v, y.v, w.dvec));
         to_coeff(d_cols, m); to_coeff(w.Ap, Lk); to_coeff(w.Sp, Lk); to_coeff(w.Z, S); to_coeff(w.Zl, Lk);
         const size_t n_perm_lines = 2 + (S - 1) + S;
         const Fr y_gate = pow_small(y, n_perm_lines + 5 * Lk);
-        for (int pi = 0; pi < 2; ++pi) {
-            const Part& pt = d.parts[pi];
-            const size_t Np = pt.size;
-            const unsigned lg = k + pt.log_e, rot = 1u << pt.log_e;
-            auto extend = [&](const uint64_t* src, size_t cnt, uint64_t* dst) {
-                PZP_CK(pz_ntt_fr_extend_dev(cx.c, src, cnt, 4 * n, dst, 4 * Np, k, pt.log_e, d.omega.v, pt.gens.data(), nullptr));
-            };
-            for (size_t s0 = 0; s0 < S; s0 += tile) extend(w.Z + s0 * n * 4, S - s0 < tile ? S - s0 : tile, w.z_ext[pi] + s0 * Np * 4);
-            PZP_CK(pz_dev_memset(cx.c, w.hh[pi], 0, 2 * Np * 32));
-            uint64_t *hg = w.hh[pi], *hp = w.hh[pi] + Np * 4;
-            const uint64_t *l0 = pk.l_ext[pi], *llast = pk.l_ext[pi] + Np * 4, *lact = pk.l_ext[pi] + 2 * Np * 4;
+        const Part &ptA = d.parts[0], &ptB = d.parts[1];
+        auto extend = [&](const Part& pt, const uint64_t* src, size_t cnt, uint64_t* dst) {
+            PZP_CK(pz_ntt_fr_extend_dev(cx.c, src, cnt, 4 * n, dst, 4 * pt.size, k, pt.log_e, d.omega.v, pt.gens.data(), nullptr));
+        };
+        auto to_coeff_part = [&](const Part& pt, uint64_t* t) {
+            PZP_CK(pz_ntt_fr_dev(cx.c, t, 1, 4 * pt.size, pt.omega_inv.v, k + pt.log_e, nullptr, pt.size_inv.v));
+            const Fr cg_inv = pzh::inv(pt.coset_g);
+            PZP_CK(pz_fr_distribute_powers_dev(cx.c, t, 1, 4 * pt.size, pt.size, cg_inv.v, nullptr));
+        };
+        uint64_t *t0 = w.tmp, *t1 = w.tmp + n * 4;
+        auto axpy = [&](const uint64_t* a, const Fr& c, const uint64_t* b, uint64_t* out) {
+            PZP_CK(pz_dev_copy(cx.c, t0, a, n * 32));
+            PZP_CK(pz_dev_copy(cx.c, t1, b, n * 32));
+            PZP_CK(pz_fr_lincomb_dev(cx.c, w.tmp, 2, 4 * n, n, c.v, out, 0));
+        };
+        {
+            const size_t Np = ptA.size;
+            const unsigned lg = k + ptA.log_e, rot = 1u << ptA.log_e;
+            for (size_t s0 = 0; s0 < S; s0 += tile) extend(ptA, w.Z + s0 * n * 4, S - s0 < tile ? S - s0 : tile, w.z_ext + s0 * Np * 4);
+            PZP_CK(pz_dev_memset(cx.c, w.hh, 0, 3 * Np * 32));
+            uint64_t *hg = w.hh, *hlow = w.hh + Np * 4, *hd = w.hh + 2 * Np * 4;
+            const uint64_t *l0 = pk.l_ext[0], *llast = pk.l_ext[0] + Np * 4, *lact = pk.l_ext[0] + 2 * Np * 4;
             auto key_tile = [&](const uint64_t* coeff, const uint64_t* resident, size_t res, int which, size_t c0, size_t cnt) -> const uint64_t* {
                 if (c0 + cnt <= res) return resident + c0 * Np * 4;
-                extend(coeff + c0 * n * 4, cnt, w.key_ext[which]);
+                extend(ptA, coeff + c0 * n * 4, cnt, w.key_ext[which]);
                 return w.key_ext[which];
             };
             for (size_t c0 = 0; c0 < m; c0 += tile) {
                 const size_t cnt = m - c0 < tile ? m - c0 : tile;
-                extend(d_cols + c0 * n * 4, cnt, w.ext[pi]);
+                extend(ptA, d_cols + c0 * n * 4, cnt, w.ext[0]);
                 const size_t na = c0 >= A ? 0 : (A - c0 < cnt ? A - c0 : cnt);
-                if (na && pi == 0)
-                    PZP_CK(pz_quotient_gate_dev(cx.c, w.ext[pi], 4 * Np, key_tile(pk.fixed_coeff, pk.fixed_ext[pi], pk.res_fixed, 0, c0, na), 4 * Np, na,
+                if (na)
+                    PZP_CK(pz_quotient_gate_dev(cx.c, w.ext[0], 4 * Np, key_tile(pk.fixed_coeff, pk.fixed_ext[0], pk.res_fixed, 0, c0, na), 4 * Np, na,
                                                 lg, rot, y.v, hg));
-                PZP_CK(pz_quotient_permutation_part_dev(cx.c, w.ext[pi], 4 * Np, key_tile(pk.sigma_coeff, pk.sigma_ext[pi], pk.res_sigma, 1, c0, cnt),
-                                                        4 * Np, w.z_ext[pi], 4 * Np,
-                                                        (uint32_t)S, (uint32_t)(c0 / CHUNK), (uint32_t)((cnt + CHUNK - 1) / CHUNK), CHUNK, (uint32_t)cnt,
-                                                        c0 == 0, lg, rot, bf + 1, l0, llast, lact, beta.v, gamma.v, delta.v, pt.coset_g.v, pt.omega.v,
-                                                        y.v, hp));
+                PZP_CK(pz_quotient_permutation_split_dev(cx.c, w.ext[0], 4 * Np, key_tile(pk.sigma_coeff, pk.sigma_ext[0], pk.res_sigma, 1, c0, cnt),
+                                                         4 * Np, w.z_ext, 4 * Np, (uint32_t)S, (uint32_t)(c0 / CHUNK),
+                                                         (uint32_t)((cnt + CHUNK - 1) / CHUNK), CHUNK, (uint32_t)cnt, c0 == 0, lg, rot, bf + 1, l0,
+                                                         llast, beta.v, gamma.v, delta.v, ptA.coset_g.v, ptA.omega.v, y.v, hlow, hd));
             }
-            uint64_t* hq = w.hp[pi];
-            PZP_CK(pz_dev_copy(cx.c, hq, hp, Np * 32));
             for (size_t l0_ = 0; l0_ < Lk; l0_ += w.lt) {
                 const size_t cnt = Lk - l0_ < w.lt ? Lk - l0_ : w.lt;
-                extend(d_cols + (A + l0_) * n * 4, cnt, w.lk_ext[pi][0]);
-                extend(w.Ap + l0_ * n * 4, cnt, w.lk_ext[pi][1]);
-                extend(w.Sp + l0_ * n * 4, cnt, w.lk_ext[pi][2]);
-                extend(w.Zl + l0_ * n * 4, cnt, w.lk_ext[pi][3]);
-                PZP_CK(pz_quotient_lookup_dev(cx.c, w.lk_ext[pi][0], 4 * Np, pk.table_ext[pi], w.lk_ext[pi][1], 4 * Np,
-                                              w.lk_ext[pi][2], 4 * Np, w.lk_ext[pi][3], 4 * Np, (uint32_t)cnt, lg, rot, l0, llast, lact, beta.v, gamma.v,
-                                              y.v, hq));
+                extend(ptA, d_cols + (A + l0_) * n * 4, cnt, w.lk_ext[0]);
+                extend(ptA, w.Ap + l0_ * n * 4, cnt, w.lk_ext[1]);
+                extend(ptA, w.Sp + l0_ * n * 4, cnt, w.lk_ext[2]);
+                extend(ptA, w.Zl + l0_ * n * 4, cnt, w.lk_ext[3]);
+                PZP_CK(pz_quotient_lookup_split_dev(cx.c, w.lk_ext[0], 4 * Np, pk.table_ext[0], w.lk_ext[1], 4 * Np, w.lk_ext[2], 4 * Np,
+                                                    w.lk_ext[3], 4 * Np, (uint32_t)cnt, lg, rot, l0, llast, lact, beta.v, gamma.v, y.v, hlow, hd));
             }
-            PZP_CK(pz_quotient_finish_dev(cx.c, hq, k, pt.log_e, pt.coset_g.v, pt.omega.v));
-            PZP_CK(pz_ntt_fr_dev(cx.c, hq, 1, 4 * Np, pt.omega_inv.v, lg, nullptr, pt.size_inv.v));
-            const Fr cg_inv = pzh::inv(pt.coset_g);
-            PZP_CK(pz_fr_distribute_powers_dev(cx.c, hq, 1, 4 * Np, Np, cg_inv.v, nullptr));
-            if (pi == 0) {
-                PZP_CK(pz_quotient_finish_dev(cx.c, hg, k, pt.log_e, pt.coset_g.v, pt.omega.v));
-                PZP_CK(pz_ntt_fr_dev(cx.c, hg, 1, 4 * Np, pt.omega_inv.v, lg, nullptr, pt.size_inv.v));
-                PZP_CK(pz_fr_distribute_powers_dev(cx.c, hg, 1, 4 * Np, Np, cg_inv.v, nullptr));
+            PZP_CK(pz_fr_lincomb_dev(cx.c, w.hh, 2, 4 * Np, Np, y_gate.v, w.gq, 0));
+            PZP_CK(pz_quotient_finish_dev(cx.c, w.gq, k, ptA.log_e, ptA.coset_g.v, ptA.omega.v));
+            to_coeff_part(ptA, w.gq);
+            PZP_CK(pz_fr_mul_row_dev(cx.c, hd, 1, 4 * Np, Np, lact, w.hp[0], 4 * Np));
+            to_coeff_part(ptA, hd);
+        }
+        const Fr g2n = pow_small(pzh::mul(d.coset_g, d.coset_g), n);
+        const Fr lam = pow_small(ptB.coset_g, n);
+        const Fr m1 = pzh::neg(pzh::FR_ONE), mg2n = pzh::neg(g2n);
+        {
+            PZP_CK(pz_ntt_fr_dev(cx.c, w.dvec, 1, 4 * n, d.omega_inv.v, k, nullptr, d.n_inv.v));
+            const uint64_t *U_D = w.hh + 2 * ptA.size * 4, *D_1 = U_D + n * 4;
+            axpy(U_D, pzh::FR_ONE, D_1, w.d2);
+            axpy(w.d2, m1, w.dvec, w.d2);
+            const Fr scale = pzh::inv(pzh::add(pzh::FR_ONE, mg2n));
+            PZP_CK(pz_fr_distribute_powers_dev(cx.c, w.d2, 1, 4 * n, n, pzh::FR_ONE.v, scale.v));
+            axpy(w.d2, pzh::add(mg2n, mg2n), U_D, w.hp[1]);
+            axpy(D_1, lam, w.hp[1], w.hp[1]);
+            extend(ptB, w.hp[1], 1, w.ext[1]);
+            PZP_CK(pz_fr_mul_row_dev(cx.c, w.ext[1], 1, 4 * n, n, pk.l_ext[1] + 2 * ptB.size * 4, w.hp[1], 4 * n));
+            for (int pi = 0; pi < 2; ++pi) {
+                const Part& pt = d.parts[pi];
+                PZP_CK(pz_quotient_finish_dev(cx.c, w.hp[pi], k, pt.log_e, pt.coset_g.v, pt.omega.v));
+                to_coeff_part(pt, w.hp[pi]);
             }
         }
         pieces = w.h;
         {
-            const Fr g2n = pow_small(pzh::mul(d.coset_g, d.coset_g), n);
-            const Fr lam = pow_small(d.parts[1].coset_g, n);
             uint64_t *U = w.hp[0], *h1 = w.hp[0] + n * 4, *V = w.hp[1];
-            uint64_t *t0 = w.tmp, *t1 = w.tmp + n * 4;
-            PZP_CK(pz_dev_copy(cx.c, pieces + n * 4, h1, n * 32));
-            PZP_CK(pz_dev_copy(cx.c, t0, h1, n * 32));
-            PZP_CK(pz_dev_copy(cx.c, t1, V, n * 32));
-            const Fr mlam = pzh::neg(lam), m1 = pzh::neg(pzh::FR_ONE), mg2n = pzh::neg(g2n);
-            PZP_CK(pz_fr_lincomb_dev(cx.c, w.tmp, 2, 4 * n, n, mlam.v, pieces + 2 * n * 4, 0));
-            PZP_CK(pz_dev_copy(cx.c, t0, pieces + 2 * n * 4, n * 32));
-            PZP_CK(pz_dev_copy(cx.c, t1, U, n * 32));
-            PZP_CK(pz_fr_lincomb_dev(cx.c, w.tmp, 2, 4 * n, n, m1.v, pieces + 2 * n * 4, 0));
+            axpy(h1, pzh::neg(lam), V, pieces + 2 * n * 4);
+            axpy(pieces + 2 * n * 4, m1, U, pieces + 2 * n * 4);
             const Fr half = pzh::inv(pzh::add(g2n, g2n));
             PZP_CK(pz_fr_distribute_powers_dev(cx.c, pieces + 2 * n * 4, 1, 4 * n, n, pzh::FR_ONE.v, half.v));
-            PZP_CK(pz_dev_copy(cx.c, t0, pieces + 2 * n * 4, n * 32));
-            PZP_CK(pz_dev_copy(cx.c, t1, U, n * 32));
-            PZP_CK(pz_fr_lincomb_dev(cx.c, w.tmp, 2, 4 * n, n, mg2n.v, pieces, 0));
-            for (size_t i = 0; i < 2; ++i) {
-                PZP_CK(pz_dev_copy(cx.c, t0, w.hh[0] + i * n * 4, n * 32));
-                PZP_CK(pz_dev_copy(cx.c, t1, pieces + i * n * 4, n * 32));
-                PZP_CK(pz_fr_lincomb_dev(cx.c, w.tmp, 2, 4 * n, n, y_gate.v, pieces + i * n * 4, 0));
-            }
+            axpy(pieces + 2 * n * 4, mg2n, U, pieces);
+            axpy(w.gq, pzh::FR_ONE, pieces, pieces);
+            axpy(w.gq + n * 4, pzh::FR_ONE, h1, pieces + n * 4);
         }
         commit(pk.bm, pieces, 3, w.out12);
         affine(w.out12, 3, out_h);
@@ -645,11 +659,12 @@
         PZP_CK(pz_shplonk_finish_dev(cx.c, st_, shu.v, w.w1, w.w2));
         commit(pk.bm, w.w2, 1, w.out12);
         affine(w.out12, 1, out_w2);
-        uint64_t top[12 + 8];
+        uint64_t top[12 + 8 + 8];
         PZP_CK(pz_download(cx.c, top, pieces + (3 * n - 3) * 4, 96));
-        PZP_CK(pz_download(cx.c, top + 12, w.hh[0] + (2 * n - 2) * 4, 64));
+        PZP_CK(pz_download(cx.c, top + 12, w.gq + (2 * n - 2) * 4, 64));
+        PZP_CK(pz_download(cx.c, top + 20, w.d2 + (n - 2) * 4, 64));
         done(6);
-        for (int i = 0; i < 12 + 8; ++i)
+        for (int i = 0; i < 12 + 8 + 8; ++i)
             if (top[i]) return false;
         return true;
     }
diff --git a/paillier_halo2_amd/prover.py b/paillier_halo2_amd/prover.py
--- a/paillier_halo2_amd/prover.py
+++ b/paillier_halo2_amd/prover.py
@@ -349,12 +349,17 @@
         big = max(pt["size"] for pt in d.parts)
         self._z_ext_flat = _zeros_cap(S, big, 4).view(-1)
         self.z_ext = [self._z_ext_flat[: S * pt["size"] * 4].view(S, pt["size"], 4) for pt in d.parts]
-        self.ext = [_zeros(tile, pt["size"], 4) for pt in d.parts]
+        two = len(d.parts) == 2
+        self.ext = [_zeros(tile if pi == 0 else 1, pt["size"], 4) for pi, pt in enumerate(d.parts)]
         if pk.streamed:
             self._key_tiles = [_zeros(tile, big, 4).view(-1) for _ in range(2)]
             self.key_ext = [[kt[: tile * pt["size"] * 4].view(tile, pt["size"], 4) for kt in self._key_tiles] for pt in d.parts]
-        self.lk_ext = [[_zeros(lt, pt["size"], 4) for _ in range(4)] for pt in d.parts]
-        self.hh = [_zeros(2, pt["size"], 4) for pt in d.parts]
+        self.lk_ext = [[_zeros(lt, pt["size"], 4) for _ in range(4)] for pt in d.parts[:1]]
+        self.hh = [_zeros(3 if two else 2, pt["size"], 4) for pt in d.parts[:1]]
+        if two:
+            self.gq = _zeros(d.parts[0]["size"], 4)
+            self.dvec = _zeros(n, 4)
+            self.d2 = _zeros(n, 4)
         self.hp = [_zeros(pt["size"], 4) for pt in d.parts]
         self.h = _zeros(N, 4)
         self.tmp = _zeros(2, n, 4)
@@ -469,84 +474,130 @@
     y_i = tr.squeeze("y")
     y = M(y_i)
     phase("products_commit")
+    if len(d.parts) == 2:
+        dvec = ws.dvec
+        eng.quotient_d_rows_dev(cols.data_ptr(), 4 * n, pk.sigma_lagrange.data_ptr(), 4 * n, Z.data_ptr(), 4 * n, m, CHUNK, lk_in.data_ptr(), 4 * n,
+                                pk.table_lagrange.data_ptr(), Ap.data_ptr(), 4 * n, Sp.data_ptr(), 4 * n, Zl.data_ptr(), 4 * n, Lk, k, u, M(d.omega),
+                                beta, gamma, M(DELTA), y, dvec.data_ptr())
     for t, cnt in ((cols, m), (Ap, Lk), (Sp, Lk), (Z, S), (Zl, Lk)):
         to_coeff(t, cnt)
     n_perm_lines = 2 + (S - 1) + S
     lt = ws.lk_ext[0][0].shape[0]
-    split_gate = len(d.parts) == 2
-    for pi, pt in enumerate(d.parts):
+    Rf, Rs = pk.ext_resident
+    h = ws.h
+    pieces = h.view(d.E, n, 4)
+
+    def key_tile(pi, coeff, resident, R_, which, c0, cnt):
+        if not pk.streamed or c0 + cnt <= R_:
+            return resident[pi][c0].data_ptr()
+        buf = ws.key_ext[pi][which]
+        extend(coeff[c0:c0 + cnt], cnt, buf, d.parts[pi])
+        return buf.data_ptr()
+
+    def to_coeff_part(t, pt):
+        eng.ntt_dev(t.data_ptr(), 1, 4 * pt["size"], M(pt["omega_inv"]), k + pt["log_e"], None, M(pt["size_inv"]))
+        eng.fr_distribute_powers_dev(t.data_ptr(), 1, 4 * pt["size"], pt["size"], M(pow(pt["coset_g"], -1, FR)))
+
+    t01 = ws.tmp
+
+    def axpy(a, c, b, out):
+        t01[0].copy_(a); t01[1].copy_(b)
+        eng.fr_lincomb_dev(t01.data_ptr(), 2, 4 * n, n, M(c % FR), out.data_ptr())
+
+    if len(d.parts) == 1:
+        pt = d.parts[0]
         Np, lg, rot = pt["size"], k + pt["log_e"], pt["E"]
         cg, om = M(pt["coset_g"]), M(pt["omega"])
-        z_ext = ws.z_ext[pi]
+        z_ext = ws.z_ext[0]
         for s0 in range(0, S, tile):
             extend(Z[s0:s0 + tile], min(tile, S - s0), z_ext[s0:s0 + tile], pt)
-        ws.hh[pi].zero_()
-        hg, hp = ws.hh[pi][0], ws.hh[pi][1]
-        ext = ws.ext[pi]
-        l0, llast, lact = (pk.l_ext[pi][i].data_ptr() for i in range(3))
-        Rf, Rs = pk.ext_resident
-
-        def key_tile(coeff, resident, R_, which, c0, cnt):
-            if not pk.streamed or c0 + cnt <= R_:
-                return resident[pi][c0].data_ptr()
-            buf = ws.key_ext[pi][which]
-            extend(coeff[c0:c0 + cnt], cnt, buf, pt)
-            return buf.data_ptr()
-
+        ws.hh[0].zero_()
+        hg, hp = ws.hh[0][0], ws.hh[0][1]
+        ext = ws.ext[0]
+        l0, llast, lact = (pk.l_ext[0][i].data_ptr() for i in range(3))
         for c0 in range(0, m, tile):
             cnt = min(tile, m - c0)
             extend(cols[c0:c0 + cnt], cnt, ext, pt)
             na = max(0, min(A, c0 + cnt) - c0)
-            if na and (pi == 0 or not split_gate):
-                eng.quotient_gate_dev(ext.data_ptr(), 4 * Np, key_tile(pk.fixed_coeff, pk.fixed_ext, Rf, 0, c0, na), 4 * Np, na, lg, rot, y, hg.data_ptr())
+            if na:
+                eng.quotient_gate_dev(ext.data_ptr(), 4 * Np, key_tile(0, pk.fixed_coeff, pk.fixed_ext, Rf, 0, c0, na), 4 * Np, na, lg, rot, y, hg.data_ptr())
             set_lo, nsets = c0 // CHUNK, -(-cnt // CHUNK)
-            eng.quotient_permutation_part_dev(ext.data_ptr(), 4 * Np, key_tile(pk.sigma_coeff, pk.sigma_ext, Rs, 1, c0, cnt), 4 * Np, z_ext.data_ptr(), 4 * Np, S, set_lo,
+            eng.quotient_permutation_part_dev(ext.data_ptr(), 4 * Np, key_tile(0, pk.sigma_coeff, pk.sigma_ext, Rs, 1, c0, cnt), 4 * Np, z_ext.data_ptr(), 4 * Np, S, set_lo,
                                               nsets, CHUNK, cnt, c0 == 0, lg, rot, bf + 1, l0, llast, lact, beta, gamma, M(DELTA), cg, om, y,
                                               hp.data_ptr())
-        hq = ws.hp[pi]
-        if split_gate:
-            hq.copy_(hp)
-        else:
-            eng.fr_lincomb_dev(ws.hh[pi].data_ptr(), 2, 4 * Np, Np, M(pow(y_i, n_perm_lines, FR)), hq.data_ptr())
+        hq = ws.hp[0]
+        eng.fr_lincomb_dev(ws.hh[0].data_ptr(), 2, 4 * Np, Np, M(pow(y_i, n_perm_lines, FR)), hq.data_ptr())
         for l0_ in range(0, Lk, lt):
             cnt = min(lt, Lk - l0_)
-            e_in, e_ap, e_sp, e_zl = ws.lk_ext[pi]
+            e_in, e_ap, e_sp, e_zl = ws.lk_ext[0]
             extend(cols[A + l0_:A + l0_ + cnt], cnt, e_in, pt)
             extend(Ap[l0_:l0_ + cnt], cnt, e_ap, pt)
             extend(Sp[l0_:l0_ + cnt], cnt, e_sp, pt)
             extend(Zl[l0_:l0_ + cnt], cnt, e_zl, pt)
-            eng.quotient_lookup_dev(e_in.data_ptr(), 4 * Np, pk.table_ext[pi].data_ptr(), e_ap.data_ptr(), 4 * Np, e_sp.data_ptr(), 4 * Np,
+            eng.quotient_lookup_dev(e_in.data_ptr(), 4 * Np, pk.table_ext[0].data_ptr(), e_ap.data_ptr(), 4 * Np, e_sp.data_ptr(), 4 * Np,
                                     e_zl.data_ptr(), 4 * Np, cnt, lg, rot, l0, llast, lact, beta, gamma, y, hq.data_ptr())
         eng.quotient_finish_dev(hq.data_ptr(), k, pt["log_e"], cg, om)
-        eng.ntt_dev(hq.data_ptr(), 1, 4 * Np, M(pt["omega_inv"]), lg, None, M(pt["size_inv"]))
-        eng.fr_distribute_powers_dev(hq.data_ptr(), 1, 4 * Np, Np, M(pow(pt["coset_g"], -1, FR)))
-        if split_gate and pi == 0:
-            eng.quotient_finish_dev(hg.data_ptr(), k, pt["log_e"], cg, om)
-            eng.ntt_dev(hg.data_ptr(), 1, 4 * Np, M(pt["omega_inv"]), lg, None, M(pt["size_inv"]))
-            eng.fr_distribute_powers_dev(hg.data_ptr(), 1, 4 * Np, Np, M(pow(pt["coset_g"], -1, FR)))
-    h = ws.h
-    pieces = h.view(d.E, n, 4)
-    if len(d.parts) == 1:
-        h.copy_(ws.hp[0])
+        to_coeff_part(hq, pt)
+        h.copy_(hq)
     else:
+        ptA, ptB = d.parts
+        Np, lg, rot = ptA["size"], k + ptA["log_e"], ptA["E"]
+        cg, om = M(ptA["coset_g"]), M(ptA["omega"])
+        z_ext = ws.z_ext[0]
+        for s0 in range(0, S, tile):
+            extend(Z[s0:s0 + tile], min(tile, S - s0), z_ext[s0:s0 + tile], ptA)
+        ws.hh[0].zero_()
+        hg, hlow, hd = ws.hh[0][0], ws.hh[0][1], ws.hh[0][2]
+        ext = ws.ext[0]
+        l0, llast, lact = (pk.l_ext[0][i].data_ptr() for i in range(3))
+        for c0 in range(0, m, tile):
+            cnt = min(tile, m - c0)
+            extend(cols[c0:c0 + cnt], cnt, ext, ptA)
+            na = max(0, min(A, c0 + cnt) - c0)
+            if na:
+                eng.quotient_gate_dev(ext.data_ptr(), 4 * Np, key_tile(0, pk.fixed_coeff, pk.fixed_ext, Rf, 0, c0, na), 4 * Np, na, lg, rot, y, hg.data_ptr())
+            set_lo, nsets = c0 // CHUNK, -(-cnt // CHUNK)
+            eng.quotient_permutation_split_dev(ext.data_ptr(), 4 * Np, key_tile(0, pk.sigma_coeff, pk.sigma_ext, Rs, 1, c0, cnt), 4 * Np, z_ext.data_ptr(), 4 * Np, S,
+                                               set_lo, nsets, CHUNK, cnt, c0 == 0, lg, rot, bf + 1, l0, llast, beta, gamma, M(DELTA), cg, om, y,
+                                               hlow.data_ptr(), hd.data_ptr())
+        for l0_ in range(0, Lk, lt):
+            cnt = min(lt, Lk - l0_)
+            e_in, e_ap, e_sp, e_zl = ws.lk_ext[0]
+            extend(cols[A + l0_:A + l0_ + cnt], cnt, e_in, ptA)
+            extend(Ap[l0_:l0_ + cnt], cnt, e_ap, ptA)
+            extend(Sp[l0_:l0_ + cnt], cnt, e_sp, ptA)
+            extend(Zl[l0_:l0_ + cnt], cnt, e_zl, ptA)
+            eng.quotient_lookup_split_dev(e_in.data_ptr(), 4 * Np, pk.table_ext[0].data_ptr(), e_ap.data_ptr(), 4 * Np, e_sp.data_ptr(), 4 * Np,
+                                          e_zl.data_ptr(), 4 * Np, cnt, lg, rot, l0, llast, lact, beta, gamma, y, hlow.data_ptr(), hd.data_ptr())
+        gq = ws.gq
+        eng.fr_lincomb_dev(ws.hh[0].data_ptr(), 2, 4 * Np, Np, M(pow(y_i, n_perm_lines + 5 * Lk, FR)), gq.data_ptr())
+        eng.quotient_finish_dev(gq.data_ptr(), k, ptA["log_e"], cg, om)
+        to_coeff_part(gq, ptA)
+        eng.fr_mul_row_dev(hd.data_ptr(), 1, 4 * Np, Np, lact, ws.hp[0].data_ptr(), 4 * Np)
+        to_coeff_part(hd, ptA)
         g2n = pow(d.coset_g, 2 * n, FR)
-        lam = pow(d.parts[1]["coset_g"], n, FR)
+        lam = pow(ptB["coset_g"], n, FR)
+        eng.ntt_dev(dvec.data_ptr(), 1, 4 * n, M(d.omega_inv), k, None, M(d.n_inv))
+        U_D, D_1, D_2, D_B = hd[:n], hd[n:], ws.d2, ws.hp[1]
+        axpy(U_D, 1, D_1, D_2)
+        axpy(D_2, -1, dvec, D_2)
+        eng.fr_distribute_powers_dev(D_2.data_ptr(), 1, 4 * n, n, M(1), M(pow(1 - g2n, -1, FR)))
+        axpy(D_2, -2 * g2n, U_D, D_B)
+        axpy(D_1, lam, D_B, D_B)
+        extB = ws.ext[1]
+        extend(D_B.view(1, n, 4), 1, extB, ptB)
+        eng.fr_mul_row_dev(extB.data_ptr(), 1, 4 * n, n, pk.l_ext[1][2].data_ptr(), ws.hp[1].data_ptr(), 4 * n)
+        for pi, pt in enumerate(d.parts):
+            eng.quotient_finish_dev(ws.hp[pi].data_ptr(), k, pt["log_e"], M(pt["coset_g"]), M(pt["omega"]))
+            to_coeff_part(ws.hp[pi], pt)
         U, h1, V = ws.hp[0][:n], ws.hp[0][n:], ws.hp[1]
-        pieces[1].copy_(h1)
-        t01 = ws.tmp
-        t01[0].copy_(h1); t01[1].copy_(V)
-        eng.fr_lincomb_dev(t01.data_ptr(), 2, 4 * n, n, M(-lam % FR), pieces[2].data_ptr())
-        t01[0].copy_(pieces[2]); t01[1].copy_(U)
-        eng.fr_lincomb_dev(t01.data_ptr(), 2, 4 * n, n, M(FR - 1), pieces[2].data_ptr())
+        axpy(h1, -lam, V, pieces[2])
+        axpy(pieces[2], -1, U, pieces[2])
         eng.fr_distribute_powers_dev(pieces[2].data_ptr(), 1, 4 * n, n, M(1), M(pow(2 * g2n, -1, FR)))
-        t01[0].copy_(pieces[2]); t01[1].copy_(U)
-        eng.fr_lincomb_dev(t01.data_ptr(), 2, 4 * n, n, M(-g2n % FR), pieces[0].data_ptr())
+        axpy(pieces[2], -g2n, U, pieces[0])
         pieces[3].zero_()
-        c_gate = M(pow(y_i, n_perm_lines + 5 * Lk, FR))
-        gq = ws.hh[0][0]
-        for i in range(2):
-            t01[0].copy_(gq[i * n:(i + 1) * n]); t01[1].copy_(pieces[i])
-            eng.fr_lincomb_dev(t01.data_ptr(), 2, 4 * n, n, c_gate, pieces[i].data_ptr())
+        axpy(gq[:n], 1, pieces[0], pieces[0])
+        axpy(gq[n:], 1, h1, pieces[1])
     c_h = commit(bm, pieces, d.E - 1, 4 * n)
     (a_h,) = tr.absorb_points(eng, c_h)
     x_i = tr.squeeze("x")
@@ -613,7 +664,7 @@
     top = host(h[3 * n - 3:] if len(d.parts) == 1 else h[3 * n - 3:3 * n])
     pr.h_top = top
     pr.h_degree_ok = not top.any()
-    if split_gate:
-        pr.h_degree_ok = pr.h_degree_ok and not host(ws.hh[0][0][2 * n - 2:2 * n]).any()
+    if len(d.parts) == 2:
+        pr.h_degree_ok = pr.h_degree_ok and not host(ws.gq[2 * n - 2:2 * n]).any() and not host(ws.d2[n - 2:n]).any()
     phase("finalise")
     return pr
diff --git a/rust/pz-sys/src/lib.rs b/rust/pz-sys/src/lib.rs
--- a/rust/pz-sys/src/lib.rs
+++ b/rust/pz-sys/src/lib.rs
@@ -267,6 +267,26 @@
                                   perm_table_stride: usize, d_z_ext: *const u64, z_stride: usize, n_lookups: u32, log_ext: u32,
                                   rot_step: u32, d_l0: *const u64, d_l_last: *const u64, d_l_active: *const u64,
                                   beta: *const u64, gamma: *const u64, y: *const u64, d_h: *mut u64) -> c_int;
+    pub fn pz_quotient_permutation_split_dev(ctx: *mut pz_ctx, d_cols_ext: *const u64, col_stride: usize, d_sigma_ext: *const u64,
+                                             sigma_stride: usize, d_z_ext: *const u64, z_stride: usize, n_sets_total: u32,
+                                             set_lo: u32, n_sets: u32, chunk_len: u32, m_cols: u32, head: c_int, log_ext: u32,
+                                             rot_step: u32, last_rotation: u32, d_l0: *const u64, d_l_last: *const u64,
+                                             beta: *const u64, gamma: *const u64, delta: *const u64, coset_g: *const u64,
+                                             omega_ext: *const u64, y: *const u64, d_h_low: *mut u64, d_h_d: *mut u64) -> c_int;
+    pub fn pz_quotient_lookup_split_dev(ctx: *mut pz_ctx, d_input_ext: *const u64, input_stride: usize, d_table_ext: *const u64,
+                                        d_perm_input_ext: *const u64, perm_input_stride: usize, d_perm_table_ext: *const u64,
+                                        perm_table_stride: usize, d_z_ext: *const u64, z_stride: usize, n_lookups: u32, log_ext: u32,
+                                        rot_step: u32, d_l0: *const u64, d_l_last: *const u64, d_l_active: *const u64,
+                                        beta: *const u64, gamma: *const u64, y: *const u64, d_h_low: *mut u64,
+                                        d_h_d: *mut u64) -> c_int;
+    pub fn pz_quotient_d_rows_dev(ctx: *mut pz_ctx, d_cols: *const u64, col_stride: usize, d_sigma: *const u64, sigma_stride: usize,
+                                  d_z: *const u64, z_stride: usize, m: u32, chunk_len: u32, d_input: *const u64, input_stride: usize,
+                                  d_table: *const u64, d_perm_input: *const u64, perm_input_stride: usize, d_perm_table: *const u64,
+                                  perm_table_stride: usize, d_zl: *const u64, zl_stride: usize, n_lookups: u32, log_n: u32,
+                                  row_lo: usize, omega: *const u64, beta: *const u64, gamma: *const u64, delta: *const u64,
+                                  y: *const u64, d_out: *mut u64) -> c_int;
+    pub fn pz_fr_mul_row_dev(ctx: *mut pz_ctx, d_a: *const u64, n_cols: usize, col_stride: usize, n: usize, d_row: *const u64,
+                             d_out: *mut u64, out_stride: usize) -> c_int;
     pub fn pz_quotient_finish_dev(ctx: *mut pz_ctx, d_h: *mut u64, log_n: u32, log_e: u32, coset_g: *const u64,
                                   omega_ext: *const u64) -> c_int;
     pub fn pz_fr_distribute_powers_dev(ctx: *mut pz_ctx, d_a: *mut u64, n_cols: usize, col_stride: usize, n: usize,
```
